# IntelLabs/coach

Measured on AMD Instinct MI355X. Metric: env-steps/sec (+ grad-updates/sec) on Atari-like Clipped-PPO, 64 vectorized envs/GPU, higher is better.
Workload: dtype f32; 1 GPU; C2: Atari-Pong-like Clipped-PPO, 64 vectorized envs/GPU, 84x84x4 uint8 obs, GAE(0.99,0.95), rollout 2048 env-steps (episodes of 32), 10 epochs x 32 minibatches of 64, fp32 conv torso x2 (value/policy), TF1-Adam; parallelism=dp1 (env vectors sharded per GPU, flat fp32 gradient all-reduce), hip_graphs=True

## Files before the change

### coach_amd/_rlx.py

```python
import ctypes
import os
import re
import subprocess
import threading

_HERE = os.path.dirname(os.path.abspath(__file__))
_ROOT = os.path.dirname(_HERE)
HEADER = os.path.join(_ROOT, "include", "rlx.h")
LIB_PATH = os.path.join(_HERE, "librlx.so")
CSRC = os.path.join(_HERE, "csrc")


class RlxUnavailable(RuntimeError):
    """librlx.so is missing or cannot be loaded; the HIP hot path cannot run."""


class RlxError(RuntimeError):
    """A librlx entry point returned a non-zero rlx_status."""


_CTYPE = {
    "int": ctypes.c_int,
    "unsigned": ctypes.c_uint,
    "unsigned int": ctypes.c_uint,
# ... 78 lines not shown
                             {"_fields_": fields, "__doc__": "%s (include/rlx.h)." % name, "__module__": __name__})
    return structs


def parse_constants(text):
    consts = {k: int(v) for k, v in _DEFINE.findall(text)}
    for body in _ENUM.findall(text):
        for item in filter(None, (" ".join(i.split()) for i in body.split(","))):
            m = re.fullmatch(r"(RLX_\w+) ?= ?(-?\d+)", item)
            if not m:
                raise ValueError("rlx.h: enumerator %r needs an explicit integer value" % item)
            consts[m.group(1)] = int(m.group(2))
    return consts


def build_library(verbose=False):
    hipcc = os.environ.get("HIPCC", "/opt/rocm/bin/hipcc")
    if not os.path.exists(hipcc):
        raise RlxUnavailable("hipcc not found at %s; cannot build librlx.so" % hipcc)
    jobs = str(max(1, min(16, os.cpu_count() or 1)))
    res = subprocess.run(["make", "-C", CSRC, "-j", jobs, "HIPCC=" + hipcc],
                         stdout=subprocess.PIPE, stderr=subprocess.STDOUT, text=True)
    if verbose or res.returncode != 0:
        print(res.stdout)
    if res.returncode != 0:
        raise RlxUnavailable("building librlx.so failed (see output above)")
    return LIB_PATH


def _as_arg(a):
    if hasattr(a, "data_ptr"):
        if hasattr(a, "is_contiguous") and not a.is_contiguous():
            raise ValueError("librlx expects contiguous tensors")
        return a.data_ptr()
    return a


class _Lib:
    def __init__(self):
        import torch

        if not os.path.exists(LIB_PATH):
            if os.path.exists("/opt/rocm/bin/hipcc"):
                build_library()
            else:
                raise RlxUnavailable(
                    "%s is missing and hipcc is not available to build it. Run "
                    "`python -c 'import __graft_entry__ as g; g.build()'`." % LIB_PATH)
        try:
            self._dll = ctypes.CDLL(LIB_PATH, mode=ctypes.RTLD_GLOBAL)
        except OSError as e:
            raise RlxUnavailable("cannot load %s: %s" % (LIB_PATH, e))
        self.protos = parse_header()
        self._fns = {}
        missing = []
        for name, (restype, params) in self.protos.items():
            try:
                fn = getattr(self._dll, name)
            except AttributeError:
                missing.append(name)
                continue
            fn.restype = restype
            fn.argtypes = [t for t, _ in params]
            self._fns[name] = fn
        if missing:
            raise RlxUnavailable("librlx.so does not export: " + ", ".join(missing))
        built = self._fns["rlx_abi_version"]()
        if built != ABI_VERSION:
            raise RlxUnavailable("%s is ABI version %d, this package drives version %d: rebuild it "
                                 "(python -c 'import __graft_entry__ as g; g.build()')" % (LIB_PATH, built, ABI_VERSION))

    def raw(self, name):
        return self._fns[name]

    def last_error(self):
        return self._fns["rlx_last_error"]().decode()

    def __getattr__(self, name):
        fns = self.__dict__.get("_fns", {})
        full = name if name.startswith("rlx_") else "rlx_" + name
        if full not in fns:
            raise AttributeError(name)
        fn = fns[full]
        nparams = len(self.protos[full][1])
        if fn.restype is ctypes.c_char_p:
            def call_str(*args):
                return fn(*args).decode()
            return call_str
        if returns_value(full):
            return fn

        def call(*args):
            global CALL_COUNT
            CALL_COUNT += 1
            if len(args) != nparams:
                raise TypeError("%s expects %d arguments, got %d" % (full, nparams, len(args)))
            rc = fn(*[_as_arg(a) for a in args])
            if rc != 0:
                raise RlxError("%s failed (%d): %s" % (full, rc, self.last_error()))
            return rc
        call.__name__ = full
        setattr(self, name, call)
        return call


_lock = threading.Lock()
_lib = None


def lib():
    global _lib
    if _lib is None:
        with _lock:
            if _lib is None:
                _lib = _Lib()
    return _lib


def current_stream():
    import torch
    return torch.cuda.current_stream().cuda_stream


class KernelTimer(object):

    def __init__(self, max_records=4096):
        self.max_records, self.records = int(max_records), []

    def __enter__(self):
        lib().profile_begin(self.max_records)
        return self

    def __exit__(self, *exc):
        n = ctypes.c_int()
        try:
            lib().profile_end(ctypes.byref(n))
        except Exception:
            if exc[0] is None:
                raise
        if exc[0] is None:
            name, ms = ctypes.c_char_p(), ctypes.c_float()
            for i in range(n.value):
                lib().profile_read(i, ctypes.byref(name), ctypes.byref(ms))
                self.records.append((name.value.decode().strip("()"), 1e3 * ms.value))
        return False


STRUCT_NAMES = {
    "rlx_column": "Column", "rlx_gemm_desc": "GemmDesc", "rlx_splitk_job": "SplitkJob", "rlx_noisy_layer": "NoisyLayer",
    "rlx_per_update_desc": "PerUpdateDesc", "rlx_conv_dw_item": "ConvDwItem",
    "rlx_small_dense_problem": "SmallDenseProblem", "rlx_mlp_dqn_desc": "MlpDqnDesc", "rlx_mlp3": "Mlp3",
    "rlx_fused_net": "FusedNet", "rlx_td3_fused_desc": "Td3FusedDesc", "rlx_sac_fused_desc": "SacFusedDesc",
    "rlx_ppo_fc_heads_desc": "PpoFcHeadsDesc", "rlx_ppo_rows_desc": "PpoRowsDesc", "rlx_observe_desc": "ObserveDesc",
    "rlx_signal_source": "SignalSource",
}
_TEXT = header_text()
STRUCTS = parse_structs(_TEXT, STRUCT_NAMES)
CONSTANTS = parse_constants(_TEXT)

Column, GemmDesc, NoisyLayer = STRUCTS["rlx_column"], STRUCTS["rlx_gemm_desc"], STRUCTS["rlx_noisy_layer"]
PerUpdateDesc, ConvDwItem = STRUCTS["rlx_per_update_desc"], STRUCTS["rlx_conv_dw_item"]
SmallDenseProblem, MlpDqnDesc = STRUCTS["rlx_small_dense_problem"], STRUCTS["rlx_mlp_dqn_desc"]
Mlp3, FusedNet = STRUCTS["rlx_mlp3"], STRUCTS["rlx_fused_net"]
Td3FusedDesc, SacFusedDesc = STRUCTS["rlx_td3_fused_desc"], STRUCTS["rlx_sac_fused_desc"]
PpoFcHeadsDesc, PpoRowsDesc = STRUCTS["rlx_ppo_fc_heads_desc"], STRUCTS["rlx_ppo_rows_desc"]
ObserveDesc, SignalSource = STRUCTS["rlx_observe_desc"], STRUCTS["rlx_signal_source"]


class SplitkJob(STRUCTS["rlx_splitk_job"]):
    __doc__ = STRUCTS["rlx_splitk_job"].__doc__

    def workspace_floats(self):
        return (self.M * self.N + self.N) * self.batch * self.splits if self.splits > 1 else 0


ABI_VERSION = CONSTANTS["RLX_ABI_VERSION"]
NOISY_PASSES = CONSTANTS["RLX_NOISY_PASSES"]
NOISY_MAX_LAYERS = CONSTANTS["RLX_NOISY_MAX_LAYERS"]
NOISY_PASS = {"act": 0, "online": 1, "target": 2, "online_next": 3}
assert sorted(NOISY_PASS.values()) == list(range(NOISY_PASSES)), "NOISY_PASS names every pass of RLX_NOISY_PASSES"
ADAM_TICKET_WORDS = CONSTANTS["RLX_ADAM_TICKET_WORDS"]
MAX_SPLITK_JOBS = CONSTANTS["RLX_MAX_SPLITK_JOBS"]
MAX_COLUMNS = CONSTANTS["RLX_MAX_COLUMNS"]
A3C_TARGETS_GIVEN = CONSTANTS["RLX_A3C_TARGETS_GIVEN"]
NSTEPQ_HORIZON = {"N-Step": CONSTANTS["RLX_NSTEPQ_N_STEP"], "1-Step": CONSTANTS["RLX_NSTEPQ_ONE_STEP"]}
NSTEPQ_TARGETS_GIVEN = CONSTANTS["RLX_NSTEPQ_TARGETS_GIVEN"]
ACER_TRUST_REGION, ACER_TARGETS_GIVEN = CONSTANTS["RLX_ACER_TRUST_REGION"], CONSTANTS["RLX_ACER_TARGETS_GIVEN"]
ACT = {None: CONSTANTS["RLX_ACT_NONE"]}
ACT.update((k[len("RLX_ACT_"):].lower(), v) for k, v in CONSTANTS.items() if k.startswith("RLX_ACT_"))


def make_columns(pairs):
    arr = (Column * len(pairs))()
    for i, (s, d) in enumerate(pairs):
        rb = (s[0].numel() if s.dim() > 1 else 1) * s.element_size()
        arr[i] = Column(s.data_ptr(), d.data_ptr(), rb)
    return arr


def splitk_reduce_jobs(jobs, stream=None, ppo_tail=None, per_tail=None):
    live = [j for j in jobs if j.splits > 1]
    s = current_stream() if stream is None else stream
    for i in range(0, len(live), MAX_SPLITK_JOBS):
        chunk = live[i:i + MAX_SPLITK_JOBS]
        arr = (SplitkJob * len(chunk))(*chunk)
        if per_tail is not None and ppo_tail is None and i + MAX_SPLITK_JOBS >= len(live):
            run = lambda a=arr, n=len(chunk), t=per_tail: lib().splitk_reduce_jobs_per_update(ctypes.byref(a), n, *t, s)
            per_tail = None
        elif ppo_tail is not None and i + MAX_SPLITK_JOBS >= len(live):
            run = lambda a=arr, n=len(chunk), t=ppo_tail: lib().splitk_reduce_jobs_ppo_tail(ctypes.byref(a), n, ctypes.byref(t), s)
            ppo_tail = None
        else:
            run = lambda a=arr, n=len(chunk): lib().splitk_reduce_jobs(ctypes.byref(a), n, s)
        _record((), run, flops=0.0)
        run()
    if ppo_tail is not None:
        lib().ppo_heads_tail(ctypes.byref(ppo_tail), s)
    if per_tail is not None:
        lib().per_update(*per_tail, s)


def conv_input_grad(dz, weights, dx, x_out, deriv, tables, B, H, W, C, KH, KW, S, Co, towers, dy_stride, w_stride,
                    dx_stride, stream=None):
    s = current_stream() if stream is None else stream
    OH, OW = (H - KH) // S + 1, (W - KW) // S + 1
    run = lambda: lib().conv_input_grad(dz, weights, dx, x_out, ACT[deriv], tables, B, H, W, C, KH, KW, S, Co, towers,
                                        dy_stride, w_stride, dx_stride, s)
    if GEMM_HOOK is not None:
        d = GemmDesc()
        d.M, d.N, d.K, d.batch = B * OH * OW, KH * KW * C, Co, towers
        _record((d,), run)
    run()


def per_update_desc(args):
    sum_t, min_t, max_t, cap, idx, err, n, alpha, eps, maxp, status = args
    d = PerUpdateDesc()
    d.sum_tree, d.min_tree, d.max_tree, d.capacity = sum_t.data_ptr(), min_t.data_ptr(), max_t.data_ptr(), int(cap)
    d.idx, d.td_errors, d.n, d.alpha, d.epsilon = idx.data_ptr(), err.data_ptr(), int(n), float(alpha), float(eps)
    d.max_priority, d.status = maxp.data_ptr(), status.data_ptr()
    return d


def conv_dw_item(x, x_tower_stride, x_is_u8, a_div, dz, dz_tower_stride, B, H, W, C, KH, KW, S, Co, towers, dw, dw_tower_stride, db,
                 db_tower_stride, workspace):
    it = ConvDwItem()
    it.x, it.x_tower_stride, it.x_is_u8, it.a_div = x.data_ptr(), x_tower_stride, int(bool(x_is_u8)), float(a_div)
    it.dz, it.dz_tower_stride = dz.data_ptr(), dz_tower_stride
    it.B, it.H, it.W, it.C, it.KH, it.KW, it.S, it.filters, it.towers = B, H, W, C, KH, KW, S, Co, towers
    it.dw, it.dw_tower_stride, it.db, it.db_tower_stride = dw.data_ptr(), dw_tower_stride, _ptr(db), db_tower_stride
    it.workspace, it.workspace_floats = workspace.data_ptr(), workspace.numel()
    return it


def conv_dw_multi(items, jobs, stream=None):
    s = current_stream() if stream is None else stream
    n = len(items)
    arr = (ConvDwItem * n)(*items)
    jarr = (SplitkJob * n)()

    def run():
        lib().conv_dw_multi(arr, jarr, n, s)
    if GEMM_HOOK is not None:
        descs = []
        for it in items:
            OH, OW = (it.H - it.KH) // it.S + 1, (it.W - it.KW) // it.S + 1
            d = GemmDesc()
            d.M, d.K = it.KH * it.KW * it.C, it.B * OH * OW
            d.N, d.batch, d.a_is_u8 = (it.towers * it.filters, 1, 1) if it.x_is_u8 else (it.filters, it.towers, 0)
            descs.append(d)
        _record(tuple(descs), run)
    run()
    for j, out in zip(jarr, jobs):
        ctypes.memmove(ctypes.byref(out), ctypes.byref(j), ctypes.sizeof(SplitkJob))


GEMM_HOOK = None
CALL_COUNT = 0


def _ptr(t):
    return None if t is None else (t.data_ptr() if hasattr(t, "data_ptr") else t)


def gemm(M, N, K, A, B, C, *, a_strides=None, a_tabs=None, a_u8=False, a_div=1.0,
         a_vec_along_k=1, a_tab_vec_ok=0, b_strides=None, ldc=None, bias=None, activation=None,
         deriv_aux=None, aux_ld=None, deriv_kind=None, accumulate=False, batch=1,
         a_batch_stride=0, b_batch_stride=0, c_batch_stride=0, bias_batch_stride=0,
         aux_batch_stride=0, workspace=None, colsum_out=None, colsum_batch_stride=0, stream=None,
         batch_inner=0, a_batch_stride2=0, b_batch_stride2=0, bias_batch_stride2=0, n_fold=0, launch=True,
         defer=None, row_heads=None, kw_min_tiles=0):
    d = GemmDesc()
    d.M, d.N, d.K, d.batch = int(M), int(N), int(K), int(batch)
    d.A, d.B, d.C = _ptr(A), _ptr(B), _ptr(C)
    if a_tabs is not None:
        d.a_row_tab, d.a_k_tab = _ptr(a_tabs[0]), _ptr(a_tabs[1])
        d.a_row_stride, d.a_k_stride = 0, 0
    else:
        rs, ks = a_strides if a_strides is not None else (K, 1)
        d.a_row_stride, d.a_k_stride = int(rs), int(ks)
    ks, ns = b_strides if b_strides is not None else (N, 1)
    d.b_k_stride, d.b_n_stride = int(ks), int(ns)
    d.a_batch_stride, d.b_batch_stride = int(a_batch_stride), int(b_batch_stride)
    d.ldc = int(N if ldc is None else ldc)
    d.c_batch_stride, d.bias_batch_stride = int(c_batch_stride), int(bias_batch_stride)
    d.bias, d.deriv_aux = _ptr(bias), _ptr(deriv_aux)
    d.aux_ld = int(N if aux_ld is None else aux_ld)
    d.aux_batch_stride = int(aux_batch_stride)
    d.workspace = _ptr(workspace)
    d.colsum_out, d.colsum_batch_stride = _ptr(colsum_out), int(colsum_batch_stride)
    d.workspace_floats = int(workspace.numel()) if workspace is not None else 0
    d.a_is_u8, d.a_div = int(bool(a_u8)), float(a_div)
    d.a_vec_along_k, d.a_tab_vec_ok = int(a_vec_along_k), int(a_tab_vec_ok)
    d.activation, d.deriv_kind = ACT[activation], ACT[deriv_kind]
    d.accumulate = int(bool(accumulate))
    d.batch_inner = int(batch_inner)
    d.a_batch_stride2, d.b_batch_stride2 = int(a_batch_stride2), int(b_batch_stride2)
    d.bias_batch_stride2 = int(bias_batch_stride2)
    d.n_fold = int(n_fold)
    d.kw_min_tiles = int(kw_min_tiles)
    if row_heads is not None:
        d._row_heads = row_heads
        d.row_heads, d.n_row_heads = ctypes.addressof(row_heads), len(row_heads)
    if not launch:
        return d
    s = current_stream() if stream is None else stream
    if defer is not None:
        run = lambda: lib().gemm_defer(ctypes.byref(d), ctypes.byref(defer), s)
    else:
        run = lambda: lib().gemm(ctypes.byref(d), s)
    _record((d,), run)
    run()


def _record(descs, run, flops=None):
    if GEMM_HOOK is not None:
        GEMM_HOOK({"descs": tuple(GemmDesc.from_buffer_copy(x) for x in descs), "run": run, "flops": flops})


def gemm_pair_or_single(desc, stream=None):
    s = current_stream() if stream is None else stream
    run = lambda: lib().gemm(ctypes.byref(desc), s)
    _record((desc,), run)
    run()


def gemm_multi(descs, jobs, stream=None):
    s = current_stream() if stream is None else stream
    n = len(descs)
    darr = (GemmDesc * n)(*descs)
    jarr = (SplitkJob * n)()

    def run():
        lib().gemm_multi_defer(darr, n, jarr, s)
        for i, j in enumerate(jobs):
            ctypes.memmove(ctypes.addressof(j), ctypes.addressof(jarr[i]), ctypes.sizeof(SplitkJob))
    _record(tuple(descs), run)
    run()


def gemm_pair(weight_grad, input_grad, stream=None, defer=None):
    s = current_stream() if stream is None else stream
    if defer is not None:
        run = lambda: lib().gemm_pair_defer(ctypes.byref(weight_grad), ctypes.byref(input_grad), ctypes.byref(defer), s)
    else:
        run = lambda: lib().gemm_pair(ctypes.byref(weight_grad), ctypes.byref(input_grad), s)
    _record((weight_grad, input_grad), run)
    run()
```

### coach_amd/agents/clipped_ppo_agent.py

```python
import os
import random

import numpy as np
import torch

from .. import _rlx
from ..core_types import EnvironmentSteps, RunPhase
from ..memories.episodic.episodic_rollout_buffer import DeviceEpisodicRolloutBuffer
from ..nn.networks import ClippedPPONet
from ..schedules import ConstantSchedule


from ..architectures.scheme_views import SchemeViews


class ClippedPPONetworkParameters(SchemeViews):
    def __init__(self):
        self.activation_function = 'tanh'
        self.embedder_scheme = 'Medium'
        self.middleware_scheme = 'Medium'
        self.batch_size = 64
        self.optimizer_type = 'Adam'
        self.learning_rate = 0.00025
        self.adam_optimizer_beta1 = 0.9
        self.adam_optimizer_beta2 = 0.99
        self.optimizer_epsilon = 0.0001
        self.clip_gradients = None
        self.use_separate_networks_per_head = True
        self.async_training = False
        self.l2_regularization = 0
        self.create_target_network = True
        self.shared_optimizer = True
        self.scale_down_gradients_by_number_of_workers_for_sync_training = True


class ClippedPPOAlgorithmParameters(object):
    def __init__(self):
        self.discount = 0.99
        self.num_episodes_in_experience_replay = 1000000
        self.gae_lambda = 0.95
        self.use_kl_regularization = False
        self.clip_likelihood_ratio_using_epsilon = 0.2
        self.estimate_state_value_using_gae = True
        self.beta_entropy = 0.01
        self.num_consecutive_playing_steps = EnvironmentSteps(2048)
        self.num_consecutive_training_steps = 1
        self.optimization_epochs = 10
        self.clipping_decay_schedule = ConstantSchedule(1)
        self.act_for_full_episodes = True
        self.reward_clipping = (-1.0, 1.0)
        self.reward_rescale = 1.0
        self.normalize_observations = False


class ClippedPPOAgentParameters(object):
    def __init__(self):
        self.algorithm = ClippedPPOAlgorithmParameters()
        self.network_wrappers = {"main": ClippedPPONetworkParameters()}
        self.seed = 0

    @property
    def path(self):
        return 'coach_amd.agents.clipped_ppo_agent:ClippedPPOAgent'


def _capture(fn):
    from .vector_agent import capture
    return capture(fn)


class ClippedPPOAgent(object):
    epoch_graph = True
    ragged = False
    _device_env = True
    restarts_memory_on_reset = True
    FUSE_ACTING_LAUNCHES = True
    RECORD_WHILE_ACTING = True
    DATASET_CHUNK = 2048

    def __init__(self, agent_parameters, environment, device=None, dist=None, use_graphs=None):
        self.ap = agent_parameters
        self.env = environment
        self.device = device or environment.device
        self.dist = dist if (dist is not None and dist.enabled) else None
        self.lib = _rlx.lib()
        self.use_graphs = True if use_graphs is None else bool(use_graphs)
        self.overlap_allreduce = None if self.dist is not None else False
        self.overlap_decision = None
        alg, net = self.ap.algorithm, self.ap.network_wrappers["main"]
        ep = environment.p
        self.continuous = ep.action_dim is not None
        self.n_env, self.A = ep.num_envs, (ep.action_dim if self.continuous else ep.num_actions)
        self.image = ep.kind == "image"
        self.stack = 4
        self.L = ep.episode_length
        obs_shape = tuple(ep.observation_shape) + (self.stack,) if self.image else tuple(ep.observation_shape)
        if self.ap.seed is not None:
            random.seed(self.ap.seed)
            np.random.seed(self.ap.seed)
        self.networks = {"main": ClippedPPONet(
            self.device, obs_shape, self.A, activation=net.activation_function,
            embedder=net.embedder_scheme, middleware=net.middleware_scheme,
            learning_rate=net.learning_rate, adam_beta1=net.adam_optimizer_beta1,
            adam_beta2=net.adam_optimizer_beta2, optimizer_epsilon=net.optimizer_epsilon,
            clip_likelihood_ratio_using_epsilon=alg.clip_likelihood_ratio_using_epsilon,
            beta_entropy=alg.beta_entropy, seed=self.ap.seed or 0, continuous=self.continuous)}
        if self.dist is not None and self.ap.seed is not None:
            random.seed(self.ap.seed + self.dist.rank)
            np.random.seed(self.ap.seed + self.dist.rank)
        per_env = -(-alg.num_consecutive_playing_steps.num_steps // self.n_env)
        self.steps_per_phase = -(-per_env // self.L) * self.L
        self._device_env = hasattr(environment, "launch_step") and hasattr(environment, "host_tick")
        lens = getattr(environment, "lengths_host", None)
        self.ragged = getattr(environment, "dones_host", None) is not None and \
            (lens is None or getattr(environment, "lengths", None) is not None)
        if self.ragged:
            longest = int(max(lens)) if lens is not None else int(self.L)
            self.steps_per_phase = per_env + longest * (1 if lens is not None else 4)
        self.memory = DeviceEpisodicRolloutBuffer(
            self.device, self.n_env, self.steps_per_phase,
            frame_shape=ep.observation_shape if self.image else None, stack=self.stack,
            obs_dim=None if self.image else int(ep.observation_shape[0]),
            action_dim=self.A if self.continuous else None)
        self._rec_missing = False
        dev, n = self.device, self.n_env
        self.actions = torch.zeros((n, self.A), dtype=torch.float32, device=dev) if self.continuous else \
            torch.zeros(n, dtype=torch.int32, device=dev)
        self.norm = None
        if alg.normalize_observations:
            if self.image:
                raise ValueError("ObservationNormalizationFilter applies to vector observations")
            from ..filters.observation import ObservationNormalizationFilter
            self.norm = ObservationNormalizationFilter(int(ep.observation_shape[0]), dev)
            self.act_obs = torch.empty(n, int(ep.observation_shape[0]), dtype=torch.float32, device=dev)
        self._records_acting()
        if self.continuous:
            lo = np.broadcast_to(np.asarray(ep.action_low, dtype=np.float32), (self.A,)).copy()
            hi = np.broadcast_to(np.asarray(ep.action_high, dtype=np.float32), (self.A,)).copy()
            self.d_low, self.d_high = torch.from_numpy(lo).to(dev), torch.from_numpy(hi).to(dev)
        self.filtered_reward = torch.zeros(n, dtype=torch.float32, device=dev)
        self.ep_return = torch.zeros(n, dtype=torch.float64, device=dev)
        self.ep_len = torch.zeros(n, dtype=torch.int32, device=dev)
        self.ep_acc = torch.zeros(8, dtype=torch.float64, device=dev)
        self.lib.episode_stats_init(self.ep_return, self.ep_len, n, self.ep_acc, _rlx.current_stream())
        self.phase = RunPhase.TRAIN
        self.total_steps_counter = 0
        self.last_training_phase_step = 0
        self.training_iteration = 0
        self.signals = {}
        self._graphs = {}
        self._warm = set()
        self._episode_steps = np.zeros(self.n_env, dtype=np.int64)
        self._episode_just_ended = False
        self._draw_pool, self._draw_pos, self._draw_table_from = None, 0, None
        self._eval_mem = None
        self._alloc_training_buffers()
        self.memory.reset(self.env.reset_internal_state())

    def _alloc_training_buffers(self):
        from ..staging import Stager
        dev, B = self.device, self.ap.network_wrappers["main"].batch_size
        cap = self.memory.cap
        f32, f64 = torch.float32, torch.float64
        self.ds_reward = torch.empty(cap, dtype=f32, device=dev)
        self.ds_done = torch.empty(cap, dtype=torch.uint8, device=dev)
        act_shape = (cap, self.A) if self.continuous else (cap,)
        self.ds_action = torch.empty(act_shape, dtype=self.actions.dtype, device=dev)
        self.ds_value = torch.empty(cap, dtype=f32, device=dev)
        self.ds_adv64 = torch.empty(cap, dtype=f64, device=dev)
        self.ds_adv = torch.empty(cap, dtype=f32, device=dev)
        self.ds_vtarget = torch.empty(cap, dtype=f32, device=dev)
        self.ds_old_probs = torch.empty(cap, self.A, dtype=f32, device=dev)
        self.ds_old_std = torch.empty(cap, self.A, dtype=f32, device=dev) if self.continuous else None
        if self.norm is not None:
            D = self.memory.obs_dim
            self.ds_obs_raw = torch.empty(cap, D, dtype=f32, device=dev)
            self.ds_obs = torch.empty(cap, D, dtype=f32, device=dev)
        self.adv_stats = torch.empty(2, dtype=f64, device=dev)
        obs_tail = tuple(self.memory.cur_state.shape[1:])
        odt = self.memory.cur_state.dtype
        self.chunk = min(int(self.DATASET_CHUNK), cap)
        self.chunk_obs = torch.empty((self.chunk,) + obs_tail, dtype=odt, device=dev)
        self.mb_obs = torch.empty((B,) + obs_tail, dtype=odt, device=dev)
        self.mb_rows = torch.empty(B, dtype=torch.int32, device=dev)
        self._perm = Stager((cap,), torch.int32, dev, depth=4)
        self.perm_dev = self._perm.dst
        self.mb_action = torch.empty((B, self.A) if self.continuous else (B,), dtype=self.actions.dtype, device=dev)
        self.mb_old_std = torch.empty(B, self.A, dtype=f32, device=dev) if self.continuous else None
        self.mb_adv = torch.empty(B, dtype=f32, device=dev)
        self.mb_vtarget = torch.empty(B, dtype=f32, device=dev)
        self.mb_old = torch.empty(B, self.A, dtype=f32, device=dev)
        self.mb_ratio = torch.empty(B, dtype=f32, device=dev)
        self.mb_clipped = torch.empty(B, dtype=f32, device=dev)
        self.scalar_acc = torch.zeros(8, dtype=f32, device=dev)
        shape = (self.steps_per_phase, self.n_env, self.A) if self.continuous else (self.steps_per_phase, self.n_env)
        if self.ragged:
            shape = (1,) + shape[1:]
        self._uniforms = Stager(shape, f64, dev, depth=32 if self.ragged else 4)
        self.uniforms_all = self._uniforms.dst

    def _run(self, key, fn):
        if not self.use_graphs:
            return fn()
        g = self._graphs.get(key)
        if g is not None:
            return g.replay()
        if key not in self._warm:
            self._warm.add(key)
            return fn()
        torch.cuda.synchronize()
        self._graphs[key] = _capture(fn)
        return self._graphs[key].replay()

    def _refill_draws(self, from_step):
        shape = (self.n_env, self.A) if self.continuous else (self.n_env,)
        need = self.steps_per_phase - from_step
        left = self._draw_pool[self._draw_pos:] if self._draw_pool is not None else np.zeros((0,) + shape)
        if left.shape[0] < need:
            m = need - left.shape[0]
            fresh = np.random.standard_normal((m,) + shape) if self.continuous else np.random.random_sample((m,) + shape)
            left = np.concatenate([left, fresh], 0)
        self._draw_pool, self._draw_pos = left, 0
        table = np.zeros((self.steps_per_phase,) + shape, dtype=np.float64)
        table[from_step:] = left[:need]
        self._uniforms.push(table)
        self._draw_table_from = from_step

    def _act_device(self, step):
        s = _rlx.current_stream()
        alg = self.ap.algorithm
# ... 142 lines not shown
        else:
            if getattr(self, "_eval_state", None) is None:
                self._eval_state = torch.empty_like(self.memory.cur_state)
            self._eval_state.copy_(first)
        if getattr(self, "_eval_total", None) is None:
            self._eval_total = torch.zeros(n, dtype=torch.float64, device=dev)
            self._eval_active = torch.ones(n, dtype=torch.float64, device=dev)
        self._eval_total.zero_()
        self._eval_active.fill_(1.0)
        finished = np.zeros(n, dtype=np.int64)
        lockstep_t = 0
        try:
            while (finished < episodes_per_env).any():
                if self._device_env:
                    self._run(("evaluate",), lambda: self._evaluate_device(scratch))
                    self.env.host_tick()
                else:
                    self._evaluate_device(scratch)
                self.env.total_steps += n
                dh = getattr(self.env, "dones_host", None)
                if dh is None:
                    lockstep_t += 1
                    dh = np.full(n, lockstep_t % self.L == 0)
                was_active = finished < episodes_per_env
                finished += dh.astype(np.int64)
                active = finished < episodes_per_env
                if (active != was_active).any():
                    self._eval_active.copy_(torch.from_numpy(active.astype(np.float64)))
        finally:
            self.phase = prev
            self.env.phase = prev_env if prev_env is not None else prev
            self._episode_steps[:] = 0
            self._episode_just_ended = False
            self.lib.episode_stats_init(self.ep_return, self.ep_len, n, None, s)
            self.memory.reset(self.env.reset_internal_state())
        return float(self._eval_total.mean().item()) / episodes_per_env

    def _should_train(self):
        steps = self.ap.algorithm.num_consecutive_playing_steps.num_steps
        if self.ragged:
            done = self.memory.num_transitions_in_complete_episodes()
            if done >= steps or (self.memory.steps >= self.memory.T and done > 0):
                if done < steps and self.dist is not None:
                    raise ValueError("rollout buffer full with %d < %d complete-episode transitions: with data "
                                     "parallelism every rank trains on num_consecutive_playing_steps transitions; "
                                     "declare a longer max episode length" % (done, steps))
                self.last_training_phase_step = self.total_steps_counter
                return True
            if self.memory.steps >= self.memory.T:
                raise ValueError("no episode completed within %d vector steps: an episode is longer than the "
                                 "environment's declared maximum" % self.memory.T)
            return False
        enough = (self.total_steps_counter - self.last_training_phase_step) >= steps
        complete = self.memory.steps > 0 and self.memory.steps % self.L == 0
        if enough and complete and self.memory.num_transitions() > 0:
            self.last_training_phase_step = self.total_steps_counter
            return True
        return False

    def _fill_advantages_device(self, n, rows, n_train=None, recorded=False):
        mem, net, alg = self.memory, self.networks["main"], self.ap.algorithm
        n_train = n if n_train is None else min(n, n_train)
        s = _rlx.current_stream()
        cols = [(mem.reward, self.ds_reward), (mem.game_over, self.ds_done), (mem.action, self.ds_action)]
        if recorded:
            cols += [(mem.act_value, self.ds_value), (mem.act_probs, self.ds_old_probs)]
        mem.gather_columns(rows, n, cols)
        if self.norm is not None:
            mem.gather_states(rows, n, self.ds_obs_raw[:n])
            self.norm.filter(self.ds_obs_raw[:n], update_internal_state=self.dist is None, out=self.ds_obs[:n])
            if self.dist is None:
                mem.gather_next_states(rows, n, self.ds_obs_raw[:n])
                self.norm.push(self.ds_obs_raw[:n])

        def chunk_obs(c0, m):
            if self.norm is not None:
                return self.ds_obs[c0:c0 + m]
            return mem.gather_states(rows[c0:c0 + m], m, self.chunk_obs[:m])
        for c0 in range(0, 0 if recorded else n, self.chunk):
            m = min(self.chunk, n - c0)
            net.values(chunk_obs(c0, m), m, out=self.ds_value[c0:c0 + m])
        n_seq = 1 if self.ragged else mem.n_env
        self.lib.gae(self.ds_reward, self.ds_value, self.ds_done, None, n_seq, n // n_seq,
                     alg.discount, alg.gae_lambda, self.ds_adv64, self.ds_vtarget, s)
        self.lib.standardize(self.ds_adv64, n, self.ds_adv, None, self.adv_stats, s)
        for c0 in range(0, 0 if recorded else n_train, self.chunk):
            m = min(self.chunk, n_train - c0)
            if self.continuous:
                net.policy_mean_std(chunk_obs(c0, m), m, use_target=True, tag="old",
                                    out_mean=self.ds_old_probs[c0:c0 + m], out_std=self.ds_old_std[c0:c0 + m])
            else:
                net.policy_probs(chunk_obs(c0, m), m, use_target=True, tag="old",
                                 out=self.ds_old_probs[c0:c0 + m])

    def fill_advantages(self):
        n = self.memory.num_transitions()
        rows = self.memory.dataset_rows()
        if self.norm is not None and self.dist is not None:
            self.memory.gather_states(rows, n, self.ds_obs_raw[:n])
            self.norm.push_shared(self.ds_obs_raw[:n], self.dist)
        n_train = min(n, self.ap.algorithm.num_consecutive_playing_steps.num_steps)
        recorded = self._records_acting() and not self._rec_missing
        self._run(("fill", n, n_train, recorded), lambda: self._fill_advantages_device(n, rows, n_train, recorded))
        if self.norm is not None and self.dist is not None:
            self.memory.gather_next_states(rows, n, self.ds_obs_raw[:n])
            self.norm.push_shared(self.ds_obs_raw[:n], self.dist)

    def _gather_minibatch(self, m, i=0):
        mem, s = self.memory, _rlx.current_stream()
        rows_all = mem.dataset_rows()
        B = self.ap.network_wrappers["main"].batch_size
        idx, rows = self.perm_dev[i * B:i * B + m], self.mb_rows[:m]
        cols = [(rows_all, rows), (self.ds_action, self.mb_action), (self.ds_adv, self.mb_adv), (self.ds_vtarget, self.mb_vtarget),
                (self.ds_old_probs, self.mb_old)]
        if self.continuous:
            cols.append((self.ds_old_std, self.mb_old_std))
        if self.norm is not None:
            cols.append((self.ds_obs, self.mb_obs))
        self.lib.copy_columns(_rlx.make_columns(cols), len(cols), idx, None, 0, 0, self.ds_adv.numel(), m, m,
                              mem.status, s)
        if self.norm is not None:
            return self.mb_obs[:m]
        return mem.gather_states(rows, m, self.mb_obs[:m])

    def _gather_epoch(self, n):
        mem, s = self.memory, _rlx.current_stream()
        e = self._epoch_buffers()
        cols = [(mem.dataset_rows(), e["rows"]), (self.ds_action, e["action"]), (self.ds_adv, e["adv"]),
                (self.ds_vtarget, e["vtarget"]), (self.ds_old_probs, e["old"])]
        if self.continuous:
            cols.append((self.ds_old_std, e["old_std"]))
        if self.norm is not None:
            cols.append((self.ds_obs, e["obs"]))
        self.lib.copy_columns(_rlx.make_columns(cols), len(cols), self.perm_dev[:n], None, 0, 0, self.ds_adv.numel(), n, n,
                              mem.status, s)
        if self.norm is None:
            mem.gather_states(e["rows"][:n], n, e["obs"][:n])
        return e

    def _epoch_buffers(self):
        e = getattr(self, "_epoch_bufs", None)
        if e is None:
            cap, dev, f32 = self.memory.cap, self.device, torch.float32
            e = self._epoch_bufs = dict(
                rows=torch.empty(cap, dtype=torch.int32, device=dev),
                action=torch.empty((cap, self.A) if self.continuous else (cap,), dtype=self.actions.dtype, device=dev),
                adv=torch.empty(cap, dtype=f32, device=dev), vtarget=torch.empty(cap, dtype=f32, device=dev),
                old=torch.empty(cap, self.A, dtype=f32, device=dev),
                old_std=torch.empty(cap, self.A, dtype=f32, device=dev) if self.continuous else None,
                obs=torch.empty((cap,) + tuple(self.mb_obs.shape[1:]), dtype=self.mb_obs.dtype, device=dev))
        return e

    def _minibatch_fb(self, m, clip_rescaler, stop_after_dense=False, i=0, epoch=None):
        if epoch is not None:
            B = self.ap.network_wrappers["main"].batch_size
            sl = slice(i * B, i * B + m)
            old = (epoch["old"][sl], epoch["old_std"][sl]) if self.continuous else epoch["old"][sl]
            self.networks["main"].forward_backward(epoch["obs"][sl], m, epoch["action"][sl], epoch["adv"][sl],
                                                   epoch["vtarget"][sl], old, clip_rescaler, self.mb_ratio,
                                                   self.mb_clipped, stop_after_dense=stop_after_dense)
            return
        obs = self._gather_minibatch(m, i)
        old = (self.mb_old, self.mb_old_std) if self.continuous else self.mb_old
        self.networks["main"].forward_backward(obs, m, self.mb_action, self.mb_adv, self.mb_vtarget,
                                               old, clip_rescaler, self.mb_ratio, self.mb_clipped,
                                               stop_after_dense=stop_after_dense)

    def _minibatch_finish(self, scale):
        net = self.networks["main"]
        net.finish_update(scale, signal_acc=self.scalar_acc)

    OVERLAP_EDGE_PAIR_US = 50.0

    def _decide_overlap(self, n, clip):
        net, d = self.networks["main"], self.dist
        off = net.late_gradient_offset()
        rec = {"graph_resident": bool(self.use_graphs and d.capturable()), "edge_pair_us": self.OVERLAP_EDGE_PAIR_US,
               "late_bucket_allreduce_us": None, "conv_backward_us": None}
        if not rec["graph_resident"] or off <= 0:
            rec.update(overlap=False, why="collectives are not graph nodes on this backend" if off > 0
                       else "no early-finished bucket (no convolution layers)")
        else:
            B = self.ap.network_wrappers["main"].batch_size
            m = min(B, n)
            e = self._gather_epoch(n)
            ev = [torch.cuda.Event(enable_timing=True) for _ in range(2)]
            us = []
            for _ in range(3):
                self._minibatch_fb(m, clip, True, i=0, epoch=e)
                ev[0].record()
                net.backward_rest()
                ev[1].record()
                ev[1].synchronize()
                us.append(1e3 * ev[0].elapsed_time(ev[1]))
            bw = d.max_over_ranks(min(us))
            ar = d.max_over_ranks(d.all_reduce_us(net.params.grads.numel() - off) or 0.0)
            hidden = min(ar, bw)
            rec.update(late_bucket_allreduce_us=round(ar, 1), conv_backward_us=round(bw, 1), overlap=bool(hidden > self.OVERLAP_EDGE_PAIR_US),
                       why="min(all-reduce, convolution backward) = %.1f us %s the %.0f us edge pair"
                           % (hidden, ">" if hidden > self.OVERLAP_EDGE_PAIR_US else "<=", self.OVERLAP_EDGE_PAIR_US))
        self.overlap_decision = rec
        self.overlap_allreduce = rec["overlap"]

    def train_network(self, order, epochs):
        alg = self.ap.algorithm
        netp = self.ap.network_wrappers["main"]
        B = netp.batch_size
        n = len(order)
        self.networks["main"].set_clip_rescaler(float(alg.clipping_decay_schedule.current_value))
        clip = None
        scale = self.dist.grad_scale(netp.scale_down_gradients_by_number_of_workers_for_sync_training) \
            if self.dist else 1.0
        results = []
        for j in range(epochs):
            batch_order = list(range(n))
            random.shuffle(batch_order)
            order = [order[i] for i in batch_order]
            full = np.zeros(self.perm_dev.numel(), dtype=np.int32)
            full[:n] = order
            self._perm.push(full)
            self.scalar_acc.zero_()
            nmb = -(-n // B)
            if self.overlap_allreduce is None:
                self._decide_overlap(n, clip)
            in_graph = self.dist is not None and self.use_graphs and self.dist.capturable()
            net = self.networks["main"]

            def reduced_fb(m, i, e=None):
                if self.overlap_allreduce and net.late_gradient_offset() > 0:
                    grads, off = net.params.grads, net.late_gradient_offset()
                    self._minibatch_fb(m, clip, True, i=i, epoch=e)
                    w1 = self.dist.all_reduce_sum_async(grads[off:])
                    net.backward_rest()
                    w2 = self.dist.all_reduce_sum_async(grads[:off])
                    w1.wait()
                    w2.wait()
                else:
                    self._minibatch_fb(m, clip, i=i, epoch=e)
                    self.dist.all_reduce_sum(net.params.grads)

            if (self.dist is None or in_graph) and self.epoch_graph and not self.ragged:
                def epoch():
                    e = self._gather_epoch(n)
                    for i in range(nmb):
                        if self.dist is None:
                            self._minibatch_fb(min(B, n - i * B), clip, i=i, epoch=e)
                        else:
                            reduced_fb(min(B, n - i * B), i, e)
                        self._minibatch_finish(scale)
                self._run(("epoch", n, clip, scale, self.dist is not None and self.overlap_allreduce), epoch)
                results.append(self.scalar_acc / nmb)
                continue
            for i in range(nmb):
                m = min(B, n - i * B)
                if self.dist is None:
                    self._run(("mb", m, clip, scale, i), lambda: (self._minibatch_fb(m, clip, i=i),
                                                                  self._minibatch_finish(scale)))
                elif in_graph:
                    self._run(("mb_dp", m, clip, scale, i, self.overlap_allreduce),
                              lambda: (reduced_fb(m, i), self._minibatch_finish(scale)))
                elif not self.overlap_allreduce:
                    if i == 0:
                        self._run(("mb_fb", m, clip, i), lambda: self._minibatch_fb(m, clip, i=i))
                    else:
                        self._run(("mb_fin_fb", m, clip, scale, i),
                                  lambda: (self._minibatch_finish(scale), self._minibatch_fb(m, clip, i=i)))
                    self.dist.all_reduce_sum(self.networks["main"].params.grads)
                    if i == nmb - 1:
                        self._run(("mb_fin", scale), lambda: self._minibatch_finish(scale))
                else:
                    grads, off = net.params.grads, net.late_gradient_offset()
                    self._run(("mb_p1", m, clip, i), lambda: self._minibatch_fb(m, clip, True, i=i))
                    w1 = self.dist.all_reduce_sum_async(grads[off:])
                    self._run(("mb_p2", m), net.backward_rest)
                    w2 = self.dist.all_reduce_sum_async(grads[:off]) if off > 0 else None
                    w1.wait()
                    if w2 is not None:
                        w2.wait()
                    self._run(("mb_fin", scale), lambda: self._minibatch_finish(scale))
            results.append(self.scalar_acc / nmb)
        return results

    def post_training_commands(self):
        self.memory.clean()
        self._rec_missing = False

    def train(self):
        if not self._should_train():
            return None
        alg = self.ap.algorithm
        net = self.networks["main"]
        results = None
        for pass_index in range(alg.num_consecutive_training_steps):
            net.update_target(1.0)
            if pass_index > 0:
                self._rec_missing = True
            self.fill_advantages()
            n = min(self.memory.num_transitions(), alg.num_consecutive_playing_steps.num_steps)
            order = list(range(n))
            random.shuffle(order)
            results = self.train_network(order, alg.optimization_epochs)
        self.post_training_commands()
        self.training_iteration += 1
        last = results[-1]
        self.signals = {"Surrogate loss": last[0], "Entropy": last[1], "KL Divergence": last[2],
                        "Value Loss": last[4], "Grads (unclipped)": last[5]}
        return results

    def check_status(self):
        bits = int(self.memory.status.item())
        if bits:
            self.memory.status.zero_()
            raise ValueError("rollout buffer kernel reported an out-of-range row (status bits %d)" % bits)
        for net in self.networks.values():
            net.check_status()

    def episode_statistics(self):
        a = self.ep_acc.cpu().numpy()
        n = max(a[0], 1.0)
        return {"episodes": int(a[0]), "mean_return": a[1] / n, "max_return": a[3], "min_return": a[4],
                "mean_length": a[5] / n}
```

### coach_amd/csrc/conv_dw_multi.hip

```cpp
#include "conv_dw_body.hpp"

namespace {

using namespace rlx_convdw;

struct MultiArgs {
    DwU8 u8;
    DwF32 f[2];
    int nb_u8, nb_f[2], kind[2];
    int u8_half;
};

template <int PASSES>
__global__ void __launch_bounds__(kThreads) conv_dw_multi_kernel(const MultiArgs m) {
    extern __shared__ __attribute__((aligned(16))) float smem[];
    int bid = blockIdx.x;
    if (bid < m.nb_u8) {
        if (m.u8_half) conv_dw_u8_body_half(m.u8, bid, smem);
        else if constexpr (PASSES > 1) conv_dw_u8_body_passes<PASSES>(m.u8, bid, smem);
        else conv_dw_u8_body<20, 16, 84>(m.u8, bid, smem);
        return;
    }
    bid -= m.nb_u8;
#pragma unroll
    for (int i = 0; i < 2; ++i) {
        if (bid < m.nb_f[i]) {
            if (m.kind[i] == 1) {
                if constexpr (PASSES > 1) conv_dw_f32_body_two_pass<64, 3, 1, 9, 7, 4, 7>(m.f[i], bid, smem);
                else conv_dw_f32_body<64, 3, 1, 9, 7>(m.f[i], bid, smem);
            } else {
                if constexpr (PASSES > 1) conv_dw_f32_body_two_pass<32, 4, 2, 20, 9, 5, 9>(m.f[i], bid, smem);
                else conv_dw_f32_body<32, 4, 2, 20, 9>(m.f[i], bid, smem);
            }
            return;
        }
        bid -= m.nb_f[i];
    }
}

int g_passes = 2;
int g_pairs_per_wg = 0;
inline int pairs_per_wg(int B, int towers) {
    if (g_passes <= 1) return 1;
    if (g_pairs_per_wg > 0) return g_pairs_per_wg;
    return towers * ((B + 1) / 2) >= 64 ? 2 : 1;
}

}

extern "C" {

int rlx_conv_dw_multi(const rlx_conv_dw_item *items, rlx_splitk_job *jobs, int n_items, void *stream) {
    RLX_REQUIRE(items && jobs && n_items >= 1 && n_items <= 3, "rlx_conv_dw_multi: 1 .. 3 items");
    int n_u8 = 0, n_f = 0;
    bool one = n_items >= 2;
    GeometryU8 gu;
    GeometryF32 gf[2];
    const rlx_conv_dw_item *iu = nullptr, *fi[2] = {nullptr, nullptr};
    int ju = -1, jf[2] = {-1, -1};
    for (int i = 0; i < n_items && one; ++i) {
        const rlx_conv_dw_item &it = items[i];
        if (it.x_is_u8) {
            one = n_u8 == 0 && geometry_u8(it.B, it.H, it.W, it.C, it.KH, it.KW, it.S, it.filters, it.towers, &gu) && gu.OW == 20 &&
                  gu.OH == 20 && it.S * it.C == 16 && gu.rowf == 336;
            iu = &it; ju = i; ++n_u8;
        } else {
            one = n_f < 2 && geometry_f32(it.B, it.H, it.W, it.C, it.KH, it.KW, it.S, it.filters, it.towers, &gf[n_f < 2 ? n_f : 1],
                                          pairs_per_wg(it.B, it.towers));
            if (n_f < 2) { fi[n_f] = &it; jf[n_f] = i; }
            ++n_f;
        }
    }
    if (!one) {
        for (int i = 0; i < n_items; ++i) {
            const rlx_conv_dw_item &it = items[i];
            const int rc = it.x_is_u8
                ? rlx_conv_dw_u8(static_cast<const unsigned char *>(it.x), it.a_div, it.dz, it.dz_tower_stride, it.B, it.H, it.W, it.C,
                                 it.KH, it.KW, it.S, it.filters, it.towers, it.dw, it.dw_tower_stride, it.db, it.db_tower_stride,
                                 it.workspace, it.workspace_floats, &jobs[i], stream)
                : rlx_conv_dw_f32(static_cast<const float *>(it.x), it.x_tower_stride, it.dz, it.dz_tower_stride, it.B, it.H, it.W,
                                  it.C, it.KH, it.KW, it.S, it.filters, it.towers, it.dw, it.dw_tower_stride, it.db,
                                  it.db_tower_stride, it.workspace, it.workspace_floats, &jobs[i], stream);
            if (rc != RLX_OK) return rc;
        }
        return RLX_OK;
    }
    MultiArgs m;
    m.nb_u8 = m.nb_f[0] = m.nb_f[1] = 0;
    m.kind[0] = m.kind[1] = 0;
    m.u8_half = 0;
    size_t lds = 0;
    if (iu) {
        const rlx_conv_dw_item &it = *iu;
        RLX_REQUIRE(it.x && it.dz && it.dw && it.workspace && it.a_div != 0.f, "rlx_conv_dw_multi: null pointer (uint8 item)");
        const long long need = (long long)it.B * ((long long)gu.K * kN + kN);
        RLX_REQUIRE(it.workspace_floats >= need, "rlx_conv_dw_multi: workspace of %lld floats, need %lld", it.workspace_floats, need);
        RLX_REQUIRE((((uintptr_t)it.x) & 3) == 0 && ((((uintptr_t)it.dz) | ((uintptr_t)it.workspace)) & 15) == 0 &&
                        (it.dz_tower_stride & 3) == 0, "rlx_conv_dw_multi: misaligned operand (uint8 item)");
        DwU8 &a = m.u8;
        a.x = static_cast<const unsigned char *>(it.x); a.dz = it.dz; a.dz_ts = it.dz_tower_stride;
        a.part = it.workspace; a.cpart = it.workspace + (size_t)it.B * gu.K * kN;
        a.a_div = it.a_div;
        a.B = it.B; a.H = it.H; a.W = it.W; a.C = it.C; a.KH = it.KH; a.S = it.S; a.OH = gu.OH; a.OW = gu.OW; a.Co = it.filters;
        a.K = gu.K; a.P = gu.P; a.rowf = gu.rowf; a.NQ = gu.NQ; a.stamps = nullptr;
        m.nb_u8 = ((it.B + 7) / 8) * 8 * gu.NQ;
        m.u8_half = gu.nch == kNH;
        lds = gu.lds;
        rlx_splitk_job &j = jobs[ju];
        j.partials = a.part; j.colsum_partials = it.db ? a.cpart : nullptr;
        j.C = it.dw; j.colsum_out = it.db;
        j.ldc = it.filters; j.c_batch_stride = it.dw_tower_stride; j.colsum_batch_stride = it.db_tower_stride;
        j.M = gu.K; j.N = gu.nch; j.batch = 1; j.splits = gu.splits; j.n_fold = it.filters;
    }
    for (int k = 0; k < 2; ++k) {
        if (!fi[k]) continue;
        const rlx_conv_dw_item &it = *fi[k];
        const GeometryF32 &g = gf[k];
        RLX_REQUIRE(it.x && it.dz && it.dw && it.workspace, "rlx_conv_dw_multi: null pointer (fp32 item)");
        const long long need = (long long)it.towers * g.splits * ((long long)g.K * kN + kN);
        RLX_REQUIRE(it.workspace_floats >= need, "rlx_conv_dw_multi: workspace of %lld floats, need %lld", it.workspace_floats, need);
        RLX_REQUIRE(((((uintptr_t)it.x) | ((uintptr_t)it.dz) | ((uintptr_t)it.workspace)) & 15) == 0 && (it.x_tower_stride & 3) == 0 &&
                        (it.dz_tower_stride & 3) == 0, "rlx_conv_dw_multi: misaligned operand (fp32 item)");
        DwF32 &a = m.f[k];
        a.x = static_cast<const float *>(it.x); a.x_ts = it.x_tower_stride; a.dz = it.dz; a.dz_ts = it.dz_tower_stride;
        a.part = it.workspace; a.cpart = it.db ? it.workspace + (size_t)it.towers * g.splits * g.K * kN : nullptr;
        a.B = it.B; a.H = it.H; a.OH = g.OH; a.KH = it.KH; a.splits = g.splits; a.units = it.towers * g.splits;
        a.ppw = pairs_per_wg(it.B, it.towers);
        a.stamps = nullptr;
        m.nb_f[k] = ((a.units + 7) / 8) * 8 * it.KH;
        m.kind[k] = g.kind;
        lds = g.lds > lds ? g.lds : lds;
        rlx_splitk_job &j = jobs[jf[k]];
        j.partials = a.part; j.colsum_partials = a.cpart;
        j.C = it.dw; j.colsum_out = it.db;
        j.ldc = it.filters; j.c_batch_stride = it.dw_tower_stride; j.colsum_batch_stride = it.db_tower_stride;
        j.M = g.K; j.N = kN; j.batch = it.towers; j.splits = g.splits; j.n_fold = 0;
    }
    static bool configured = false;
    if (!configured) {
        RLX_HIP(hipFuncSetAttribute(reinterpret_cast<const void *>(conv_dw_multi_kernel<1>),
                                    hipFuncAttributeMaxDynamicSharedMemorySize, 160 * 1024));
        RLX_HIP(hipFuncSetAttribute(reinterpret_cast<const void *>(conv_dw_multi_kernel<2>),
                                    hipFuncAttributeMaxDynamicSharedMemorySize, 160 * 1024));
        RLX_HIP(hipFuncSetAttribute(reinterpret_cast<const void *>(conv_dw_multi_kernel<4>),
                                    hipFuncAttributeMaxDynamicSharedMemorySize, 160 * 1024));
        configured = true;
    }
    const unsigned grid = m.nb_u8 + m.nb_f[0] + m.nb_f[1];
    if (g_passes > 1) {
        size_t lds2 = iu ? (m.u8_half ? lds_u8_half() : (g_passes == 4 ? lds_u8_passes<4>() : lds_u8_passes<2>())) : 0;
        for (int k = 0; k < 2; ++k) {
            if (!fi[k]) continue;
            const size_t l = m.kind[k] == 2 ? lds_f32_two_pass<32, 20, 9, 5>() : lds_f32_two_pass<64, 9, 7, 4>();
            lds2 = l > lds2 ? l : lds2;
        }
        if (g_passes == 4) RLX_LAUNCH((conv_dw_multi_kernel<4>), grid, kThreads, lds2, rlx::as_stream(stream), m);
        else RLX_LAUNCH((conv_dw_multi_kernel<2>), grid, kThreads, lds2, rlx::as_stream(stream), m);
    } else {
        RLX_LAUNCH((conv_dw_multi_kernel<1>), grid, kThreads, lds, rlx::as_stream(stream), m);
    }
    RLX_LAUNCH_CHECK();
    return RLX_OK;
}

int rlx_conv_dw_pairs_per_workgroup(int pairs) {
    RLX_REQUIRE(pairs >= 0 && pairs <= 2, "rlx_conv_dw_pairs_per_workgroup: 0 (by the number of workgroups), 1 or 2");
    g_pairs_per_wg = pairs;
    return RLX_OK;
}

int rlx_conv_dw_passes(int passes) {
    RLX_REQUIRE(passes == 1 || passes == 2 || passes == 4, "rlx_conv_dw_passes: 1, 2 or 4");
    g_passes = passes;
    return RLX_OK;
}

}
```

### coach_amd/csrc/optim.hip

```cpp
#include "rlx_common.hpp"

namespace {

constexpr int kBlock = 256;

#if defined(__HIP_DEVICE_COMPILE__) && !defined(__gfx950__) && !defined(__gfx942__)
#error "optim.hip: the last-arriver ticket protocol is written for gfx950 (gfx942-compatible) only"
#endif

constexpr unsigned kTicketGroups = 32, kTicketStride = 32;
static_assert(kTicketStride * (1 + kTicketGroups) == RLX_ADAM_TICKET_WORDS, "rlx.h: RLX_ADAM_TICKET_WORDS");
__device__ __forceinline__ bool draw_last_ticket(unsigned int *ticket) {
    const unsigned G = gridDim.x < kTicketGroups ? gridDim.x : kTicketGroups;
    const unsigned grp = blockIdx.x % G, gsize = (gridDim.x - grp + G - 1) / G;
    unsigned int *gw = ticket + kTicketStride * (1 + grp);
    if (__hip_atomic_fetch_add(gw, 1u, __ATOMIC_RELAXED, __HIP_MEMORY_SCOPE_AGENT) != gsize - 1) return false;
    __hip_atomic_store(gw, 0u, __ATOMIC_RELAXED, __HIP_MEMORY_SCOPE_AGENT);
    if (__hip_atomic_fetch_add(ticket, 1u, __ATOMIC_RELAXED, __HIP_MEMORY_SCOPE_AGENT) != G - 1) return false;
    __hip_atomic_store(ticket, 0u, __ATOMIC_RELAXED, __HIP_MEMORY_SCOPE_AGENT);
    return true;
}

template <bool NORM>
__global__ void adam_tf1_kernel(float *__restrict__ w, const float *__restrict__ g,
                                float *__restrict__ m, float *__restrict__ v, long long n,
                                float lr, float beta1, float beta2, float eps,
                                const float *__restrict__ state, float grad_scale,
                                float *__restrict__ sumsq_part) {
    __shared__ float red[kBlock];
    float ss = 0.f;
    const float b1p = state[0], b2p = state[1];
    const float alpha = lr * sqrtf(1.f - b2p) / (1.f - b1p);
    const float omb1 = 1.f - beta1, omb2 = 1.f - beta2;
    const long long stride = (long long)gridDim.x * blockDim.x;
    const long long n4 = n >> 2;
    for (long long i = (long long)blockIdx.x * blockDim.x + threadIdx.x; i < n4; i += stride) {
        float4 gw = reinterpret_cast<const float4 *>(g)[i];
        float4 mw = reinterpret_cast<float4 *>(m)[i];
        float4 vw = reinterpret_cast<float4 *>(v)[i];
        float4 ww = reinterpret_cast<float4 *>(w)[i];
        float *gp = &gw.x, *mp = &mw.x, *vp = &vw.x, *wp = &ww.x;
#pragma unroll
        for (int k = 0; k < 4; ++k) {
            if (NORM) ss += gp[k] * gp[k];
            const float gr = gp[k] * grad_scale;
            mp[k] += (gr - mp[k]) * omb1;
            vp[k] += (gr * gr - vp[k]) * omb2;
            wp[k] -= (mp[k] * alpha) / (sqrtf(vp[k]) + eps);
        }
        reinterpret_cast<float4 *>(m)[i] = mw;
        reinterpret_cast<float4 *>(v)[i] = vw;
        reinterpret_cast<float4 *>(w)[i] = ww;
    }
    for (long long i = (n4 << 2) + (long long)blockIdx.x * blockDim.x + threadIdx.x; i < n; i += stride) {
        if (NORM) ss += g[i] * g[i];
        const float gr = g[i] * grad_scale;
        m[i] += (gr - m[i]) * omb1;
        v[i] += (gr * gr - v[i]) * omb2;
        w[i] -= (m[i] * alpha) / (sqrtf(v[i]) + eps);
    }
    if (NORM) {
        red[threadIdx.x] = ss;
        __syncthreads();
        for (int d = kBlock >> 1; d > 0; d >>= 1) {
            if (threadIdx.x < d) red[threadIdx.x] += red[threadIdx.x + d];
            __syncthreads();
        }
        if (threadIdx.x == 0) sumsq_part[blockIdx.x] = red[0];
    }
}


template <bool NORM, bool MIX, bool TICKET>
__global__ void __launch_bounds__(kBlock)
adam_step_kernel(float *__restrict__ w, const float *__restrict__ g, float *__restrict__ m, float *__restrict__ v,
                 long long n, float lr, float beta1, float beta2, float eps, float *state, float grad_scale,
                 float *sumsq_part, float *__restrict__ target, float rate, float one_minus_rate,
                 unsigned int *ticket, float *norm_out, const float *acc_src, float *acc_dst, int n_acc) {
    __shared__ float red[kBlock];
    __shared__ int last_s;
    float ss = 0.f;
    const float b1p = state[0], b2p = state[1];
    const float alpha = lr * sqrtf(1.f - b2p) / (1.f - b1p);
    const float omb1 = 1.f - beta1, omb2 = 1.f - beta2;
    const long long stride = (long long)gridDim.x * blockDim.x;
    const long long n4 = n >> 2;
    for (long long i = (long long)blockIdx.x * blockDim.x + threadIdx.x; i < n4; i += stride) {
        float4 gw = reinterpret_cast<const float4 *>(g)[i];
        float4 mw = reinterpret_cast<float4 *>(m)[i];
        float4 vw = reinterpret_cast<float4 *>(v)[i];
        float4 ww = reinterpret_cast<float4 *>(w)[i];
        float4 tw = MIX ? reinterpret_cast<float4 *>(target)[i] : make_float4(0.f, 0.f, 0.f, 0.f);
        float *gp = &gw.x, *mp = &mw.x, *vp = &vw.x, *wp = &ww.x, *tp = &tw.x;
#pragma unroll
        for (int k = 0; k < 4; ++k) {
            if (NORM) ss += gp[k] * gp[k];
            const float gr = gp[k] * grad_scale;
            mp[k] += (gr - mp[k]) * omb1;
            vp[k] += (gr * gr - vp[k]) * omb2;
            wp[k] -= (mp[k] * alpha) / (sqrtf(vp[k]) + eps);
            if (MIX) tp[k] = rate * wp[k] + one_minus_rate * tp[k];
        }
        reinterpret_cast<float4 *>(m)[i] = mw;
        reinterpret_cast<float4 *>(v)[i] = vw;
        reinterpret_cast<float4 *>(w)[i] = ww;
        if (MIX) reinterpret_cast<float4 *>(target)[i] = tw;
    }
    for (long long i = (n4 << 2) + (long long)blockIdx.x * blockDim.x + threadIdx.x; i < n; i += stride) {
        if (NORM) ss += g[i] * g[i];
        const float gr = g[i] * grad_scale;
        m[i] += (gr - m[i]) * omb1;
        v[i] += (gr * gr - v[i]) * omb2;
        w[i] -= (m[i] * alpha) / (sqrtf(v[i]) + eps);
        if (MIX) target[i] = rate * w[i] + one_minus_rate * target[i];
    }
    if (NORM) {
        red[threadIdx.x] = ss;
        __syncthreads();
        for (int d = kBlock >> 1; d > 0; d >>= 1) {
            if (threadIdx.x < d) red[threadIdx.x] += red[threadIdx.x + d];
            __syncthreads();
        }
        if (threadIdx.x == 0) {
            if (TICKET) __hip_atomic_store(&sumsq_part[blockIdx.x], red[0], __ATOMIC_RELAXED, __HIP_MEMORY_SCOPE_AGENT);
            else sumsq_part[blockIdx.x] = red[0];
        }
    }
    if (!TICKET) return;
    __syncthreads();
    if (threadIdx.x == 0) {
        if (NORM) asm volatile("s_waitcnt vmcnt(0)" ::: "memory");
        const bool last = draw_last_ticket(ticket);
        if (last && !NORM) {
            state[0] = b1p * beta1;
            state[1] = b2p * beta2;
        }
        last_s = last;
    }
    if (!NORM) return;
    __syncthreads();
    if (!last_s) return;
    __builtin_amdgcn_fence(__ATOMIC_ACQUIRE, "agent");
    float s = 0.f;
    for (int i = threadIdx.x; i < (int)gridDim.x; i += kBlock)
        s += __hip_atomic_load(&sumsq_part[i], __ATOMIC_RELAXED, __HIP_MEMORY_SCOPE_AGENT);
    red[threadIdx.x] = s;
    __syncthreads();
    for (int d = kBlock >> 1; d > 0; d >>= 1) {
        if (threadIdx.x < d) red[threadIdx.x] += red[threadIdx.x + d];
        __syncthreads();
    }
    if (threadIdx.x == 0) {
        norm_out[0] = sqrtf(red[0]);
        state[0] = b1p * beta1;
        state[1] = b2p * beta2;
        for (int i = 0; i < n_acc; ++i) acc_dst[i] += acc_src[i];
    }
}

constexpr int kNormIt = 4;
template <bool MIX>
__global__ void __launch_bounds__(kBlock)
adam_step_norm_kernel(float *__restrict__ w, const float *__restrict__ g, float *__restrict__ m, float *__restrict__ v,
                      long long n, float lr, float beta1, float beta2, float eps, float *state, float grad_scale,
                      float *sumsq_part, float *__restrict__ target, float rate, float one_minus_rate,
                      unsigned int *ticket, float *norm_out, const float *acc_src, float *acc_dst, int n_acc) {
    __shared__ float red[kBlock];
    __shared__ int last_s;
    const float b1p = state[0], b2p = state[1];
    const float alpha = lr * sqrtf(1.f - b2p) / (1.f - b1p);
    const float omb1 = 1.f - beta1, omb2 = 1.f - beta2;
    const long long stride = (long long)gridDim.x * blockDim.x;
    const long long n4 = n >> 2;
    const long long i0 = (long long)blockIdx.x * blockDim.x + threadIdx.x;
    float4 gw[kNormIt], mw[kNormIt], vw[kNormIt], ww[kNormIt], tw[kNormIt];
#pragma unroll
    for (int it = 0; it < kNormIt; ++it) {
        const long long i = i0 + it * stride;
        if (i < n4) {
            gw[it] = reinterpret_cast<const float4 *>(g)[i];
            mw[it] = reinterpret_cast<float4 *>(m)[i];
            vw[it] = reinterpret_cast<float4 *>(v)[i];
            ww[it] = reinterpret_cast<float4 *>(w)[i];
            if (MIX) tw[it] = reinterpret_cast<float4 *>(target)[i];
        }
    }
    const long long it0 = (n4 << 2) + i0;
    const bool has_tail = it0 < n;
    const float gt = has_tail ? g[it0] : 0.f;
    float ss = 0.f;
#pragma unroll
    for (int it = 0; it < kNormIt; ++it)
        if (i0 + it * stride < n4) {
            const float *gp = &gw[it].x;
#pragma unroll
            for (int k = 0; k < 4; ++k) ss += gp[k] * gp[k];
        }
    if (has_tail) ss += gt * gt;
    red[threadIdx.x] = ss;
    __syncthreads();
    for (int d = kBlock >> 1; d > 0; d >>= 1) {
        if (threadIdx.x < d) red[threadIdx.x] += red[threadIdx.x + d];
        __syncthreads();
    }
    float old = 0.f;
    if (threadIdx.x == 0)
        old = __hip_atomic_exchange(&sumsq_part[blockIdx.x], red[0], __ATOMIC_RELAXED, __HIP_MEMORY_SCOPE_AGENT);
#pragma unroll
    for (int it = 0; it < kNormIt; ++it) {
        const long long i = i0 + it * stride;
        if (i < n4) {
            float *gp = &gw[it].x, *mp = &mw[it].x, *vp = &vw[it].x, *wp = &ww[it].x, *tp = &tw[it].x;
#pragma unroll
            for (int k = 0; k < 4; ++k) {
                const float gr = gp[k] * grad_scale;
                mp[k] += (gr - mp[k]) * omb1;
                vp[k] += (gr * gr - vp[k]) * omb2;
                wp[k] -= (mp[k] * alpha) / (sqrtf(vp[k]) + eps);
                if (MIX) tp[k] = rate * wp[k] + one_minus_rate * tp[k];
            }
            reinterpret_cast<float4 *>(m)[i] = mw[it];
            reinterpret_cast<float4 *>(v)[i] = vw[it];
            reinterpret_cast<float4 *>(w)[i] = ww[it];
            if (MIX) reinterpret_cast<float4 *>(target)[i] = tw[it];
        }
    }
    if (has_tail) {
        const float gr = gt * grad_scale;
        m[it0] += (gr - m[it0]) * omb1;
        v[it0] += (gr * gr - v[it0]) * omb2;
        w[it0] -= (m[it0] * alpha) / (sqrtf(v[it0]) + eps);
        if (MIX) target[it0] = rate * w[it0] + one_minus_rate * target[it0];
    }
    if (threadIdx.x == 0) {
        asm volatile("" ::"v"(old) : "memory");
        last_s = draw_last_ticket(ticket);
    }
    __syncthreads();
    if (!last_s) return;
    __builtin_amdgcn_fence(__ATOMIC_ACQUIRE, "agent");
    float s = 0.f;
    for (int i = threadIdx.x; i < (int)gridDim.x; i += kBlock)
        s += __hip_atomic_load(&sumsq_part[i], __ATOMIC_RELAXED, __HIP_MEMORY_SCOPE_AGENT);
    red[threadIdx.x] = s;
    __syncthreads();
    for (int d = kBlock >> 1; d > 0; d >>= 1) {
        if (threadIdx.x < d) red[threadIdx.x] += red[threadIdx.x + d];
        __syncthreads();
    }
    if (threadIdx.x == 0) {
        norm_out[0] = sqrtf(red[0]);
        state[0] = b1p * beta1;
        state[1] = b2p * beta2;
        for (int i = 0; i < n_acc; ++i) acc_dst[i] += acc_src[i];
    }
}

__global__ void adam_advance_kernel(float *state, float beta1, float beta2) {
    state[0] *= beta1;
    state[1] *= beta2;
}

__global__ void adam_finish_norm_kernel(float *state, float beta1, float beta2,
                                        const float *__restrict__ part, int nparts,
                                        float *__restrict__ norm_out, const float *acc_src,
                                        float *acc_dst, int n_acc) {
    __shared__ float red[kBlock];
    float s = 0.f;
    for (int i = threadIdx.x; i < nparts; i += kBlock) s += part[i];
    red[threadIdx.x] = s;
    __syncthreads();
    for (int d = kBlock >> 1; d > 0; d >>= 1) {
        if (threadIdx.x < d) red[threadIdx.x] += red[threadIdx.x + d];
        __syncthreads();
    }
    if (threadIdx.x == 0) {
        norm_out[0] = sqrtf(red[0]);
        state[0] *= beta1;
        state[1] *= beta2;
        for (int i = 0; i < n_acc; ++i) acc_dst[i] += acc_src[i];
    }
}

__global__ void mix_kernel(float *__restrict__ target, const float *__restrict__ online, long long n,
                           float rate, float one_minus_rate) {
    const long long stride = (long long)gridDim.x * blockDim.x;
    const long long n4 = n >> 2;
    for (long long i = (long long)blockIdx.x * blockDim.x + threadIdx.x; i < n4; i += stride) {
        const float4 o = reinterpret_cast<const float4 *>(online)[i];
        float4 t = reinterpret_cast<float4 *>(target)[i];
        t.x = rate * o.x + one_minus_rate * t.x;
        t.y = rate * o.y + one_minus_rate * t.y;
        t.z = rate * o.z + one_minus_rate * t.z;
        t.w = rate * o.w + one_minus_rate * t.w;
        reinterpret_cast<float4 *>(target)[i] = t;
    }
    for (long long i = (n4 << 2) + (long long)blockIdx.x * blockDim.x + threadIdx.x; i < n; i += stride)
        target[i] = rate * online[i] + one_minus_rate * target[i];
}

__global__ void sumsq_partial_kernel(const float *__restrict__ x, long long n, float *__restrict__ part) {
    __shared__ float red[kBlock];
    float s = 0.f;
    for (long long i = (long long)blockIdx.x * blockDim.x + threadIdx.x; i < n;
         i += (long long)gridDim.x * blockDim.x)
        s += x[i] * x[i];
    red[threadIdx.x] = s;
    __syncthreads();
    for (int d = kBlock >> 1; d > 0; d >>= 1) {
        if (threadIdx.x < d) red[threadIdx.x] += red[threadIdx.x + d];
        __syncthreads();
    }
    if (threadIdx.x == 0) part[blockIdx.x] = red[0];
}
__global__ void sumsq_final_kernel(const float *__restrict__ part, int nparts, float *__restrict__ out) {
    __shared__ float red[kBlock];
    float s = 0.f;
    for (int i = threadIdx.x; i < nparts; i += kBlock) s += part[i];
    red[threadIdx.x] = s;
    __syncthreads();
    for (int d = kBlock >> 1; d > 0; d >>= 1) {
        if (threadIdx.x < d) red[threadIdx.x] += red[threadIdx.x + d];
        __syncthreads();
    }
    if (threadIdx.x == 0) out[0] = sqrtf(red[0]);
}

__global__ void clip_by_global_norm_kernel(float *__restrict__ g, long long n, const float *__restrict__ norm,
                                           float clip) {
    const float inv_norm = 1.0f / *norm, inv_clip = 1.0f / clip;
    const float scale = clip * (inv_clip < inv_norm ? inv_clip : inv_norm);
    const long long stride = (long long)gridDim.x * blockDim.x;
    for (long long i = (long long)blockIdx.x * blockDim.x + threadIdx.x; i < n; i += stride) g[i] *= scale;
}

__global__ void clip_by_value_kernel(float *__restrict__ g, long long n, float clip) {
    const long long stride = (long long)gridDim.x * blockDim.x;
    for (long long i = (long long)blockIdx.x * blockDim.x + threadIdx.x; i < n; i += stride) {
        float x = g[i];
        x = x < -clip ? -clip : x;
        g[i] = x > clip ? clip : x;
    }
}

int g_norm_in_kernel = 2;
}

extern "C" {

int rlx_adam_init(float *m, float *v, long long n, float *state, float beta1, float beta2,
                  void *stream) {
    RLX_REQUIRE(m && v && state && n > 0, "rlx_adam_init: bad arguments");
    hipStream_t s = rlx::as_stream(stream);
    RLX_HIP(hipMemsetAsync(m, 0, sizeof(float) * n, s));
    RLX_HIP(hipMemsetAsync(v, 0, sizeof(float) * n, s));
    const float init[2] = {beta1, beta2};
    RLX_HIP(hipMemcpyAsync(state, init, sizeof(init), hipMemcpyHostToDevice, s));
    return RLX_OK;
}

int rlx_adam_tf1(float *weights, const float *grads, float *m, float *v, long long n,
                 float learning_rate, float beta1, float beta2, float epsilon, float *state,
                 float grad_scale, void *stream) {
    RLX_REQUIRE(weights && grads && m && v && state, "rlx_adam_tf1: null pointer");
    RLX_REQUIRE(n > 0, "rlx_adam_tf1: empty parameter buffer");
    RLX_REQUIRE((((uintptr_t)weights | (uintptr_t)grads | (uintptr_t)m | (uintptr_t)v) & 15) == 0,
                "rlx_adam_tf1: buffers must be 16-byte aligned");
    hipStream_t s = rlx::as_stream(stream);
    RLX_LAUNCH((adam_tf1_kernel<false>), rlx::grid_for(n / 4 + 1, kBlock), kBlock, 0, s, weights, grads, m, v, n, learning_rate, beta1, beta2, epsilon, state, grad_scale, nullptr);
    RLX_LAUNCH_CHECK();
    RLX_LAUNCH((adam_advance_kernel), 1, 1, 0, s, state, beta1, beta2);
    RLX_LAUNCH_CHECK();
    return RLX_OK;
}

int rlx_adam_tf1_norm(float *weights, const float *grads, float *m, float *v, long long n,
                      float learning_rate, float beta1, float beta2, float epsilon, float *state,
                      float grad_scale, float *norm_out, float *workspace, long long workspace_floats,
                      const float *acc_src, float *acc_dst, int n_acc, void *stream) {
    RLX_REQUIRE(weights && grads && m && v && state && norm_out && workspace,
                "rlx_adam_tf1_norm: null pointer");
    RLX_REQUIRE(n > 0, "rlx_adam_tf1_norm: empty parameter buffer");
    RLX_REQUIRE(n_acc == 0 || (acc_src && acc_dst && n_acc > 0 && n_acc <= 64),
                "rlx_adam_tf1_norm: bad signal accumulation arguments");
    RLX_REQUIRE((((uintptr_t)weights | (uintptr_t)grads | (uintptr_t)m | (uintptr_t)v) & 15) == 0,
                "rlx_adam_tf1_norm: buffers must be 16-byte aligned");
    int blocks = rlx::grid_for(n / 4 + 1, kBlock, 1024);
    if (blocks > workspace_floats) blocks = (int)workspace_floats;
    RLX_REQUIRE(blocks >= 1, "rlx_adam_tf1_norm: workspace too small");
    hipStream_t s = rlx::as_stream(stream);
    RLX_LAUNCH((adam_tf1_kernel<true>), blocks, kBlock, 0, s, weights, grads, m, v, n, learning_rate, beta1, beta2,
                                                    epsilon, state, grad_scale, workspace);
    RLX_LAUNCH_CHECK();
    RLX_LAUNCH((adam_finish_norm_kernel), 1, kBlock, 0, s, state, beta1, beta2, workspace, blocks, norm_out, acc_src,
                                                 acc_dst, n_acc);
    RLX_LAUNCH_CHECK();
    return RLX_OK;
}

int rlx_adam_norm_in_kernel(int on) {
    g_norm_in_kernel = on;
    return RLX_OK;
}

int rlx_adam_tf1_step(float *weights, const float *grads, float *m, float *v, long long n, float learning_rate,
                      float beta1, float beta2, float epsilon, float *state, float grad_scale, float *norm_out,
                      float *workspace, long long workspace_floats, const float *acc_src, float *acc_dst, int n_acc,
                      float *target, double mix_rate, unsigned int *ticket, void *stream) {
    RLX_REQUIRE(weights && grads && m && v && state && ticket, "rlx_adam_tf1_step: null pointer");
    RLX_REQUIRE(n > 0, "rlx_adam_tf1_step: empty parameter buffer");
    RLX_REQUIRE(!norm_out || workspace, "rlx_adam_tf1_step: the gradient norm needs a workspace");
    RLX_REQUIRE(n_acc == 0 || (acc_src && acc_dst && n_acc > 0 && n_acc <= 64),
                "rlx_adam_tf1_step: bad signal accumulation arguments");
    RLX_REQUIRE((((uintptr_t)weights | (uintptr_t)grads | (uintptr_t)m | (uintptr_t)v | (uintptr_t)target) & 15) == 0,
                "rlx_adam_tf1_step: buffers must be 16-byte aligned");
    int blocks = rlx::grid_for(n / 4 + 1, kBlock, 1024);
    if (norm_out && blocks > workspace_floats) blocks = (int)workspace_floats;
    RLX_REQUIRE(blocks >= 1, "rlx_adam_tf1_step: workspace too small");
    hipStream_t s = rlx::as_stream(stream);
    const float rate = (float)mix_rate, omr = (float)(1.0 - mix_rate);
#define RLX_ADAM_STEP(NORM, MIX, TICKET)                                                                      \
    RLX_LAUNCH((adam_step_kernel<NORM, MIX, TICKET>), blocks, kBlock, 0, s, weights, grads, m, v, n, learning_rate, beta1,  \
                                                                  beta2, epsilon, state, grad_scale, workspace, \
                                                                  target, rate, omr, ticket, nullptr, nullptr, nullptr, 0)
    if (norm_out && g_norm_in_kernel == 2 && (n >> 2) <= (long long)blocks * kBlock * kNormIt) {
        if (target)
            RLX_LAUNCH((adam_step_norm_kernel<true>), blocks, kBlock, 0, s, weights, grads, m, v, n, learning_rate, beta1, beta2,
                       epsilon, state, grad_scale, workspace, target, rate, omr, ticket, norm_out, acc_src, acc_dst, n_acc);
        else
            RLX_LAUNCH((adam_step_norm_kernel<false>), blocks, kBlock, 0, s, weights, grads, m, v, n, learning_rate, beta1, beta2,
                       epsilon, state, grad_scale, workspace, target, rate, omr, ticket, norm_out, acc_src, acc_dst, n_acc);
        RLX_LAUNCH_CHECK();
        return RLX_OK;
    }
    if (norm_out && g_norm_in_kernel == 1) {
        if (target)
            RLX_LAUNCH((adam_step_kernel<true, true, true>), blocks, kBlock, 0, s, weights, grads, m, v, n, learning_rate, beta1,
                       beta2, epsilon, state, grad_scale, workspace, target, rate, omr, ticket, norm_out, acc_src, acc_dst, n_acc);
        else
            RLX_LAUNCH((adam_step_kernel<true, false, true>), blocks, kBlock, 0, s, weights, grads, m, v, n, learning_rate, beta1,
                       beta2, epsilon, state, grad_scale, workspace, target, rate, omr, ticket, norm_out, acc_src, acc_dst, n_acc);
        RLX_LAUNCH_CHECK();
        return RLX_OK;
    }
    if (norm_out && target) RLX_ADAM_STEP(true, true, false);
    else if (norm_out) RLX_ADAM_STEP(true, false, false);
    else if (target) RLX_ADAM_STEP(false, true, true);
    else RLX_ADAM_STEP(false, false, true);
#undef RLX_ADAM_STEP
    RLX_LAUNCH_CHECK();
    if (norm_out) {
        RLX_LAUNCH((adam_finish_norm_kernel), 1, kBlock, 0, s, state, beta1, beta2, workspace, blocks, norm_out, acc_src,
                                                     acc_dst, n_acc);
        RLX_LAUNCH_CHECK();
    } else if (n_acc > 0) {
        RLX_REQUIRE(false, "rlx_adam_tf1_step: signal sums ride with the norm finish (give norm_out)");
    }
    return RLX_OK;
}

int rlx_mix_weights(float *target, const float *online, long long n, double rate, void *stream) {
    RLX_REQUIRE(target && online && n > 0, "rlx_mix_weights: bad arguments");
    RLX_REQUIRE((((uintptr_t)target | (uintptr_t)online) & 15) == 0,
                "rlx_mix_weights: buffers must be 16-byte aligned");
    RLX_LAUNCH((mix_kernel), rlx::grid_for(n / 4 + 1, kBlock), kBlock, 0, rlx::as_stream(stream), target, online, n, (float)rate, (float)(1.0 - rate));
    RLX_LAUNCH_CHECK();
    return RLX_OK;
}

int rlx_global_norm(const float *x, long long n, float *norm_out, float *workspace,
                    long long workspace_floats, void *stream) {
    RLX_REQUIRE(x && norm_out && workspace && n > 0, "rlx_global_norm: bad arguments");
    int parts = rlx::grid_for(n, kBlock, 1024);
    if (parts > workspace_floats) parts = (int)workspace_floats;
    RLX_REQUIRE(parts >= 1, "rlx_global_norm: workspace too small");
    hipStream_t s = rlx::as_stream(stream);
    RLX_LAUNCH((sumsq_partial_kernel), parts, kBlock, 0, s, x, n, workspace);
    RLX_LAUNCH_CHECK();
    RLX_LAUNCH((sumsq_final_kernel), 1, kBlock, 0, s, workspace, parts, norm_out);
    RLX_LAUNCH_CHECK();
    return RLX_OK;
}

int rlx_clip_by_global_norm(float *grads, long long n, const float *global_norm, float clip_norm,
                            void *stream) {
    RLX_REQUIRE(grads && global_norm && n > 0, "rlx_clip_by_global_norm: bad arguments");
    RLX_REQUIRE(clip_norm > 0.f, "rlx_clip_by_global_norm: clip_norm must be positive (got %g)", (double)clip_norm);
    RLX_LAUNCH((clip_by_global_norm_kernel), rlx::grid_for(n, kBlock, 1024), kBlock, 0, rlx::as_stream(stream), grads, n, global_norm, clip_norm);
    RLX_LAUNCH_CHECK();
    return RLX_OK;
}

int rlx_clip_by_value(float *grads, long long n, float clip_value, void *stream) {
    RLX_REQUIRE(grads && n > 0, "rlx_clip_by_value: bad arguments");
    RLX_REQUIRE(clip_value > 0.f, "rlx_clip_by_value: clip_value must be positive (got %g)", (double)clip_value);
    RLX_LAUNCH((clip_by_value_kernel), rlx::grid_for(n, kBlock, 1024), kBlock, 0, rlx::as_stream(stream), grads, n, clip_value);
    RLX_LAUNCH_CHECK();
    return RLX_OK;
}

}
```

### coach_amd/nn/graph.py

```python
import ctypes
import math
import os

import numpy as np
import torch

from .. import _rlx

ALIGN = 4
SMALL_N = 16
FOLD_SHARED_INPUT = True


def _thin_takes(M, N, K, batch):
    return K <= 1024 and N * K <= (1 << 18) and -(-M // 64) * -(-N // 64) * batch <= 96


def _fold(M, N, K, T):
    return FOLD_SHARED_INPUT and not (_thin_takes(M, N, K, T) and K >= 64)


def _align(n):
    return (n + ALIGN - 1) // ALIGN * ALIGN


class FlatParams:

    def __init__(self):
        self.entries = {}
        self.size = 0
        self.weights = self.grads = None

    def add_group(self, specs, towers=1):
        per_tower = sum(_align(int(np.prod(s))) for _, s in specs)
        base, off = self.size, 0
        for name, shape in specs:
            if name in self.entries:
                raise ValueError("duplicate parameter name %s" % name)
            self.entries[name] = (base + off, tuple(shape), towers, per_tower)
            off += _align(int(np.prod(shape)))
        self.size += per_tower * towers
        return per_tower

    def finalize(self, device):
        self.both = torch.zeros(2, self.size, dtype=torch.float32, device=device)
        self.weights = self.both[0]
        self.target_weights = self.both[1]
        self.grads = torch.zeros(self.size, dtype=torch.float32, device=device)
        return self

    def view(self, buf, name, tower=0):
        off, shape, towers, stride = self.entries[name]
        n = int(np.prod(shape))
        return buf[off + tower * stride: off + tower * stride + n].view(*shape)

    def w(self, name, tower=0, buf=None):
        return self.view(self.weights if buf is None else buf, name, tower)

    def g(self, name, tower=0):
        return self.view(self.grads, name, tower)

    def stride(self, name):
        return self.entries[name][3]

    def named_arrays(self, buf=None):
        out = {}
        for name, (off, shape, towers, stride) in self.entries.items():
            out[name] = [self.view(self.weights if buf is None else buf, name, t).cpu().numpy().copy()
                         for t in range(towers)]
        return out


def xavier_uniform(rng, fan_in, fan_out, shape):
    limit = math.sqrt(6.0 / (fan_in + fan_out))
    return rng.uniform(-limit, limit, size=shape).astype(np.float32)


def normalized_columns(std):
    def init(shape):
        out = np.random.randn(*shape).astype(np.float32)
        out *= std / np.sqrt(np.square(out).sum(axis=0, keepdims=True))
        return out
    return init


PAIR_GRADIENT_GEMMS = True
DIRECT_CONV_INPUT_GRAD = False
FUSE_CONV_PAIR = True
FUSE_CONV_FIRST = True
FUSE_CONV_INPUT_GRADS = True
FUSE_CONV_INPUT_GRADS_MIN_WORKGROUPS = 64
PER_RIDER_MAX_WORKGROUPS = 256
DENSE_DX_KW_MIN_TILES = 96
CONV1_CHUNKS = None
CONV_FORWARD_WAVE_GROUPS = 4


def _fused_operands_aligned(args):
    prev_tensor = False
    for a in args:
        if hasattr(a, "data_ptr"):
            if a.data_ptr() % 16:
                return False
            prev_tensor = True
        else:
            if prev_tensor and isinstance(a, int) and a % 4:
                return False
            prev_tensor = False
    return True


def _tiled_wave_groups(M, N, batch):
    if N <= 32:
        return 1
    below, least = ctypes.c_int(), ctypes.c_int()
    _rlx.lib().gemm_tuning_get(ctypes.byref(below), ctypes.byref(least), None)
    t64 = -(-M // 64) * -(-N // 64) * batch
    if t64 >= below.value:
        return 1
    if -(-M // 32) * -(-N // 64) * batch >= least.value:
        return 2
    if -(-M // 32) * -(-N // 32) * batch >= least.value:
        return 4
    return 1


def _kw2_tiling(M, N, batch):
    return _tiled_wave_groups(M, N, batch) == 2


MULTI_DW = False
SPLIT_CAP_BOUND = 128
CONV_DW_U8 = True
CONV_DW_F32 = True
CONV_DW_ONE_LAUNCH = True


class Workspace:
    def __init__(self, device, floats=1 << 24):
        self.splitk = torch.empty(floats, dtype=torch.float32, device=device)
        self.splitk_side = torch.empty(floats, dtype=torch.float32, device=device)
        self.small = torch.empty(1 << 18, dtype=torch.float32, device=device)


class Context:

    def __init__(self, device, ws=None):
        self.device = device
        self.lib = _rlx.lib()
        self.ws = ws or Workspace(device)
        self.cache = {}
        self.buffers = {}
        self.overlap = False
        self.deferred, self.arena, self._arena_off = None, None, 0

    @property
    def stream(self):
        return torch.cuda.current_stream().cuda_stream

    def join(self):
        pass

    ARENA_FLOATS = 1 << 25
    _arenas = {}
    private_arena = False

    def begin_deferring(self):
        if self.deferred is not None:
            return False
        if self.arena is None or (self.private_arena and self.arena is Context._arenas.get(str(self.device))):
            if self.private_arena:
                self.arena = torch.empty(self.ARENA_FLOATS, dtype=torch.float32, device=self.device)
            else:
                key = str(self.device)
                if key not in Context._arenas:
                    Context._arenas[key] = torch.empty(self.ARENA_FLOATS, dtype=torch.float32, device=self.device)
                self.arena = Context._arenas[key]
        self.deferred, self._arena_off = [], 0
        return True

    def deferred_workspace(self, M, N, batch):
        bound = (M * N + N) * batch * SPLIT_CAP_BOUND
        room = self.ARENA_FLOATS - self._arena_off
        if self.deferred is None or len(self.deferred) >= _rlx.MAX_SPLITK_JOBS or room < (M * N + N) * batch * 2:
            return None, self.ws.splitk
        return _rlx.SplitkJob(), self.arena[self._arena_off:self._arena_off + min(bound, room)]

    def commit_deferred(self, job, reserved=False):
        if job is not None and job.splits > 1:
            self.deferred.append(job)
            if not reserved:
                self._arena_off += (job.workspace_floats() + 3) // 4 * 4

    def reserve_deferred_workspace(self, M, N, batch):
        job, ws = self.deferred_workspace(M, N, batch)
        if job is not None:
            self._arena_off += (ws.numel() + 3) // 4 * 4
        return job, ws

    def flush_deferred(self):
        jobs, self.deferred = self.deferred, None
        tail, self.ppo_tail = self.ppo_tail, None
        per, self.per_tail = self.per_tail, None
        if jobs or tail is not None or per is not None:
            _rlx.splitk_reduce_jobs(jobs or [], self.stream, ppo_tail=tail, per_tail=per)

    ppo_tail = None
    per_tail = None

    def flush_ppo_tail(self):
        tail, self.ppo_tail = self.ppo_tail, None
        if tail is not None:
            self.lib.ppo_heads_tail(ctypes.byref(tail), self.stream)

    def buffer(self, name, shape, dtype=torch.float32, tag=""):
        key = (name, tuple(shape), dtype, tag)
        buf = self.buffers.get(key)
        if buf is None:
            buf = torch.empty(shape, dtype=dtype, device=self.device)
            self.buffers[key] = buf
        return buf


class Tensor:

    def __init__(self, data, rows, cols, towers, u8=False, div=1.0, grad_key=None, act=None):
        self.data, self.rows, self.cols, self.towers = data, rows, cols, towers
        self.u8, self.div = u8, div
        self.act = act
        self.grad_is_dz = False
        self.grad = None
        self.grad_key = grad_key
        self.bn_saved = None

    def tower_stride(self):
        return 0 if self.towers == 0 else self.rows * self.cols

    def ensure_grad(self):
        if self.grad is None:
            if self.grad_key is not None:
                ctx, name, tag = self.grad_key
                self.grad = ctx.buffer(name + ":grad", tuple(self.data.shape), tag=tag)
            else:
                self.grad = torch.empty(self.data.shape, dtype=torch.float32, device=self.data.device)
        return self.grad

    def tower(self, t):
        g = self.ensure_grad()
        v = Tensor(self.data[t:t + 1], self.rows, self.cols, 1, u8=self.u8, div=self.div, act=self.act)
        v.grad = g[t:t + 1]
        v.bn_saved = self.bn_saved
        return v

    def slice_towers(self, t0, n, with_grad=True):
        v = Tensor(self.data[t0:t0 + n], self.rows, self.cols, n, u8=self.u8, div=self.div, act=self.act)
        if with_grad:
            v.grad = self.ensure_grad()[t0:t0 + n]
        v.bn_saved = self.bn_saved
        return v

    def tower_view(self, t):
        return Tensor(self.data[t:t + 1], self.rows, self.cols, 1, u8=self.u8, div=self.div, act=self.act)


def input_tensor(data, rows, cols, u8=False, div=1.0):
    return Tensor(data, rows, cols, 0, u8=u8, div=div)


class Layer:
    def _range(self, t0, nt):
        nt = self.T - t0 if nt is None else nt
        assert 0 <= t0 and t0 + nt <= self.T
        return t0, nt


class Dense(Layer):

    def __init__(self, params, name, in_features, units, activation=None, towers=1, init=None):
        self.name, self.K, self.N, self.act, self.T = name, in_features, units, activation, towers
        self.init, self.params = init, params
        self.kname, self.bname = name + "/kernel", name + "/bias"
        params.add_group([(self.kname, (in_features, units)), (self.bname, (units,))], towers)

    def initialize(self, rng):
        for t in range(self.T):
            w = self.init((self.K, self.N)) if self.init is not None else \
                xavier_uniform(rng, self.K, self.N, (self.K, self.N))
            self.params.w(self.kname, t).copy_(torch.from_numpy(np.ascontiguousarray(w)))

    def forward(self, ctx, x, tag="", weights=None, t0=0, nt=None, pair=False, launch=True, row_heads=None):
        t0, T = self._range(t0, nt)
        p = self.params
        M = x.rows
        assert x.cols == self.K, (self.name, x.cols, self.K)
        wstride, bstride = p.stride(self.kname), p.stride(self.bname)
        kw = {}
        if pair:
            assert weights is None and t0 == 0 and T == self.T
            if x.towers == 2 * T:
                a_stride, a_stride2 = M * self.K, T * M * self.K
            else:
                assert x.towers == 2, (self.name, x.towers)
                a_stride, a_stride2 = 0, M * self.K
            kw = dict(batch_inner=T, a_batch_stride2=a_stride2, b_batch_stride2=p.size, bias_batch_stride2=p.size)
            TT = 2 * T
        else:
            assert x.towers in (0, T), (self.name, x.towers, T)
            a_stride, TT = x.tower_stride(), T
        y = ctx.buffer(self.name, (TT, M, self.N), tag=tag)
        desc, head_outs = None, None
        if self.N <= SMALL_N and not x.u8:
            if not pair:
                ctx.lib.dense_small_forward(x.data, a_stride, p.w(self.kname, t0, weights), wstride,
                                            p.w(self.bname, t0, weights), bstride, y, M * self.N, T, M,
                                            self.K, self.N, _rlx.ACT[self.act], ctx.stream)
            else:
                import ctypes
                arr = (_rlx.SmallDenseProblem * 2)()
                for c in range(2):
                    q = arr[c]
                    q.x, q.x_tower_stride = x.data.data_ptr() + c * a_stride2 * 4, a_stride
                    q.w, q.w_tower_stride = p.w(self.kname).data_ptr() + c * p.size * 4, wstride
                    q.bias, q.bias_tower_stride = p.w(self.bname).data_ptr() + c * p.size * 4, bstride
                    q.y, q.y_tower_stride = y.data_ptr() + c * T * M * self.N * 4, M * self.N
                    q.towers, q.M, q.K, q.N, q.activation = T, M, self.K, self.N, _rlx.ACT[self.act]
                ctx.lib.dense_small_forward_multi(ctypes.byref(arr), 2, ctx.stream)
        elif launch and not pair and x.towers == 0 and T > 1 and self.N % 4 == 0 and _fold(M, self.N, self.K, T):
            _rlx.gemm(M, T * self.N, self.K, x.data, p.w(self.kname, t0, weights), y,
                      b_strides=(self.N, 1), ldc=self.N, bias=p.w(self.bname, t0, weights),
                      activation=self.act, batch=1, b_batch_stride=wstride, c_batch_stride=M * self.N,
                      bias_batch_stride=bstride, workspace=ctx.ws.splitk, n_fold=self.N)
        else:
            if row_heads:
                heads_arr, head_outs = row_head_problems(ctx, row_heads, y, M, self.N, tag, weights)
                kw = dict(kw, row_heads=heads_arr)
            desc = _rlx.gemm(M, self.N, self.K, x.data, p.w(self.kname, t0, weights), y,
                             bias=p.w(self.bname, t0, weights), activation=self.act, batch=TT,
                             a_batch_stride=a_stride, b_batch_stride=wstride,
                             c_batch_stride=M * self.N, bias_batch_stride=bstride,
                             workspace=ctx.ws.splitk, launch=launch, **kw)
        T = TT
        out = Tensor(y, M, self.N, T, grad_key=(ctx, self.name, tag), act=self.act)
        if row_heads:
            assert head_outs is not None and launch, "row_heads: only on the tiled-GEMM path of a wide layer"
            return out, head_outs
        return out if launch else (out, desc)

    def backward(self, ctx, x, y, need_dx=True, weights=None, t0=0, nt=None, need_dw=True, overlap=False):
        t0, T = self._range(t0, nt)
        M, p = x.rows, self.params
        overlap = overlap and ctx.overlap
        dz = y.grad
        own_act = self.act if (self.act is not None and not y.grad_is_dz) else None
        lower = x.act if need_dx else None
        shared_dx = need_dx and x.towers == 0 and T > 1
        if need_dx and not shared_dx:
            assert x.towers == T, "input gradients need a per-tower input"
        if self.N <= SMALL_N and not x.u8 and M * self.N <= 1024 and not shared_dx:
            dx = x.ensure_grad() if need_dx else None
            ctx.lib.dense_small_backward(
                x.data, x.tower_stride(), p.w(self.kname, t0, weights), p.stride(self.kname),
                dz, M * self.N, y.data if own_act else None, M * self.N,
                p.g(self.kname, t0) if need_dw else None, p.stride(self.kname),
                p.g(self.bname, t0) if need_dw else None, p.stride(self.bname),
                dx, M * self.K, T, M, self.K, self.N, _rlx.ACT[own_act], _rlx.ACT[lower], ctx.stream)
            if need_dx:
                x.grad_is_dz = lower is not None
            return
        if own_act is not None:
            ctx.lib.act_backward(dz, y.data, T * M * self.N, _rlx.ACT[own_act], ctx.stream)
        if need_dw:
            fold = x.towers == 0 and T > 1 and self.N % 4 == 0 and _fold(self.K, self.N, M, T)
            job, dws = ctx.deferred_workspace(self.K, T * self.N if fold else self.N, 1 if fold else T) \
                if not overlap else (None, None)

            def dw(ws, launch=True):
                ws = dws if job is not None else ws
                dj = job if launch else None
                if fold:
                    return _rlx.gemm(self.K, T * self.N, M, x.data, dz, p.g(self.kname, t0), a_strides=(1, self.K),
                                     b_strides=(self.N, 1), ldc=self.N, batch=1, b_batch_stride=M * self.N,
                                     c_batch_stride=p.stride(self.kname), workspace=ws,
                                     colsum_out=p.g(self.bname, t0), colsum_batch_stride=p.stride(self.bname),
                                     n_fold=self.N, launch=launch, defer=dj)
                return _rlx.gemm(self.K, self.N, M, x.data, dz, p.g(self.kname, t0), a_strides=(1, self.K), batch=T,
                                 a_batch_stride=x.tower_stride(), b_batch_stride=M * self.N,
                                 c_batch_stride=p.stride(self.kname), workspace=ws,
                                 colsum_out=p.g(self.bname, t0), colsum_batch_stride=p.stride(self.bname),
                                 launch=launch, defer=dj)
            pair_dw = need_dx and not shared_dx and not overlap and PAIR_GRADIENT_GEMMS
            if not pair_dw:
                dw(ctx.ws.splitk)
        if shared_dx:
            dx = x.ensure_grad()
            for t in range(T):
                _rlx.gemm(M, self.K, self.N, dz[t], p.w(self.kname, t0 + t, weights), dx, b_strides=(1, self.N),
                          workspace=ctx.ws.splitk, deriv_aux=x.data if lower else None, aux_ld=self.K,
                          deriv_kind=lower, accumulate=t > 0)
            x.grad_is_dz = lower is not None
        elif need_dx:
            dx = x.ensure_grad()
            dxd = _rlx.gemm(M, self.K, self.N, dz, p.w(self.kname, t0, weights), dx, b_strides=(1, self.N),
                            batch=T, a_batch_stride=M * self.N, b_batch_stride=p.stride(self.kname),
                            c_batch_stride=M * self.K, workspace=ctx.ws.splitk,
                            deriv_aux=x.data if lower else None, aux_ld=self.K, deriv_kind=lower,
                            aux_batch_stride=M * self.K, launch=False, kw_min_tiles=DENSE_DX_KW_MIN_TILES)
            if need_dw and not overlap and PAIR_GRADIENT_GEMMS:
                _rlx.gemm_pair(dw(ctx.ws.splitk_side, launch=False), dxd, defer=job)
            else:
                _rlx.gemm_pair_or_single(dxd)
            x.grad_is_dz = lower is not None
        if need_dw:
            ctx.commit_deferred(job)


class NoisyDense(Layer):
    SIGMA0 = 0.5

    def __init__(self, params, name, in_features, units, activation=None, towers=1, init=None):
        if towers != 1 or init is not None:
            raise NotImplementedError("NoisyDense: one tower, the layer's own initialiser")
        self.name, self.K, self.N, self.act, self.T, self.params = name, in_features, units, activation, 1, params
        self.wmname, self.bmname = name + "/weight_mean", name + "/bias_mean"
        self.wsname, self.bsname = name + "/weight_stddev", name + "/bias_stddev"
        self.kname, self.bname = self.wmname, self.bmname
        self.index = None
        params.add_group([(self.wmname, (in_features, units)), (self.bmname, (units,)),
                          (self.wsname, (in_features, units)), (self.bsname, (units,))], 1)

    def initialize(self, rng):
        lim = 1.0 / math.sqrt(self.K)
        put = lambda name, a: self.params.w(name).copy_(torch.from_numpy(np.ascontiguousarray(a.astype(np.float32))))
        put(self.wmname, rng.uniform(-lim, lim, size=(self.K, self.N)))
        put(self.wsname, rng.uniform(-self.SIGMA0 * lim, self.SIGMA0 * lim, size=(self.K, self.N)))
        put(self.bsname, rng.uniform(-self.SIGMA0 * lim, self.SIGMA0 * lim, size=(self.N,)))

    def noise(self, ctx, tag):
        return ctx.buffer(self.name + "/noise", (self.K + 2 * self.N,), tag=tag)

    def forward(self, ctx, x, tag="", weights=None, t0=0, nt=None, pair=False, launch=True, row_heads=None):
        if pair or row_heads or not launch:
            raise NotImplementedError("NoisyDense runs as a launch of its own (no paired / row-head / deferred form)")
        self._range(t0, nt)
        assert x.towers in (0, 1) and x.cols == self.K and not x.u8, (self.name, x.towers, x.cols, self.K)
        p, M = self.params, x.rows
        y = ctx.buffer(self.name, (1, M, self.N), tag=tag)
        ctx.lib.noisy_dense_forward(x.data, self.K, p.w(self.wmname, 0, weights), p.w(self.wsname, 0, weights),
                                    p.w(self.bmname, 0, weights), p.w(self.bsname, 0, weights), self.noise(ctx, tag),
                                    y, self.N, M, self.K, self.N, _rlx.ACT[self.act], ctx.ws.splitk,
                                    ctx.ws.splitk.numel(), ctx.stream)
        return Tensor(y, M, self.N, 1, grad_key=(ctx, self.name, tag), act=self.act)

    def backward(self, ctx, x, y, need_dx=True, weights=None, t0=0, nt=None, need_dw=True, overlap=False):
        p, M = self.params, x.rows
        dz = y.grad
        if self.act is not None and not y.grad_is_dz:
            ctx.lib.act_backward(dz, y.data, M * self.N, _rlx.ACT[self.act], ctx.stream)
        lower = x.act if need_dx else None
        g = (lambda n: p.g(n)) if need_dw else (lambda n: None)
        ctx.lib.noisy_dense_backward(x.data, self.K, p.w(self.wmname, 0, weights), p.w(self.wsname, 0, weights), dz,
                                     self.N, self.noise(ctx, y.grad_key[2]), g(self.wmname), g(self.wsname),
                                     g(self.bmname), g(self.bsname), x.ensure_grad() if need_dx else None, self.K, M,
                                     self.K, self.N, _rlx.ACT[lower], ctx.ws.splitk, ctx.ws.splitk.numel(),
                                     ctx.stream)
        if need_dx:
            x.grad_is_dz = lower is not None


class BatchNorm(Layer):
    MOMENTUM, EPSILON = 0.99, 1e-3
    TRACKED_TAG = "train"

    def __init__(self, params, name, channels, activation=None):
        self.name, self.C, self.act, self.T, self.params = name, channels, activation, 1, params
        self.gname, self.bname = name + "/gamma", name + "/beta"
        self.mname, self.vname = name + "/moving_mean", name + "/moving_variance"
        params.add_group([(self.gname, (channels,)), (self.bname, (channels,)), (self.mname, (channels,)),
                          (self.vname, (channels,))], 1)

    def initialize(self, rng):
        self.params.w(self.gname).fill_(1.0)
        self.params.w(self.vname).fill_(1.0)

    def _saved(self, ctx, tag):
        return (ctx.buffer(self.name + "/batch_mean", (self.C,), tag=tag),
                ctx.buffer(self.name + "/batch_variance", (self.C,), tag=tag))

    def forward(self, ctx, x, tag="", weights=None, t0=0, nt=None, pair=False):
        assert not pair and x.towers == 1 and x.cols == self.C and x.act is None, (self.name, x.towers, x.cols, x.act)
        p, M = self.params, x.rows
        training = bool(getattr(ctx, "bn_training", False))
        y = ctx.buffer(self.name, (1, M, self.C), tag=tag)
        mean, var = self._saved(ctx, tag) if training else (None, None)
        ctx.lib.bn_forward(x.data, p.w(self.gname, 0, weights), p.w(self.bname, 0, weights),
                           p.w(self.mname, 0, weights), p.w(self.vname, 0, weights), M, self.C, self.EPSILON,
                           int(training), _rlx.ACT[self.act], y, mean, var, ctx.stream)
        out = Tensor(y, M, self.C, 1, grad_key=(ctx, self.name, tag), act=self.act)
        out.bn_saved = (mean, var)
        return out

    def backward(self, ctx, x, y, need_dx=True, weights=None, t0=0, nt=None, need_dw=True, overlap=False):
        mean, var = y.bn_saved
        if mean is None:
            raise ValueError("%s: backward through a batch-norm pass that ran on the moving statistics" % self.name)
        p, M = self.params, x.rows
        own = self.act if (self.act is not None and not y.grad_is_dz) else None
        ctx.lib.bn_backward(y.grad, y.data if own else None, x.data, p.w(self.gname, 0, weights), mean, var, M, self.C,
                            self.EPSILON, _rlx.ACT[own], x.ensure_grad(), p.g(self.gname) if need_dw else None,
                            p.g(self.bname) if need_dw else None, ctx.stream)
        x.grad_is_dz = False

    def commit(self, ctx):
        p = self.params
        mean, var = self._saved(ctx, self.TRACKED_TAG)
        ctx.lib.bn_update_moving(p.w(self.mname), p.w(self.vname), mean, var, self.C, self.MOMENTUM, ctx.stream)


class Conv2d(Layer):

    def __init__(self, params, name, in_hwc, filters, kernel, stride, activation=None, towers=1):
        self.name, self.T, self.act, self.params = name, towers, activation, params
        self.H, self.W, self.C = in_hwc
        self.KH = self.KW = kernel
        self.S, self.Co = stride, filters
        self.OH = (self.H - kernel) // stride + 1
        self.OW = (self.W - kernel) // stride + 1
        self.K = kernel * kernel * self.C
        self.kname, self.bname = name + "/kernel", name + "/bias"
        params.add_group([(self.kname, (self.K, filters)), (self.bname, (filters,))], towers)

    @property
    def out_hwc(self):
        return (self.OH, self.OW, self.Co)

    def initialize(self, rng):
        fan_in, fan_out = self.K, self.KH * self.KW * self.Co
        for t in range(self.T):
            w = xavier_uniform(rng, fan_in, fan_out, (self.K, self.Co))
            self.params.w(self.kname, t).copy_(torch.from_numpy(w))

    def _tables(self, ctx, B):
        key = ("convtab", self.name, B)
        if key not in ctx.cache:
            rb = torch.empty(B * self.OH * self.OW, dtype=torch.int32, device=ctx.device)
            ko = torch.empty(self.K, dtype=torch.int32, device=ctx.device)
            ctx.lib.conv_tables(rb, ko, B, self.H, self.W, self.C, self.KH, self.KW, self.S, ctx.stream)
            ctx.cache[key] = (rb, ko)
        return ctx.cache[key]

    def forward(self, ctx, x, tag="", weights=None, t0=0, nt=None, pair=False):
        y, T, args, kw = self.forward_product(ctx, x, tag, weights, t0, nt, pair)
        _rlx.gemm(*args, **kw)
        return Tensor(y, x.rows, self.OH * self.OW * self.Co, T, grad_key=(ctx, self.name, tag), act=self.act)

    def forward_product(self, ctx, x, tag="", weights=None, t0=0, nt=None, pair=False):
        t0, T = self._range(t0, nt)
        B, p = x.rows, self.params
        wstride, bstride = p.stride(self.kname), p.stride(self.bname)
        if pair:
            assert self.T == 1 and weights is None
            T, wstride, bstride = 2, p.size, p.size
        assert x.cols == self.H * self.W * self.C, (self.name, x.cols)
        assert x.towers in (0, T)
        M = B * self.OH * self.OW
        rb, ko = self._tables(ctx, B)
        y = ctx.buffer(self.name, (T, M, self.Co), tag=tag)
# ... 363 lines not shown
        y3 = ctx.buffer(b.name, (T, M3, b.Co), tag=tag)
        stream = ctx.stream
        args = (x.data, x.tower_stride(), p.w(a.kname, t0_, weights), ws2, p.w(a.bname, t0_, weights), bs2,
                p.w(b.kname, t0_, weights), ws3, p.w(b.bname, t0_, weights), bs3, y2, M2 * a.Co, y3, M3 * b.Co, B, T,
                _rlx.ACT[a.act], groups, stream)
        if not _fused_operands_aligned(args):
            return None
        run = lambda: ctx.lib.conv23_forward(*args)
        if _rlx.GEMM_HOOK is not None:
            d2, d3 = _rlx.GemmDesc(), _rlx.GemmDesc()
            d2.M, d2.N, d2.K, d2.batch = M2, a.Co, a.K, T
            d3.M, d3.N, d3.K, d3.batch = M3, b.Co, b.K, T
            _rlx._record((d2, d3), run)
        run()
        return [Tensor(y2, B, a.OH * a.OW * a.Co, T, grad_key=(ctx, a.name, tag), act=a.act),
                Tensor(y3, B, b.OH * b.OW * b.Co, T, grad_key=(ctx, b.name, tag), act=b.act)]

    def _fused_conv_triple(self, ctx, i, x, tag, weights, t0, nt, pair):
        if not (FUSE_CONV_PAIR and FUSE_CONV_FIRST) or i + 2 >= len(self.layers):
            return None
        f, a, b = self.layers[i], self.layers[i + 1], self.layers[i + 2]
        if not all(isinstance(l, Conv2d) for l in (f, a, b)) or not x.u8 or not (f.act == a.act == b.act) or \
                not (f.T == a.T == b.T):
            return None
        t0_, T = f._range(t0, nt)
        p = f.params
        if pair:
            if f.T != 1 or weights is not None:
                return None
            T = 2
        stride = (lambda name: p.size) if pair else p.stride
        lib = ctx.lib
        if x.towers not in (0, T) or f.out_hwc != (a.H, a.W, a.C) or a.out_hwc != (b.H, b.W, b.C) or \
                x.data.data_ptr() % 16 or x.tower_stride() % 16 or \
                not lib.conv123_forward_supported(f.H, f.W, f.C, f.KH, f.S, f.Co) or \
                not lib.conv23_forward_supported(a.H, a.W, a.C, a.KH, a.S, a.Co, b.KH, b.S, b.Co):
            return None
        B = x.rows
        M1, M2, M3 = B * f.OH * f.OW, B * a.OH * a.OW, B * b.OH * b.OW
        groups = _tiled_wave_groups(M2, a.Co, T)
        if groups not in (2, 4) or _tiled_wave_groups(M3, b.Co, T) != groups:
            return None
        groups = CONV_FORWARD_WAVE_GROUPS or groups
        y1, T1, gargs, gkw = f.forward_product(ctx, x, tag, weights, t0, nt, pair)
        assert T1 == T
        d1 = _rlx.gemm(*gargs, launch=False, **gkw)
        q = (ctypes.c_int * 8)()
        lib.gemm_describe(ctypes.byref(d1), q)
        fast, bm, bn, kw, splits, kchunk, ring, thin = list(q)
        if not fast or ring or thin or kw != 1:
            return None
        if (bm, bn) not in ((64, 64), (128, 32)):
            return None
        if splits == 1:
            chunks = 1
        elif splits == 3 and kchunk == 96:
            chunks = 3
        else:
            return None
        chunks = CONV1_CHUNKS or chunks
        y2 = ctx.buffer(a.name, (T, M2, a.Co), tag=tag)
        y3 = ctx.buffer(b.name, (T, M3, b.Co), tag=tag)
        w = lambda l: p.w(l.kname, t0_, weights)
        bi = lambda l: p.w(l.bname, t0_, weights)
        args = (x.data, x.tower_stride(), float(x.div), w(f), stride(f.kname), bi(f), stride(f.bname), y1, M1 * f.Co,
                w(a), stride(a.kname), bi(a), stride(a.bname), w(b), stride(b.kname), bi(b), stride(b.bname),
                y2, M2 * a.Co, y3, M3 * b.Co, B, T, _rlx.ACT[f.act], groups, chunks, ctx.stream)
        if not _fused_operands_aligned(args[3:]):
            return None
        run = lambda: lib.conv123_forward(*args)
        if _rlx.GEMM_HOOK is not None:
            d2, d3 = _rlx.GemmDesc(), _rlx.GemmDesc()
            d2.M, d2.N, d2.K, d2.batch = M2, a.Co, a.K, T
            d3.M, d3.N, d3.K, d3.batch = M3, b.Co, b.K, T
            _rlx._record((d1, d2, d3), run)
        run()
        return [Tensor(y, B, l.OH * l.OW * l.Co, T, grad_key=(ctx, l.name, tag), act=l.act)
                for y, l in ((y1, f), (y2, a), (y3, b))]

    def _fused_conv_input_grads(self, ctx, acts, i, weights, t0, nt, kw, need_dx_below):
        b, a = self.layers[i], self.layers[i - 1]
        if not FUSE_CONV_INPUT_GRADS or not (isinstance(a, Conv2d) and isinstance(b, Conv2d)) or ctx.overlap or \
                not need_dx_below or a.T != b.T or a.direct_input_grad() or b.direct_input_grad():
            return False
        y3, x2, x1 = acts[i + 1], acts[i], acts[i - 1]
        t0_, T = b._range(t0, nt)
        B, p, lib = x2.rows, b.params, ctx.lib
        if x2.towers != T or x1.towers != T or x1.u8 or x2.act != x1.act or a.out_hwc != (b.H, b.W, b.C) or \
                2 * B * T < FUSE_CONV_INPUT_GRADS_MIN_WORKGROUPS or \
                not lib.conv32_input_grad_supported(a.H, a.W, a.C, a.KH, a.S, a.Co, b.KH, b.S, b.Co):
            return False
        M3, M2, M1 = B * b.OH * b.OW, B * a.OH * a.OW, B * a.H * a.W
        dz3 = y3.grad
        dz2, dz1 = x2.ensure_grad(), x1.ensure_grad()
        descs = []
        for l, M, dz in ((b, M3, dz3), (a, M2, dz2)):
            dcol = ctx.buffer(l.name + "/dcol", (T, M, l.K))
            d = _rlx.gemm(M, l.K, l.Co, dz, p.w(l.kname, t0_, weights), dcol, b_strides=(1, l.Co), batch=T,
                          a_batch_stride=M * l.Co, b_batch_stride=p.stride(l.kname), c_batch_stride=M * l.K,
                          workspace=ctx.ws.splitk, launch=False)
            q = (ctypes.c_int * 8)()
            lib.gemm_describe(ctypes.byref(d), q)
            fast, bm, bn, kwg, splits, kchunk, ring, thin = list(q)
            if not (fast and ring and not thin and kwg == 1 and splits == 1):
                return False
            descs.append(d)
        if b.act is not None and not y3.grad_is_dz:
            lib.act_backward(dz3, y3.data, dz3.numel(), _rlx.ACT[b.act], ctx.stream)
            y3.grad_is_dz = True
        args = (dz3, M3 * b.Co, p.w(b.kname, t0_, weights), p.stride(b.kname), x2.data, M2 * a.Co, dz2, M2 * a.Co,
                p.w(a.kname, t0_, weights), p.stride(a.kname), x1.data, M1 * a.C, dz1, M1 * a.C, B, T,
                _rlx.ACT[x2.act], ctx.stream)
        per, ctx.per_tail = ctx.per_tail, None
        if per is not None and 2 * B * T + 1 <= PER_RIDER_MAX_WORKGROUPS:
            pd = _rlx.per_update_desc(per)
            run = lambda: lib.conv32_input_grad_per_update(*args[:-1], ctypes.byref(pd), args[-1])
        else:
            ctx.per_tail = per
            run = lambda: lib.conv32_input_grad(*args)
        _rlx._record(tuple(descs), run)
        run()
        x2.grad_is_dz, x1.grad_is_dz = x2.act is not None, x1.act is not None
        if kw.get("need_dw", True):
            for l, x, y in ((b, x2, y3), (a, x1, x2)):
                l.backward(ctx, x, y, need_dx=False, weights=weights, t0=t0, nt=nt, **kw)
        return True

    def backward(self, ctx, acts, need_input_grad=False, weights=None, t0=0, nt=None, need_dw=True,
                 layers=None):
        lo, hi = layers if layers is not None else (0, len(self.layers))
        mine = need_dw and ctx.begin_deferring()
        try:
            later = [] if (MULTI_DW and need_dw and ctx.deferred is not None and not ctx.overlap and
                           sum(isinstance(self.layers[i], Conv2d) for i in range(lo, hi)) >= 2) else None
            collect = [] if (CONV_DW_ONE_LAUNCH and need_dw and later is None and ctx.deferred is not None and
                             not ctx.overlap) else None
            i = hi
            while i > lo:
                i -= 1
                kw = {"overlap": True} if need_dw else {"need_dw": False}
                if collect is not None and isinstance(self.layers[i], Conv2d):
                    kw["dw_collect"] = collect
                if i - 1 >= lo and later is None and \
                        self._fused_conv_input_grads(ctx, acts, i, weights, t0, nt, kw, i - 1 > 0 or need_input_grad):
                    i -= 1
                    continue
                if later is not None and isinstance(self.layers[i], Conv2d):
                    kw["dw_later"] = later
                self.layers[i].backward(ctx, acts[i], acts[i + 1], need_dx=(i > 0 or need_input_grad),
                                        weights=weights, t0=t0, nt=nt, **kw)
            while collect:
                group = sorted(collect[:3], key=lambda e: (not e[0].x_is_u8, -e[0].H))
                collect = collect[3:]
                _rlx.conv_dw_multi([it for it, _ in group], [j for _, j in group], ctx.stream)
                for _, j in group:
                    ctx.commit_deferred(j, reserved=True)
            while later:
                group, later = later[:3], later[3:]
                _rlx.gemm_multi([d for d, _ in group], [j for _, j in group])
                for _, j in group:
                    ctx.commit_deferred(j, reserved=True)
            ctx.join()
        finally:
            if mine:
                ctx.flush_deferred()


class AdamState:

    def __init__(self, params, lr, beta1=0.9, beta2=0.99, epsilon=1e-4):
        dev = params.weights.device
        self.params, self.lr, self.beta1, self.beta2, self.eps = params, lr, beta1, beta2, epsilon
        self.m = torch.empty_like(params.weights)
        self.v = torch.empty_like(params.weights)
        self.state = torch.empty(2, dtype=torch.float32, device=dev)
        self.ticket = torch.zeros(_rlx.ADAM_TICKET_WORDS, dtype=torch.int32, device=dev)
        self.one_launch = True
        _rlx.lib().adam_init(self.m, self.v, params.size, self.state, beta1, beta2, _rlx.current_stream())

    def step(self, grad_scale=1.0, lr=None, norm_out=None, workspace=None, acc=None, grads=None, mix_target=None,
             mix_rate=0.0):
        p = self.params
        lr = self.lr if lr is None else lr
        g = p.grads if grads is None else grads
        if self.one_launch:
            _rlx.lib().adam_tf1_step(p.weights, g, self.m, self.v, p.size, lr, self.beta1, self.beta2, self.eps,
                                     self.state, grad_scale, norm_out, workspace if norm_out is not None else None,
                                     workspace.numel() if norm_out is not None else 0,
                                     acc[0] if acc else None, acc[1] if acc else None, int(acc[2]) if acc else 0,
                                     mix_target, float(mix_rate), self.ticket, _rlx.current_stream())
            return
        if mix_target is not None:
            raise ValueError("the two-launch Adam path does not fuse the target update")
        if norm_out is not None:
            _rlx.lib().adam_tf1_norm(p.weights, g, self.m, self.v, p.size, lr, self.beta1,
                                     self.beta2, self.eps, self.state, grad_scale, norm_out, workspace,
                                     workspace.numel(), acc[0] if acc else None, acc[1] if acc else None,
                                     int(acc[2]) if acc else 0, _rlx.current_stream())
        else:
            _rlx.lib().adam_tf1(p.weights, g, self.m, self.v, p.size, lr, self.beta1, self.beta2,
                                self.eps, self.state, grad_scale, _rlx.current_stream())
```

### coach_amd/nn/networks.py

```python
import numpy as np
import torch

from .. import _rlx
from ..architectures.head_parameters import DuelingQHeadParameters
from . import graph as G

IMAGE_EMBEDDER = {"Medium": [(32, 8, 4), (64, 4, 2), (64, 3, 1)], "Shallow": [(32, 3, 1)]}
VECTOR_EMBEDDER = {"Medium": [256], "Shallow": [128], "Empty": []}
FC_MIDDLEWARE = {"Medium": [512], "Shallow": [64], "Empty": []}


def build_torso(params, prefix, obs_shape, activation, towers, embedder="Medium", middleware="Medium", noisy=False):
    layers = []
    Dense = G.NoisyDense if noisy else G.Dense
    if len(obs_shape) == 3:
        hwc = tuple(obs_shape)
        convs = IMAGE_EMBEDDER[embedder] if isinstance(embedder, str) else embedder
        for i, (f, k, s) in enumerate(convs):
            c = G.Conv2d(params, "%s/embedder/conv%d" % (prefix, i), hwc, f, k, s, activation, towers)
            layers.append(c)
            hwc = c.out_hwc
        feat = hwc[0] * hwc[1] * hwc[2]
    else:
        feat = int(obs_shape[0])
# ... 124 lines not shown
        fused_heads = self.pi_head.N <= G.SMALL_N and B * self.pi_head.N <= 1024
        if fused_heads and self.HEADS_FORWARD_WITH_TORSO and self.torso.layers[-1].N > G.SMALL_N:
            acts, (v, logits) = self.torso.forward(ctx, self.obs_tensor(obs, B), tag=tag,
                                                   row_heads=[(self.v_head, 0, value_out), (self.pi_head, 1)])
        else:
            acts = self.torso.forward(ctx, self.obs_tensor(obs, B), tag=tag)
            mid = acts[-1]
            if fused_heads:
                v, logits = G.small_dense_forward_multi(ctx, [(self.v_head, mid.tower_view(0)), (self.pi_head, mid.tower_view(1))], tag=tag)
            else:
                v = self.v_head.forward(ctx, mid.tower_view(0), tag=tag)
                logits = self.pi_head.forward(ctx, mid.tower_view(1), tag=tag)
            value_out.copy_(v.data.view(-1))
        self.lib.softmax_categorical_sample(logits.data, self.A, uniforms, B, self.A, probs_out, self.A, actions, ctx.stream)

    def policy_mean_std(self, obs, B, use_target=False, tag="act", out_mean=None, out_std=None):
        w = self.target if use_target else None
        acts = self.torso.forward(self.ctx, self.obs_tensor(obs, B), tag=tag, weights=w, t0=1, nt=1)
        mean = self.pi_head.forward(self.ctx, acts[-1], tag=tag, weights=w).data.view(B, self.A)
        std = out_std if out_std is not None else self.ctx.buffer("policy_std", (B, self.A), tag=tag)
        ls = self.params.w("main/ppo_head/policy_log_std", 0, w)
        self.lib.exp_rows(ls, std, B, self.A, self.ctx.stream)
        if out_mean is not None:
            out_mean.copy_(mean)
            mean = out_mean
        return mean, std

    def values(self, obs, B, tag="val", out=None):
        if self.HEADS_FORWARD_WITH_TORSO and self.torso.layers[-1].N > G.SMALL_N:
            acts, (v,) = self.torso.forward(self.ctx, self.obs_tensor(obs, B), tag=tag, t0=0, nt=1,
                                            row_heads=[(self.v_head, 0)])
        else:
            acts = self.torso.forward(self.ctx, self.obs_tensor(obs, B), tag=tag, t0=0, nt=1)
            v = self.v_head.forward(self.ctx, acts[-1], tag=tag)
        if out is not None:
            out.copy_(v.data.view(-1))
            return out
        return v.data.view(-1)

    def late_gradient_offset(self):
        return self.params.entries[self.torso.layers[self._split_layer()].kname][0]

    def _split_layer(self):
        from .graph import Conv2d
        for i, l in enumerate(self.torso.layers):
            if not isinstance(l, Conv2d):
                return i
        return 0

    def set_clip_rescaler(self, value):
        if self._clip_scale_dev is None:
            self._clip_scale_dev = torch.ones(1, dtype=torch.float32, device=self.device)
        if self._clip_scale_value != float(value):
            self._clip_scale_dev.fill_(float(value))
            self._clip_scale_value = float(value)

    def forward_backward(self, obs, B, actions, advantages, value_targets, old_probs,
                         clip_rescaler=1.0, ratio_out=None, clipped_out=None, stop_after_dense=False):
        ctx = self.ctx
        clip_dev = self._clip_scale_dev if clip_rescaler is None else None
        if clip_rescaler is None:
            assert clip_dev is not None, "set_clip_rescaler first"
            clip_rescaler = 1.0
        fused_heads = self.pi_head.N <= G.SMALL_N and B * self.pi_head.N <= 1024
        heads_with_torso = fused_heads and self.HEADS_FORWARD_WITH_TORSO and self.torso.layers[-1].N > G.SMALL_N
        discrete_fused = heads_with_torso and not self.continuous and self.HEADS_LOSS_BACKWARD_ONE_LAUNCH
        if (self.FC_HEADS_ONE_LAUNCH or (self.HEADS_ROW_LOCAL and B <= 256)) and discrete_fused:
            acts = self.torso.forward(ctx, self.obs_tensor(obs, B), tag="train", skip_last=True)
            if self.HEADS_ROW_LOCAL and B <= 256 and not self.FC_HEADS_ONE_LAUNCH and len(acts) == len(self.torso.layers):
                res = G.ppo_fc_rows(ctx, self.torso.layers[-1], acts[-1], self.v_head, self.pi_head, value_targets, actions,
                                    advantages, old_probs, self.A, self.clip_eps * clip_rescaler, clip_dev, self.beta,
                                    self.scalars, ratio_out, clipped_out, self.status, tag="train",
                                    tail_now=stop_after_dense)
                if res is not None:
                    acts.append(res[0])
                    return self._backward_torso(acts, stop_after_dense)
            if self.FC_HEADS_ONE_LAUNCH and len(acts) == len(self.torso.layers) and \
                    G.ppo_fc_heads_supported(ctx, self.torso.layers[-1], acts[-1], self.v_head, self.pi_head):
                mid, v, logits = G.ppo_fc_heads(ctx, self.torso.layers[-1], acts[-1], self.v_head, self.pi_head, value_targets,
                                                actions, advantages, old_probs, self.A, self.clip_eps * clip_rescaler, clip_dev,
                                                self.beta, self.scalars, ratio_out, clipped_out, self.status, tag="train")
                acts.append(mid)
                return self._backward_torso(acts, stop_after_dense)
            last = self.torso.layers[-1]
            if heads_with_torso:
                y, (v, logits) = last.forward(ctx, acts[-1], tag="train", row_heads=[(self.v_head, 0), (self.pi_head, 1)])
            else:
                y = last.forward(ctx, acts[-1], tag="train")
            acts.append(y)
        elif heads_with_torso:
            acts, (v, logits) = self.torso.forward(ctx, self.obs_tensor(obs, B), tag="train",
                                                   row_heads=[(self.v_head, 0), (self.pi_head, 1)])
        else:
            acts = self.torso.forward(ctx, self.obs_tensor(obs, B), tag="train")
        mid = acts[-1]
        mid.ensure_grad()
        xv, xp = mid.tower(0), mid.tower(1)
        if heads_with_torso:
            pass
        elif fused_heads:
            v, logits = G.small_dense_forward_multi(ctx, [(self.v_head, xv), (self.pi_head, xp)], tag="train")
        else:
            v = self.v_head.forward(ctx, xv, tag="train")
            logits = self.pi_head.forward(ctx, xp, tag="train")
        one_launch = fused_heads and not self.continuous and B <= 256 and self.HEADS_LOSS_BACKWARD_ONE_LAUNCH
        if one_launch:
            G.ppo_heads_loss_backward(ctx, (self.v_head, xv, v), (self.pi_head, xp, logits), value_targets, actions,
                                      advantages, old_probs, self.A, self.clip_eps * clip_rescaler, clip_dev, self.beta,
                                      self.scalars, ratio_out, clipped_out, self.status)
        dv, dlogits = v.ensure_grad(), logits.ensure_grad()
        if one_launch:
            pass
        elif not self.continuous:
            self.lib.ppo_discrete_value_losses(logits.data, self.A, actions, advantages, old_probs, self.A, B,
                                               self.A, self.clip_eps * clip_rescaler, self.beta, 1.0, dlogits,
                                               self.A, self.scalars[0:4], ratio_out, clipped_out, self.status,
                                               v.data, value_targets, dv, self.scalars[4:5], clip_dev, ctx.stream)
        else:
            self.lib.regression_loss(v.data, 1, value_targets, 1, None, B, 1, 0, 1.0, 1.0, dv, 1,
                                     self.scalars[4:5], ctx.stream)
        if self.continuous:
            old_mean, old_std = old_probs
            self.lib.ppo_continuous_loss(logits.data, self.A, self.params.w("main/ppo_head/policy_log_std"),
                                         actions, advantages, old_mean, old_std, self.A, B, self.A,
                                         self.clip_eps * clip_rescaler, self.beta, 1.0, dlogits, self.A,
                                         self.params.g("main/ppo_head/policy_log_std"), self.scalars[0:4],
                                         ratio_out, clipped_out, clip_dev, ctx.stream)

        if one_launch:
            pass
        elif fused_heads:
            G.small_dense_backward_multi(ctx, [(self.v_head, xv, v), (self.pi_head, xp, logits)])
        else:
            self.v_head.backward(ctx, xv, v)
            self.pi_head.backward(ctx, xp, logits)
        mid.grad_is_dz = xv.grad_is_dz and xp.grad_is_dz
        self._backward_torso(acts, stop_after_dense)

    def _backward_torso(self, acts, stop_after_dense):
        ctx = self.ctx
        if stop_after_dense:
            k = self._split_layer()
            self.torso.backward(ctx, acts, layers=(k, len(self.torso.layers)))
            self._resume = (acts, k)
        else:
            self.torso.backward(ctx, acts)
        ctx.flush_ppo_tail()

    def backward_rest(self):
        acts, k = self._resume
        if k > 0:
            self.torso.backward(self.ctx, acts, layers=(0, k))

    def finish_update(self, grad_scale=1.0, signal_acc=None):
        self.apply_gradients(grad_scale, with_norm=True,
                             acc=(self.scalars, signal_acc, 6) if signal_acc is not None else None)

    def train_minibatch(self, obs, B, actions, advantages, value_targets, old_probs,
                        clip_rescaler=1.0, grad_scale=1.0, ratio_out=None, clipped_out=None):
        self.forward_backward(obs, B, actions, advantages, value_targets, old_probs, clip_rescaler,
                              ratio_out, clipped_out)
        self.finish_update(grad_scale)
        return self.scalars


def dqn_net_kwargs(np_, seed):
    head = np_.heads_parameters[0]
    return dict(activation=np_.activation_function, embedder=np_.embedder_scheme, middleware=np_.middleware_scheme,
                learning_rate=np_.learning_rate, adam_beta1=np_.adam_optimizer_beta1,
                adam_beta2=np_.adam_optimizer_beta2, optimizer_epsilon=np_.optimizer_epsilon,
                replace_mse_with_huber_loss=np_.replace_mse_with_huber_loss, seed=seed,
                dueling=isinstance(head, DuelingQHeadParameters), head_activation=head.activation_function,
                head_gradient_rescale=head.rescale_gradient_from_head_by_factor,
                clip_gradients=getattr(np_, "clip_gradients", None))


class DQNNet(_NetBase):
    HEAD_FORWARD_WITH_TORSO = True
    HEAD_LOSS_BACKWARD_ONE_LAUNCH = True
    FUSED_MLP = True
    FUSED_ACT = True

    def __init__(self, device, obs_shape, n_actions, activation="relu", embedder="Medium",
                 middleware="Medium", learning_rate=2.5e-4, adam_beta1=0.9, adam_beta2=0.99,
                 optimizer_epsilon=1e-4, replace_mse_with_huber_loss=True, seed=0, dueling=False,
                 head_activation="relu", head_gradient_rescale=1.0, clip_gradients=None, noisy=False):
        self.obs_shape, self.image, self.A = tuple(obs_shape), len(obs_shape) == 3, n_actions
        self.huber = replace_mse_with_huber_loss
        self.dueling = dueling
        self.noisy = bool(noisy)
        self.head_gradient_rescale = float(head_gradient_rescale)
        self.clip_gradients = clip_gradients
        self.params = G.FlatParams()
        self.torso, feat = build_torso(self.params, "main", obs_shape, activation, 1, embedder, middleware,
                                       noisy=self.noisy)
        if dueling and self.noisy:
            hn = "main/dueling_q_values_head"
            self.v_fc = G.NoisyDense(self.params, hn + "/state_value/fc1", feat, 512, head_activation)
            self.a_fc = G.NoisyDense(self.params, hn + "/action_advantage/fc1", feat, 512, head_activation)
            self.v_out = G.NoisyDense(self.params, hn + "/state_value/fc2", 512, 1, None)
            self.a_out = G.NoisyDense(self.params, hn + "/action_advantage/fc2", 512, n_actions, None)
            self.modules = [self.torso, self.v_fc, self.a_fc, self.v_out, self.a_out]
        elif dueling:
            hn = "main/dueling_q_values_head"
            self.stream_fc = G.Dense(self.params, hn + "/fc1", feat, 512, head_activation, 2)
            self.v_out = G.Dense(self.params, hn + "/state_value/fc2", 512, 1, None, 1)
            self.a_out = G.Dense(self.params, hn + "/action_advantage/fc2", 512, n_actions, None, 1)
            self.modules = [self.torso, self.stream_fc, self.v_out, self.a_out]
        else:
            self.q_head = self._q_head_layer(feat, n_actions)
            self.modules = [self.torso, self.q_head]
        self._finish(device, seed, learning_rate, adam_beta1, adam_beta2, optimizer_epsilon)
        self.loss = torch.zeros(1, dtype=torch.float32, device=device)
        self._noisy_setup()
        self._fused = self._fused_mlp_setup()
        self._act = self._act_setup()

    def _q_head_layer(self, feat, units):
        return (G.NoisyDense if self.noisy else G.Dense)(self.params, "main/q_head/dense", feat, units, None, 1)

    def _noisy_setup(self):
        self.noisy_layers = [l for m in self.modules for l in (m.layers if isinstance(m, G.Sequential) else [m])
                             if isinstance(l, G.NoisyDense)]
        for i, l in enumerate(self.noisy_layers):
            l.index = i
        if len(self.noisy_layers) > _rlx.NOISY_MAX_LAYERS:
            raise ValueError("a noisy network may have at most %d dense layers (this one has %d)"
                             % (_rlx.NOISY_MAX_LAYERS, len(self.noisy_layers)))
        self.noise_seed, self.noise_rank = 0, 0
        self.noise_counters = torch.zeros(max(1, len(self.noisy_layers)) * _rlx.NOISY_PASSES, dtype=torch.int64,
                                          device=self.device) if self.noisy else None

    def sample_noise(self, tag, noise_pass):
        if not self.noisy:
            return
        key = ("noisy_layers", tag)
        arr = self.ctx.cache.get(key)
        if arr is None:
            arr = (_rlx.NoisyLayer * len(self.noisy_layers))()
            for q, l in zip(arr, self.noisy_layers):
                q.f, q.f64, q.K, q.N, q.layer = l.noise(self.ctx, tag).data_ptr(), None, l.K, l.N, l.index
            self.ctx.cache[key] = arr
        import ctypes
        self.lib.noisy_sample(ctypes.byref(arr), len(arr), self.noise_counters, _rlx.NOISY_PASS[noise_pass],
                              self.noise_seed, self.noise_rank, self.ctx.stream)

    def _small_mlp(self):
        ls = self.torso.layers
        if self.image or self.dueling or len(ls) != 2 or \
                any(not isinstance(l, G.Dense) or l.act != "relu" or l.T != 1 for l in ls):
            return None
        offs = tuple(self.params.entries[n][0] for l in (ls[0], ls[1], self.q_head) for n in (l.kname, l.bname))
        return (ls[0].K, ls[0].N, ls[1].N), offs

    def _fused_mlp_setup(self):
        mlp = self._small_mlp() if self.FUSED_MLP else None
        if mlp is None or self.head_gradient_rescale != 1.0 or self.clip_gradients:
            return None
        dims, offs = mlp
        if not self.lib.rlx_mlp_dqn_supported(1, *dims, self.A):
            return None
        import ctypes
        n = ctypes.c_longlong()
        self.lib.mlp_dqn_workspace_floats(dims[1], dims[2], self.A, ctypes.byref(n))
        return dict(dims=dims, ws=torch.zeros(n.value, dtype=torch.float32, device=self.device),
                    sync=torch.zeros(4, dtype=torch.int32, device=self.device), offs=offs)

    def _act_setup(self):
        mlp = self._small_mlp() if self.FUSED_ACT else None
        if mlp is None or getattr(self.q_head, "act", None) is not None:
            return None
        return dict(dims=mlp[0], offs=mlp[1])

    def can_act_fused(self, n_env):
        a = self._act
        return a is not None and bool(self.lib.rlx_mlp_q_act_supported(int(n_env), *a["dims"], self.A))

    def q_act(self, states, n_env, explore_u, random_act, tie_rand, epsilon, q_out, actions, use_target=False):
        a = self._act
        w = self.target if use_target else self.params.weights
        self.lib.mlp_q_act(w, *a["offs"], states, int(n_env), *a["dims"], self.A, explore_u, random_act, tie_rand,
                           float(epsilon), q_out, actions, self.ctx.stream)

    def _fused_learn(self, obs, next_obs, B, actions, rewards, game_overs, discount, w, td_errors, double_dqn,
                     grad_scale):
        f = self._fused
        d = _rlx.MlpDqnDesc()
        d.weights, d.target_weights = self.params.weights.data_ptr(), self.target.data_ptr()
        d.adam_m, d.adam_v, d.adam_state = self.adam.m.data_ptr(), self.adam.v.data_ptr(), self.adam.state.data_ptr()
        d.states, d.next_states = obs.data_ptr(), next_obs.data_ptr()
        d.actions, d.rewards, d.game_overs = actions.data_ptr(), rewards.data_ptr(), game_overs.data_ptr()
        d.importance_weights = None if w is None else w.data_ptr()
        d.workspace, d.workspace_floats, d.sync_words = f["ws"].data_ptr(), f["ws"].numel(), f["sync"].data_ptr()
        d.loss_out, d.norm_out = self.loss.data_ptr(), self.norm.data_ptr()
        d.td_errors = None if td_errors is None else td_errors.data_ptr()
        d.status = self.status.data_ptr()
        d.off_w1, d.off_b1, d.off_w2, d.off_b2, d.off_w3, d.off_b3 = f["offs"]
        d.discount = float(discount)
        d.batch, (d.obs_dim, d.h1, d.h2), d.n_actions = int(B), f["dims"], self.A
        d.huber, d.double_dqn = int(self.huber), int(bool(double_dqn))
        a = self.adam
        d.learning_rate, d.beta1, d.beta2, d.epsilon, d.grad_scale = a.lr, a.beta1, a.beta2, a.eps, float(grad_scale)
        import ctypes
        self.lib.mlp_dqn_update(ctypes.byref(d), self.ctx.stream)
        return self.loss

    def _dueling_forward(self, feat, B, tag, weights=None, train=False):
        ctx = self.ctx
        if self.noisy:
# ... 706 lines not shown
```

### include/rlx.h

```cpp
#ifndef RLX_H
#define RLX_H

#include <stddef.h>
#include <stdint.h>

#ifdef __cplusplus
extern "C" {
#endif

typedef enum rlx_status {
    RLX_OK = 0,
    RLX_ERR_INVALID_ARG = -1,
    RLX_ERR_HIP = -2,
    RLX_ERR_UNSUPPORTED = -3
} rlx_status;

#define RLX_ABI_VERSION 11
int rlx_abi_version(void);
const char *rlx_last_error(void);
const char *rlx_build_arch(void);
int rlx_device_count(int *count_host);
int rlx_stream_sync(void *stream);
int rlx_event_create(void **event_host);
int rlx_event_destroy(void *event);
// ... 272 lines not shown
    const float *colsum_partials;
    float *C;
    float *colsum_out;
    long long ldc, c_batch_stride, colsum_batch_stride;
    int M, N, batch, splits;
    int n_fold;
} rlx_splitk_job;
int rlx_gemm_defer(const rlx_gemm_desc *desc_host, rlx_splitk_job *job_host, void *stream);
int rlx_gemm_pair_defer(const rlx_gemm_desc *weight_grad, const rlx_gemm_desc *input_grad,
                        rlx_splitk_job *weight_grad_job_host, void *stream);
int rlx_splitk_reduce_jobs(const rlx_splitk_job *jobs_host, int n_jobs, void *stream);
int rlx_gemm_multi_defer(const rlx_gemm_desc *descs, int n, rlx_splitk_job *jobs, void *stream);
int rlx_gemm_debug_stamps(void *buffer, long long capacity_u64);
int rlx_gemm_debug_calls(long long *out_host, int max_calls, int *n_calls_host);
int rlx_colsum(const float *x, int M, int N, long long ld, float *out, int accumulate,
               float *workspace, long long workspace_floats, void *stream);
int rlx_act_backward(float *dy, const float *y, long long n, int kind, void *stream);
int rlx_conv_tables(int *rowbase, int *koff, int batch, int H, int W, int C, int KH, int KW,
                    int stride, void *stream);
int rlx_col2im(const float *dcol, float *dx, const float *x_out, int deriv_kind, int batch, int H,
               int W, int C, int KH, int KW, int stride, void *stream);

int rlx_bn_forward(const float *x, const float *gamma, const float *beta, const float *moving_mean,
                   const float *moving_var, int batch, int channels, double epsilon, int training, int activation,
                   float *y, float *save_mean, float *save_var, void *stream);
int rlx_bn_backward(const float *dy, const float *y, const float *x, const float *gamma, const float *save_mean,
                    const float *save_var, int batch, int channels, double epsilon, int activation, float *dx,
                    float *dgamma, float *dbeta, void *stream);
int rlx_bn_update_moving(float *moving_mean, float *moving_var, const float *batch_mean, const float *batch_var,
                         int channels, double momentum, void *stream);

typedef struct rlx_mlp_dqn_desc {
    float *weights; const float *target_weights; float *adam_m; float *adam_v; float *adam_state;
    const float *states; const float *next_states; const int *actions; const float *rewards;
    const unsigned char *game_overs; const double *importance_weights;
    float *workspace; unsigned int *sync_words;
    float *loss_out; float *norm_out; double *td_errors; int *status;
    long long workspace_floats;
    long long off_w1, off_b1, off_w2, off_b2, off_w3, off_b3;
    double discount;
    int batch, obs_dim, h1, h2, n_actions;
    int huber, double_dqn;
    float learning_rate, beta1, beta2, epsilon, grad_scale;
} rlx_mlp_dqn_desc;
int rlx_mlp_dqn_supported(int batch, int obs_dim, int h1, int h2, int n_actions);
int rlx_mlp_dqn_workspace_floats(int h1, int h2, int n_actions, long long *floats_host);
int rlx_mlp_dqn_update(const rlx_mlp_dqn_desc *desc_host, void *stream);
int rlx_mlp_q_act_supported(int n_env, int obs_dim, int h1, int h2, int n_actions);
int rlx_mlp_q_act(const float *weights, long long off_w1, long long off_b1, long long off_w2, long long off_b2,
                  long long off_w3, long long off_b3, const float *states, int n_env, int obs_dim, int h1, int h2,
                  int n_actions, const double *explore_uniforms, const int *random_actions,
                  const double *tie_break_uniforms, double epsilon, float *q_out, int *actions, void *stream);

int rlx_dense_small_forward(const float *x, long long x_tower_stride, const float *w,
                            long long w_tower_stride, const float *bias, long long bias_tower_stride,
                            float *y, long long y_tower_stride, int towers, int M, int K, int N,
                            int activation, void *stream);
int rlx_dense_small_backward(const float *x, long long x_tower_stride, const float *w,
                             long long w_tower_stride, const float *dy, long long dy_tower_stride,
                             const float *y, long long y_tower_stride, float *dw,
                             long long dw_tower_stride, float *db, long long db_tower_stride, float *dx,
                             long long dx_tower_stride, int towers, int M, int K, int N, int activation,
                             int lower_activation, void *stream);

typedef struct rlx_small_dense_problem {
    const float *x; long long x_tower_stride;
    const float *w; long long w_tower_stride;
    const float *bias; long long bias_tower_stride;
    float *y; long long y_tower_stride;
    const float *dy; long long dy_tower_stride;
    float *dw; long long dw_tower_stride;
    float *db; long long db_tower_stride;
    float *dx; long long dx_tower_stride;
    int towers, M, K, N, activation, lower_activation;
} rlx_small_dense_problem;
int rlx_dqn_head_loss_backward(const rlx_small_dense_problem *q_head, const float *q_online, long long ld_q,
                               const float *q_next_target, const float *q_next_selector, long long ld_next,
                               const int *actions, const float *rewards, const unsigned char *game_overs,
                               const double *importance_weights, double discount, int batch, int n_actions, int huber,
                               float grad_scale, double *td_errors, float *loss_scalar, int *status, void *stream);
int rlx_dense_small_forward_multi(const rlx_small_dense_problem *problems_host, int n_problems, void *stream);
int rlx_dense_small_backward_multi(const rlx_small_dense_problem *problems_host, int n_problems, void *stream);
int rlx_ppo_heads_loss_backward(const rlx_small_dense_problem *value_head, const rlx_small_dense_problem *policy_head,
                                const float *values, const float *value_targets, const float *logits,
                                const int *actions, const float *advantages, const float *old_probs, long long ld_old,
                                int batch, float clip_epsilon, const float *clip_scale, float beta_entropy,
                                float grad_scale, float *scalars, float *likelihood_ratio,
                                float *clipped_likelihood_ratio, int *status, void *stream);
typedef struct rlx_ppo_rows_desc {
    rlx_small_dense_problem value_head, policy_head;
    const float *value_targets;
    const int *actions;
    const float *advantages;
    const float *old_probs; long long ld_old;
    const float *clip_scale;
    float clip_epsilon, beta_entropy, grad_scale;
    int batch;
    float *row_terms;
    float *scalars;
    float *likelihood_ratio, *clipped_likelihood_ratio;
    int *status;
} rlx_ppo_rows_desc;
int rlx_ppo_fc_rows_supported(const rlx_gemm_desc *fc, int n_actions);
int rlx_ppo_fc_rows(const rlx_gemm_desc *fc, const rlx_ppo_rows_desc *rows, void *stream);
int rlx_ppo_heads_tail(const rlx_ppo_rows_desc *rows, void *stream);
int rlx_splitk_reduce_jobs_ppo_tail(const rlx_splitk_job *jobs_host, int n_jobs, const rlx_ppo_rows_desc *rows, void *stream);
int rlx_splitk_reduce_jobs_per_update(const rlx_splitk_job *jobs_host, int n_jobs, double *sum_tree, double *min_tree,
                                      double *max_tree, int capacity, const int *idx, const double *td_errors, int n,
                                      double alpha, double epsilon, double *max_priority, int *status, void *stream);

int rlx_regression_loss(const float *out, long long ld_out, const float *target,
                        long long ld_target, const float *importance_weights, int batch, int dim,
                        int kind, float loss_weight, float grad_scale, float *grad,
                        long long ld_grad, float *loss_scalar, void *stream);
int rlx_softmax(const float *logits, long long ld, int batch, int n, float *probs,
                long long ld_out, void *stream);
int rlx_ppo_discrete_loss(const float *logits, long long ld, const int *actions,
                          const float *advantages, const float *old_probs, long long ld_old,
                          int batch, int n_actions, float clip_epsilon, float beta_entropy,
                          float grad_scale, float *dlogits, long long ld_grad, float *scalars,
                          float *likelihood_ratio, float *clipped_likelihood_ratio, int *status,
                          const float *clip_scale, void *stream);

int rlx_ppo_discrete_value_losses(const float *logits, long long ld, const int *actions,
                                  const float *advantages, const float *old_probs, long long ld_old,
                                  int batch, int n_actions, float clip_epsilon, float beta_entropy,
                                  float grad_scale, float *dlogits, long long ld_grad, float *scalars,
                                  float *likelihood_ratio, float *clipped_likelihood_ratio, int *status,
                                  const float *values, const float *value_targets, float *dvalues,
                                  float *value_loss_scalar, const float *clip_scale, void *stream);

int rlx_ppo_continuous_loss(const float *mean, long long ld, const float *log_std, const float *actions,
                            const float *advantages, const float *old_mean, const float *old_std,
                            long long ld_old, int batch, int action_dim, float clip_epsilon,
                            float beta_entropy, float grad_scale, float *dmean, long long ld_grad,
                            float *dlog_std, float *scalars, float *likelihood_ratio,
                            float *clipped_likelihood_ratio, const float *clip_scale, void *stream);

int rlx_adam_init(float *m, float *v, long long n, float *state, float beta1, float beta2,
                  void *stream);
int rlx_adam_tf1(float *weights, const float *grads, float *m, float *v, long long n,
                 float learning_rate, float beta1, float beta2, float epsilon, float *state,
                 float grad_scale, void *stream);
int rlx_adam_tf1_norm(float *weights, const float *grads, float *m, float *v, long long n,
                      float learning_rate, float beta1, float beta2, float epsilon, float *state,
                      float grad_scale, float *norm_out, float *workspace, long long workspace_floats,
                      const float *acc_src, float *acc_dst, int n_acc, void *stream);
#define RLX_ADAM_TICKET_WORDS 1056
int rlx_adam_tf1_step(float *weights, const float *grads, float *m, float *v, long long n, float learning_rate,
                      float beta1, float beta2, float epsilon, float *state, float grad_scale, float *norm_out,
                      float *workspace, long long workspace_floats, const float *acc_src, float *acc_dst, int n_acc,
                      float *target, double mix_rate, unsigned int *ticket, void *stream);
int rlx_adam_norm_in_kernel(int on);
int rlx_mix_weights(float *target, const float *online, long long n, double rate,
                    void *stream);
int rlx_global_norm(const float *x, long long n, float *norm_out, float *workspace,
                    long long workspace_floats, void *stream);

int rlx_clip_by_global_norm(float *grads, long long n, const float *global_norm, float clip_norm,
                            void *stream);
int rlx_clip_by_value(float *grads, long long n, float clip_value, void *stream);

int rlx_copy_2d(const float *src, long long src_ld, float *dst, long long dst_ld, int rows, int cols,
                float scale, void *stream);
int rlx_exp_rows(const float *log_std, float *out, int batch, int action_dim,
                 void *stream);
int rlx_axpby(float *out, float a, const float *x, float b, const float *y, long long n,
              void *stream);
int rlx_min_pair(const float *q1, const float *q2, float *out_min, float *grad1, float *grad2,
                 float grad_scale, int n, void *stream);
int rlx_sac_min_targets(const float *q1, const float *q2, const float *sampled_logprob, float grad_scale, int n,
                        float *out_min, float *value_targets, float *grad1, float *grad2, void *stream);
int rlx_select_rows(const unsigned char *mask, const void *if_set, const void *if_clear, void *out,
                    int n, long long row_bytes, void *stream);
int rlx_sac_policy_head(const float *mu_logsig, long long ld, const double *standard_normals, int batch,
                        int action_dim, float *out_mean, float *out_log_std, float *out_raw_actions,
                        float *out_actions, float *out_logprob, void *stream);
int rlx_sac_policy_head_backward(const float *mu_logsig, long long ld, const double *standard_normals,
                                 int batch, int action_dim, float logprob_mean_weight,
                                 const float *action_weights, float action_weight_scale,
                                 float *d_mu_logsig, long long ld_grad, int accumulate, void *stream);

int rlx_categorical_sample(const float *probs, long long ld, const double *uniforms, int n_env,
                           int n_actions, int *actions, void *stream);
int rlx_softmax_categorical_sample(const float *logits, long long ld, const double *uniforms, int n_env,
                                   int n_actions, float *probs_out, long long ld_out, int *actions, void *stream);
int rlx_argmax_rows(const float *values, long long ld, int n_rows, int n_cols, int *out,
                    void *stream);
int rlx_egreedy(const float *q_values, long long ld, const double *explore_uniforms,
                const int *random_actions, const double *tie_break_uniforms, double epsilon,
                int n_env, int n_actions, int *actions, void *stream);
int rlx_gaussian_action(const float *mean, const float *std_per_dim, const float *std_per_sample,
                        const double *standard_normals, const float *action_low,
                        const float *action_high, int n_env, int action_dim, float *actions,
                        void *stream);

int rlx_qr_dqn_head_loss(const float *theta, long long ld_theta, const float *theta_next_target, long long ld_next,
                         const int *actions, const float *rewards, const unsigned char *game_overs, double discount,
                         float kappa, int n_atoms, int n_actions, int batch, float grad_scale, float *dtheta,
                         long long ld_dtheta, float *row_partials, unsigned int *ticket, float *loss_scalar,
                         int *status, float *targets_out, float *tau_out, int *target_actions_out, void *stream);
int rlx_quantile_egreedy(const float *quantiles, long long ld, int n_atoms, const double *explore_uniforms,
                         const int *random_actions, const double *tie_break_uniforms, double epsilon, int n_env,
                         int n_actions, double *q_out, int *actions, void *stream);

int rlx_c51_head_loss(const float *logits, long long ld_logits, const float *logits_next_target, long long ld_next,
                      const double *z, const int *actions, const float *rewards, const unsigned char *game_overs,
                      double discount, int n_atoms, int n_actions, int batch, float grad_scale, float *dlogits,
                      long long ld_dlogits, double *per_errors, float *row_partials, unsigned int *ticket,
                      float *loss_scalar, int *status, float *m_out, int *target_actions_out, float *action_losses_out,
                      void *stream);
int rlx_categorical_egreedy(const float *logits, long long ld, const double *z, int n_atoms,
                            const double *explore_uniforms, const int *random_actions,
                            const double *tie_break_uniforms, double epsilon, int n_env, int n_actions, double *q_out,
                            int *actions, void *stream);

int rlx_synth_env_reset(int kind, void *obs, int *episode, int *step, int n_env, int obs_elems,
                        unsigned int seed, unsigned int env_id0, void *stream);
int rlx_synth_env_step(int kind, void *next_obs, void *reset_obs, float *reward,
                       unsigned char *game_over, int *episode, int *step, int n_env, int obs_elems,
                       int episode_len, unsigned int seed, unsigned int env_id0, void *stream);

int rlx_synth_env_step_lengths(int kind, void *next_obs, void *reset_obs, float *reward,
                               unsigned char *game_over, int *episode, int *step, int n_env, int obs_elems,
                               const int *episode_len_per_env, unsigned int seed, unsigned int env_id0,
                               void *stream);

int rlx_normal_fill(double *out, const long long *events, int n_events, int stream0, int n_streams, int n,
                    unsigned int seed, unsigned int rank, double scale, void *stream);

#define RLX_NOISY_PASSES 4
#define RLX_NOISY_MAX_LAYERS 8
typedef struct rlx_noisy_layer {
    float *f;
    double *f64;
    int K, N;
    int layer;
} rlx_noisy_layer;
int rlx_noisy_sample(const rlx_noisy_layer *layers_host, int n_layers, long long *counters, int pass,
                     unsigned int seed, unsigned int rank, void *stream);
int rlx_noisy_dense_workspace_floats(int M, int K, int N, long long *floats_host);
int rlx_noisy_dense_forward(const float *x, long long ldx, const float *weight_mean, const float *weight_stddev,
                            const float *bias_mean, const float *bias_stddev, const float *noise, float *y,
                            long long ldy, int M, int K, int N, int activation, float *workspace,
                            long long workspace_floats, void *stream);
int rlx_noisy_dense_backward(const float *x, long long ldx, const float *weight_mean, const float *weight_stddev,
                             const float *dz, long long lddz, const float *noise, float *d_weight_mean,
                             float *d_weight_stddev, float *d_bias_mean, float *d_bias_stddev, float *dx,
                             long long lddx, int M, int K, int N, int lower_activation, float *workspace,
                             long long workspace_floats, void *stream);
int rlx_quantile_argmax(const float *quantiles, long long ld, int n_atoms, int n_env, int n_actions, double *q_out,
                        int *actions, void *stream);
int rlx_categorical_argmax(const float *logits, long long ld, const double *z, int n_atoms, int n_env, int n_actions,
                           double *q_out, int *actions, void *stream);

int rlx_bootstrapped_dqn_head_loss(const float *q_online, long long ld_q, const float *q_next_target,
                                   const float *q_next_online, long long ld_next, const int *actions,
                                   const float *rewards, const unsigned char *game_overs, const uint32_t *masks,
                                   double discount, int batch, int n_heads, int n_actions, int huber, float grad_scale,
                                   float *dq, long long ld_dq, float *partials, unsigned int *ticket, float *loss_scalar,
                                   int *status, float *head_losses, float *td_targets, int *target_actions,
                                   void *stream);
int rlx_bootstrapped_egreedy(const float *q_values, long long ld, int n_heads, const int *selected_head, int vote,
                             const double *explore_uniforms, const int *random_actions,
                             const double *tie_break_uniforms, double epsilon, int n_env, int n_actions,
                             float *values_out, int *actions, void *stream);
int rlx_ucb_egreedy(const float *q_values, long long ld, int n_heads, float lamb, int use_std,
                    const double *explore_uniforms, const int *random_actions, const double *tie_break_uniforms,
                    double epsilon, int n_env, int n_actions, float *values_out, float *std_out, int *actions,
                    void *stream);

int rlx_naf_head_loss(const float *v, long long ld_v, const float *mu_unscaled, long long ld_mu, const float *l_vector,
                      long long ld_l, const float *output_scale, const float *actions, long long ld_act,
                      const float *v_next, long long ld_vnext, const float *rewards, const unsigned char *game_overs,
                      double discount, int batch, int action_dim, int huber, float grad_scale, float *dv,
                      long long ld_dv, float *dmu_unscaled, long long ld_dmu, float *dl_vector, long long ld_dl,
                      float *partials, unsigned int *ticket, float *loss_scalar, float *td_targets_out, float *q_out,
                      float *adv_out, void *stream);
int rlx_naf_head_forward(const float *v, long long ld_v, const float *mu_unscaled, long long ld_mu,
                         const float *l_vector, long long ld_l, const float *output_scale, const float *actions,
                         long long ld_act, int batch, int action_dim, float *mu_out, float *q_out, float *adv_out,
                         float *l_out, void *stream);

int rlx_mixed_target_head_loss(const float *q_online, long long ld_q, const float *q_target_cur,
                               const float *q_next_target, const float *q_next_selector, long long ld_next,
                               const int *actions, const float *rewards, const unsigned char *game_overs,
                               const double *total_returns, double discount, double pal_alpha, int persistent,
                               double mixing_rate, int batch, int n_actions, int huber, float grad_scale, float *dq,
                               long long ld_dq, float *td_targets, long long ld_targets, float *loss_scalar, int *status,
                               void *stream);

int rlx_cartpole_reset(double *state, float *obs, int *episode, int *steps, int n_env, unsigned int seed,
                       unsigned int env_id0, int next_episode, void *stream);
int rlx_cartpole_step(const int *action, double *state, int *episode, int *steps, float *next_obs, float *reset_obs,
                      double *next_state64, float *reward, unsigned char *game_over, int n_env,
                      int max_episode_steps, unsigned int seed, unsigned int env_id0, int *status, void *stream);
int rlx_libm_sincos(const double *x, double *sin_out, double *cos_out, int n, int *status, void *stream);


typedef struct rlx_mlp3 {
    long long off_w1, off_b1, off_w2, off_b2, off_w3, off_b3;
    long long tower_stride1, tower_stride2, tower_stride3;
    int d_in, h1, h2, d_out;
} rlx_mlp3;
typedef struct rlx_fused_net {
    float *weights, *target_weights, *adam_m, *adam_v, *adam_state, *grads, *norm_out;
    unsigned int *ticket;
    float learning_rate, beta1, beta2, epsilon, grad_scale, mix_rate;
} rlx_fused_net;
typedef struct rlx_td3_fused_desc {
    rlx_fused_net actor, critic;
    rlx_mlp3 actor_mlp, critic_mlp;
    const float *obs, *next_obs, *actions, *rewards;
    const unsigned char *game_overs;
    const double *noise;
    const float *action_low, *action_high;
    double noise_clip, discount, clip_low, clip_high;
    int use_non_zero_discount_for_terminal_states, has_clip;
    float actor_scale;
    int batch, obs_dim, act_dim;
    float *workspace; long long workspace_floats;
    float *td_targets, *q_min, *loss, *neg_action_grad;
} rlx_td3_fused_desc;
int rlx_td3_fused_supported(const rlx_td3_fused_desc *desc_host);
int rlx_fused_phase_stamps(int enable);
int rlx_td3_fused_workspace_floats(const rlx_td3_fused_desc *desc_host, long long *floats_host);
int rlx_td3_fused_critic_update(const rlx_td3_fused_desc *desc_host, int write_grads, void *stream);
int rlx_td3_fused_actor_update(const rlx_td3_fused_desc *desc_host, int write_grads, void *stream);


typedef struct rlx_sac_fused_desc {
    rlx_fused_net policy, q, v;
    rlx_mlp3 policy_mlp, v_mlp;
    long long q_off_obs_w, q_off_obs_b, q_off_act_w, q_off_act_b, q_off_fc_w, q_off_fc_b, q_off_out_w, q_off_out_b;
    long long q_stride_obs, q_stride_act, q_stride_fc, q_stride_out;
    const float *obs, *next_obs, *actions, *rewards;
    const unsigned char *game_overs;
    const double *normals;
    double discount;
    int resample_noise_per_pass, batch, obs_dim, act_dim, q_hidden, reserved;
    float *workspace; long long workspace_floats;
    float *value_targets, *log_target, *td_targets, *dq_da, *q_loss, *v_loss;
} rlx_sac_fused_desc;
int rlx_sac_fused_supported(const rlx_sac_fused_desc *desc_host);
int rlx_sac_fused_workspace_floats(const rlx_sac_fused_desc *desc_host, long long *floats_host);
int rlx_sac_fused_update(const rlx_sac_fused_desc *desc_host, int write_grads, void *stream);

int rlx_conv_dw_u8_supported(int B, int H, int W, int C, int KH, int KW, int S, int filters, int towers);
int rlx_conv_dw_u8_workspace_floats(int B, int H, int W, int C, int KH, int KW, int S, int filters, int towers,
                                    long long *floats_host);
int rlx_conv_dw_u8(const unsigned char *frames, float a_div, const float *dz, long long dz_tower_stride, int B, int H, int W,
                   int C, int KH, int KW, int S, int filters, int towers, float *dw, long long dw_tower_stride, float *db,
                   long long db_tower_stride, float *workspace, long long workspace_floats, rlx_splitk_job *job_host,
                   void *stream);
int rlx_conv_dw_u8_stamps(long long *device_words5);

int rlx_conv_dw_f32_supported(int B, int H, int W, int C, int KH, int KW, int S, int filters, int towers);
int rlx_conv_dw_f32_workspace_floats(int B, int H, int W, int C, int KH, int KW, int S, int filters, int towers,
                                     long long *floats_host);
int rlx_conv_dw_f32(const float *x, long long x_tower_stride, const float *dz, long long dz_tower_stride, int B, int H, int W,
                    int C, int KH, int KW, int S, int filters, int towers, float *dw, long long dw_tower_stride, float *db,
                    long long db_tower_stride, float *workspace, long long workspace_floats, rlx_splitk_job *job_host,
                    void *stream);
int rlx_conv_dw_f32_stamps(long long *device_words4);

typedef struct rlx_conv_dw_item {
    const void *x; long long x_tower_stride;
    int x_is_u8; float a_div;
    const float *dz; long long dz_tower_stride;
    int B, H, W, C, KH, KW, S, filters, towers;
    float *dw; long long dw_tower_stride;
    float *db; long long db_tower_stride;
    float *workspace; long long workspace_floats;
} rlx_conv_dw_item;
int rlx_conv_dw_multi(const rlx_conv_dw_item *items_host, rlx_splitk_job *jobs_host, int n_items, void *stream);
int rlx_conv_dw_passes(int passes);
int rlx_conv_dw_pairs_per_workgroup(int pairs);

typedef struct rlx_ppo_fc_heads_desc {
    const float *x; long long x_tower_stride;
    const float *weights; long long weight_tower_stride;
    const float *bias; long long bias_tower_stride;
    const float *value_w, *value_b, *policy_w, *policy_b;
    const float *value_targets, *advantages, *old_probs; long long ld_old;
    const int *actions;
    const float *clip_scale;
    float clip_epsilon, beta_entropy, grad_scale;
    int batch, in_features, units, n_actions, activation;
    float *h, *dz, *values, *logits, *dvalues, *dlogits;
    float *d_value_w, *d_value_b, *d_policy_w, *d_policy_b;
    float *scalars, *likelihood_ratio, *clipped_likelihood_ratio;
    int *status;
    float *workspace; long long workspace_floats;
    unsigned int *tickets;
} rlx_ppo_fc_heads_desc;
int rlx_ppo_fc_heads_supported(int batch, int in_features, int units, int n_actions);
int rlx_ppo_fc_heads_workspace(int units, long long *floats_host, long long *ticket_words_host);
int rlx_ppo_fc_heads(const rlx_ppo_fc_heads_desc *desc_host, void *stream);
int rlx_ppo_fc_heads_stamps(int enable);

int rlx_bitflip_reset(unsigned char *bits, float *obs, int *episode, int *steps, int n_env, int bit_length,
                      int mean_zero, unsigned int seed, unsigned int env_id0, int next_episode, void *stream);
int rlx_bitflip_step(const int *action, unsigned char *bits, int *episode, int *steps, float *next_obs,
                     float *reset_obs, float *reward, unsigned char *game_over, int n_env, int bit_length,
                     int max_steps, int mean_zero, unsigned int seed, unsigned int env_id0, int *status,
                     void *stream);
#define RLX_HER_EUCLIDEAN 0
#define RLX_HER_MANHATTAN 2
int rlx_her_relabel_episode(float *obs, float *next_obs, void *action, float *reward, unsigned char *game_over,
                            const int *selected_steps, long long first_step, int length, int n_base, int k, int env,
                            int n_env, long long ring_steps, int obs_dim, int goal_at, int achieved_at, int goal_dim,
                            int action_row_bytes, int metric, double threshold, float goal_reaching_reward,
                            float default_reward, int *status, void *stream);

int rlx_chain_reset(int *state, int *steps, float *obs, int n_env, int chain_length, int start_state, int therm,
                    void *stream);
int rlx_chain_step(const int *action, int *state, int *steps, float *next_obs, float *reset_obs, float *reward,
                   unsigned char *game_over, int n_env, int chain_length, int start_state, int max_steps, int therm,
                   float left_state_reward, float right_state_reward, int *status, void *stream);

#define RLX_PG_TOTAL_RETURN 0
#define RLX_PG_FUTURE_RETURN 1
#define RLX_PG_FUTURE_RETURN_NORMALIZED_BY_EPISODE 2
#define RLX_PG_FUTURE_RETURN_NORMALIZED_BY_TIMESTEP 3
#define RLX_PG_STATUS_EPISODE_TOO_LONG 2
int rlx_pg_episode_window(const float *rewards, int length, int start, double discount, int rescaler,
                          double *mean_over_episodes, double *episodes_seen, int max_length, double *returns_out,
                          double *rescaled_out, float *advantages_out, double *stats_out, int *status, void *stream);
int rlx_pg_head_loss(const float *logits, long long ld, const int *actions, const float *advantages, float beta_entropy,
                     int rows, int true_rows, int n_actions, float *dlogits, long long ld_dlogits, float *scalars,
                     int *status, void *stream);
int rlx_action_entropy(const float *probs, long long ld, int n_env, int n_actions, float *entropy_out, void *stream);

#define RLX_A3C_A_VALUE 5
#define RLX_A3C_GAE 8
#define RLX_A3C_TARGETS_GIVEN -1
#define RLX_A3C_STATUS_NO_BOOTSTRAP_ROW 2
int rlx_a3c_window_loss(const float *V, long long ld_v, const float *logits, long long ld, const int *actions,
                        const float *rewards, const unsigned char *game_over, int T, int rows, int n_actions,
                        double discount, double gae_lambda, int rescaler, int estimate_state_value_using_gae,
                        float beta_entropy, float v_loss_weight, double *targets_out, double *advantages_out, float *dV,
                        long long ld_dv, float *dlogits, long long ld_dlogits, float *scalars, int *status,
                        void *stream);

#define RLX_NSTEPQ_N_STEP 0
#define RLX_NSTEPQ_ONE_STEP 1
#define RLX_NSTEPQ_TARGETS_GIVEN -1
#define RLX_NSTEPQ_STATUS_BAD_ACTION 1
#define RLX_NSTEPQ_STATUS_NO_TARGET_ROWS 2
int rlx_nstep_q_window_loss(const float *q_online, long long ld_q, const float *q_target, long long ld_t, int rows_t,
                            const int *actions, const float *rewards, const unsigned char *game_over, int T,
                            int n_actions, double discount, int horizon, int huber, float *targets, float *td_targets,
                            long long ld_tt, float *dq, long long ld_dq, float *scalars, int *status, void *stream);

#define RLX_ACER_TRUST_REGION 1
#define RLX_ACER_TARGETS_GIVEN 2
#define RLX_ACER_STATUS_BAD_ACTION 1
#define RLX_ACER_STATUS_NO_BOOTSTRAP_ROW 2
int rlx_acer_window_loss(const float *q, long long ld_q, const float *logits, long long ld_logits, int rows,
                         const float *avg_logits, long long ld_avg_logits, const float *mu, long long ld_mu,
                         const int *actions, const float *rewards, const unsigned char *game_over, int T, int n_actions,
                         double discount, float truncation, float max_kl, float beta_entropy, float q_loss_weight,
                         int mode, float *V, float *rho, long long ld_rho, float *rho_i, float *avg_policy,
                         long long ld_avg_policy, float *q_retrace, float *bootstrap_value, float *td_targets,
                         long long ld_tt, float *dq, long long ld_dq, float *dlogits, long long ld_dlogits,
                         float *scalars, int *status, void *stream);

#ifdef __cplusplus
}
#endif
#endif
```

Baseline: 38760 env-steps/s.

## Overlap early Adam blocks for dense parameters with the conv weight-gradient kernel

Splits the Adam step into early blocks, which cover the dense torso parameters whose gradients are already final, and late blocks. The early blocks ride as extra workgroups inside the conv dW multi-kernel launch, so part of the optimizer update runs alongside the conv backward instead of after it. A late launch then finishes the remaining blocks and the global norm from per-block partials. The cost is added complexity, a forced four-pass conv dW configuration when Adam rides along, and register-held block limits on parameter count.

```diff
diff --git a/coach_amd/_rlx.py b/coach_amd/_rlx.py
--- a/coach_amd/_rlx.py
+++ b/coach_amd/_rlx.py
@@ -254,7 +254,7 @@
     "rlx_small_dense_problem": "SmallDenseProblem", "rlx_mlp_dqn_desc": "MlpDqnDesc", "rlx_mlp3": "Mlp3",
     "rlx_fused_net": "FusedNet", "rlx_td3_fused_desc": "Td3FusedDesc", "rlx_sac_fused_desc": "SacFusedDesc",
     "rlx_ppo_fc_heads_desc": "PpoFcHeadsDesc", "rlx_ppo_rows_desc": "PpoRowsDesc", "rlx_observe_desc": "ObserveDesc",
-    "rlx_signal_source": "SignalSource",
+    "rlx_signal_source": "SignalSource", "rlx_adam_split_desc": "AdamSplitDesc",
 }
 _TEXT = header_text()
 STRUCTS = parse_structs(_TEXT, STRUCT_NAMES)
@@ -267,6 +267,7 @@
 Td3FusedDesc, SacFusedDesc = STRUCTS["rlx_td3_fused_desc"], STRUCTS["rlx_sac_fused_desc"]
 PpoFcHeadsDesc, PpoRowsDesc = STRUCTS["rlx_ppo_fc_heads_desc"], STRUCTS["rlx_ppo_rows_desc"]
 ObserveDesc, SignalSource = STRUCTS["rlx_observe_desc"], STRUCTS["rlx_signal_source"]
+AdamSplitDesc = STRUCTS["rlx_adam_split_desc"]
 
 
 class SplitkJob(STRUCTS["rlx_splitk_job"]):
@@ -355,7 +356,7 @@
     return it
 
 
-def conv_dw_multi(items, jobs, stream=None):
+def conv_dw_multi(items, jobs, stream=None, adam=None):
     s = current_stream() if stream is None else stream
     n = len(items)
     arr = (ConvDwItem * n)(*items)
@@ -363,6 +364,12 @@
 
     def run():
         lib().conv_dw_multi(arr, jarr, n, s)
+    if adam is not None:
+        if GEMM_HOOK is not None:
+            raise RuntimeError("rlx_conv_dw_multi_adam applies an Adam step: it cannot be recorded for replay")
+        desc, riders, first = adam
+        lib().conv_dw_multi_adam(arr, jarr, n, ctypes.byref(desc), int(riders), int(bool(first)), s)
+        run = lambda: None
     if GEMM_HOOK is not None:
         descs = []
         for it in items:
diff --git a/coach_amd/agents/clipped_ppo_agent.py b/coach_amd/agents/clipped_ppo_agent.py
--- a/coach_amd/agents/clipped_ppo_agent.py
+++ b/coach_amd/agents/clipped_ppo_agent.py
@@ -76,6 +76,7 @@
     restarts_memory_on_reset = True
     FUSE_ACTING_LAUNCHES = True
     RECORD_WHILE_ACTING = True
+    ADAM_UNDER_CONV_DW = True
     DATASET_CHUNK = 2048
 
     def __init__(self, agent_parameters, environment, device=None, dist=None, use_graphs=None):
@@ -524,6 +525,7 @@
         return e
 
     def _minibatch_fb(self, m, clip_rescaler, stop_after_dense=False, i=0, epoch=None):
+        self._arm_early_adam(stop_after_dense)
         if epoch is not None:
             B = self.ap.network_wrappers["main"].batch_size
             sl = slice(i * B, i * B + m)
@@ -537,6 +539,14 @@
         self.networks["main"].forward_backward(obs, m, self.mb_action, self.mb_adv, self.mb_vtarget,
                                                old, clip_rescaler, self.mb_ratio, self.mb_clipped,
                                                stop_after_dense=stop_after_dense)
+
+    EARLY_ADAM_SCALE = 1.0
+
+    def _arm_early_adam(self, stop_after_dense=False):
+        net = self.networks["main"]
+        net.disarm_early_adam()
+        if self.ADAM_UNDER_CONV_DW and self.dist is None and not stop_after_dense and _rlx.GEMM_HOOK is None:
+            net.arm_early_adam(self.EARLY_ADAM_SCALE, prepare=not torch.cuda.is_current_stream_capturing())
 
     def _minibatch_finish(self, scale):
         net = self.networks["main"]
@@ -581,6 +591,9 @@
         n = len(order)
         self.networks["main"].set_clip_rescaler(float(alg.clipping_decay_schedule.current_value))
         clip = None
+        early = bool(self.ADAM_UNDER_CONV_DW and self.dist is None)
+        if early:
+            self.networks["main"].prepare_early_adam()
         scale = self.dist.grad_scale(netp.scale_down_gradients_by_number_of_workers_for_sync_training) \
             if self.dist else 1.0
         results = []
@@ -620,13 +633,13 @@
                         else:
                             reduced_fb(min(B, n - i * B), i, e)
                         self._minibatch_finish(scale)
-                self._run(("epoch", n, clip, scale, self.dist is not None and self.overlap_allreduce), epoch)
+                self._run(("epoch", n, clip, scale, self.dist is not None and self.overlap_allreduce, early), epoch)
                 results.append(self.scalar_acc / nmb)
                 continue
             for i in range(nmb):
                 m = min(B, n - i * B)
                 if self.dist is None:
-                    self._run(("mb", m, clip, scale, i), lambda: (self._minibatch_fb(m, clip, i=i),
+                    self._run(("mb", m, clip, scale, i, early), lambda: (self._minibatch_fb(m, clip, i=i),
                                                                   self._minibatch_finish(scale)))
                 elif in_graph:
                     self._run(("mb_dp", m, clip, scale, i, self.overlap_allreduce),
diff --git a/coach_amd/csrc/adam_block_body.hpp b/coach_amd/csrc/adam_block_body.hpp
--- /dev/null
+++ b/coach_amd/csrc/adam_block_body.hpp
@@ -0,0 +1,130 @@
+#pragma once
+#include "rlx_common.hpp"
+
+namespace rlx_adam {
+
+constexpr int kBlock = 256;
+constexpr int kNormIt = 4;
+
+struct Coef {
+    float alpha, omb1, omb2, eps, grad_scale, rate, one_minus_rate;
+};
+
+__device__ __forceinline__ Coef coef(const float b1p, const float b2p, float lr, float beta1, float beta2, float eps,
+                                     float grad_scale, float rate, float one_minus_rate) {
+    Coef c;
+    c.alpha = lr * sqrtf(1.f - b2p) / (1.f - b1p);
+    c.omb1 = 1.f - beta1;
+    c.omb2 = 1.f - beta2;
+    c.eps = eps;
+    c.grad_scale = grad_scale;
+    c.rate = rate;
+    c.one_minus_rate = one_minus_rate;
+    return c;
+}
+
+template <bool MIX, bool EXCHANGE>
+__device__ __forceinline__ float block_step(float *__restrict__ w, const float *__restrict__ g, float *__restrict__ m,
+                                            float *__restrict__ v, const long long n, const Coef c, float *sumsq_part,
+                                            float *__restrict__ target, const int vb, const int blocks, float *red) {
+    const long long stride = (long long)blocks * kBlock;
+    const long long n4 = n >> 2;
+    const long long i0 = (long long)vb * kBlock + threadIdx.x;
+    float4 gw[kNormIt], mw[kNormIt], vw[kNormIt], ww[kNormIt], tw[kNormIt];
+#pragma unroll
+    for (int it = 0; it < kNormIt; ++it) {
+        const long long i = i0 + it * stride;
+        if (i < n4) {
+            gw[it] = reinterpret_cast<const float4 *>(g)[i];
+            mw[it] = reinterpret_cast<float4 *>(m)[i];
+            vw[it] = reinterpret_cast<float4 *>(v)[i];
+            ww[it] = reinterpret_cast<float4 *>(w)[i];
+            if (MIX) tw[it] = reinterpret_cast<float4 *>(target)[i];
+        }
+    }
+    const long long it0 = (n4 << 2) + i0;
+    const bool has_tail = it0 < n;
+    const float gt = has_tail ? g[it0] : 0.f;
+    float ss = 0.f;
+#pragma unroll
+    for (int it = 0; it < kNormIt; ++it)
+        if (i0 + it * stride < n4) {
+            const float *gp = &gw[it].x;
+#pragma unroll
+            for (int k = 0; k < 4; ++k) ss += gp[k] * gp[k];
+        }
+    if (has_tail) ss += gt * gt;
+    red[threadIdx.x] = ss;
+    __syncthreads();
+    for (int d = kBlock >> 1; d > 0; d >>= 1) {
+        if (threadIdx.x < d) red[threadIdx.x] += red[threadIdx.x + d];
+        __syncthreads();
+    }
+    float old = 0.f;
+    if (threadIdx.x == 0) {
+        if (EXCHANGE) old = __hip_atomic_exchange(&sumsq_part[vb], red[0], __ATOMIC_RELAXED, __HIP_MEMORY_SCOPE_AGENT);
+        else __hip_atomic_store(&sumsq_part[vb], red[0], __ATOMIC_RELAXED, __HIP_MEMORY_SCOPE_AGENT);
+    }
+#pragma unroll
+    for (int it = 0; it < kNormIt; ++it) {
+        const long long i = i0 + it * stride;
+        if (i < n4) {
+            float *gp = &gw[it].x, *mp = &mw[it].x, *vp = &vw[it].x, *wp = &ww[it].x, *tp = &tw[it].x;
+#pragma unroll
+            for (int k = 0; k < 4; ++k) {
+                const float gr = gp[k] * c.grad_scale;
+                mp[k] += (gr - mp[k]) * c.omb1;
+                vp[k] += (gr * gr - vp[k]) * c.omb2;
+                wp[k] -= (mp[k] * c.alpha) / (sqrtf(vp[k]) + c.eps);
+                if (MIX) tp[k] = c.rate * wp[k] + c.one_minus_rate * tp[k];
+            }
+            reinterpret_cast<float4 *>(m)[i] = mw[it];
+            reinterpret_cast<float4 *>(v)[i] = vw[it];
+            reinterpret_cast<float4 *>(w)[i] = ww[it];
+            if (MIX) reinterpret_cast<float4 *>(target)[i] = tw[it];
+        }
+    }
+    if (has_tail) {
+        const float gr = gt * c.grad_scale;
+        m[it0] += (gr - m[it0]) * c.omb1;
+        v[it0] += (gr * gr - v[it0]) * c.omb2;
+        w[it0] -= (m[it0] * c.alpha) / (sqrtf(v[it0]) + c.eps);
+        if (MIX) target[it0] = c.rate * w[it0] + c.one_minus_rate * target[it0];
+    }
+    return old;
+}
+
+struct EarlyDev {
+    float *w;
+    const float *g;
+    float *m, *v;
+    long long n;
+    float lr, beta1, beta2, eps, grad_scale;
+    const float *state;
+    float *sumsq_part;
+    const int *early;
+    int n_early, blocks;
+};
+
+__device__ __forceinline__ void early_blocks(const EarlyDev &e, const int r, const int R, float *red) {
+    const Coef c = coef(e.state[0], e.state[1], e.lr, e.beta1, e.beta2, e.eps, e.grad_scale, 0.f, 0.f);
+    for (int k = r; k < e.n_early; k += R)
+        block_step<false, false>(e.w, e.g, e.m, e.v, e.n, c, e.sumsq_part, nullptr, e.early[k], e.blocks, red);
+}
+
+inline int early_dev(const rlx_adam_split_desc *d, EarlyDev *e, const char *who) {
+    RLX_REQUIRE(d && d->weights && d->grads && d->m && d->v && d->state && d->partials, "%s: null pointer", who);
+    RLX_REQUIRE(d->n > 0 && d->blocks >= 1 && (d->n >> 2) <= (long long)d->blocks * kBlock * kNormIt,
+                "%s: %lld parameters do not fit %d register-held blocks", who, d->n, d->blocks);
+    RLX_REQUIRE(d->n_early >= 0 && d->n_late >= 1 && d->n_early + d->n_late == d->blocks && d->late && (d->early || !d->n_early),
+                "%s: the early and late lists must name every one of the %d blocks once (%d + %d), late not empty", who,
+                d->blocks, d->n_early, d->n_late);
+    RLX_REQUIRE((((uintptr_t)d->weights | (uintptr_t)d->grads | (uintptr_t)d->m | (uintptr_t)d->v) & 15) == 0,
+                "%s: buffers must be 16-byte aligned", who);
+    e->w = d->weights; e->g = d->grads; e->m = d->m; e->v = d->v; e->n = d->n;
+    e->lr = d->learning_rate; e->beta1 = d->beta1; e->beta2 = d->beta2; e->eps = d->epsilon; e->grad_scale = d->grad_scale;
+    e->state = d->state; e->sumsq_part = d->partials; e->early = d->early; e->n_early = d->n_early; e->blocks = d->blocks;
+    return RLX_OK;
+}
+
+}
diff --git a/coach_amd/csrc/conv_dw_multi.hip b/coach_amd/csrc/conv_dw_multi.hip
--- a/coach_amd/csrc/conv_dw_multi.hip
+++ b/coach_amd/csrc/conv_dw_multi.hip
@@ -1,4 +1,7 @@
 #include "conv_dw_body.hpp"
+#pragma clang fp contract(off)
+#include "adam_block_body.hpp"
+#pragma clang fp contract(fast)
 
 namespace {
 
@@ -38,20 +41,48 @@
     }
 }
 
+__global__ void __launch_bounds__(kThreads)
+conv_dw_multi_adam_kernel(const MultiArgs m, const rlx_adam::EarlyDev e, const int riders, const int first) {
+    extern __shared__ __attribute__((aligned(16))) float smem[];
+    static_assert(kThreads == rlx_adam::kBlock, "a rider is one Adam block");
+    int bid = blockIdx.x;
+    if (first) {
+        if (bid < riders) {
+            rlx_adam::early_blocks(e, bid, riders, smem);
+            return;
+        }
+        bid -= riders;
+    }
+    if (bid < m.nb_u8) {
+        if (m.u8_half) conv_dw_u8_body_half(m.u8, bid, smem);
+        else conv_dw_u8_body_passes<4>(m.u8, bid, smem);
+        return;
+    }
+    bid -= m.nb_u8;
+#pragma unroll
+    for (int i = 0; i < 2; ++i) {
+        if (bid < m.nb_f[i]) {
+            if (m.kind[i] == 1) conv_dw_f32_body_two_pass<64, 3, 1, 9, 7, 4, 7>(m.f[i], bid, smem);
+            else conv_dw_f32_body_two_pass<32, 4, 2, 20, 9, 5, 9>(m.f[i], bid, smem);
+            return;
+        }
+        bid -= m.nb_f[i];
+    }
+    if (!first && bid < riders) rlx_adam::early_blocks(e, bid, riders, smem);
+}
+
 int g_passes = 2;
 int g_pairs_per_wg = 0;
-inline int pairs_per_wg(int B, int towers) {
-    if (g_passes <= 1) return 1;
+inline int pairs_per_wg(int B, int towers, int passes) {
+    if (passes <= 1) return 1;
     if (g_pairs_per_wg > 0) return g_pairs_per_wg;
     return towers * ((B + 1) / 2) >= 64 ? 2 : 1;
 }
 
-}
-
-extern "C" {
-
-int rlx_conv_dw_multi(const rlx_conv_dw_item *items, rlx_splitk_job *jobs, int n_items, void *stream) {
+int conv_dw_multi_impl(const rlx_conv_dw_item *items, rlx_splitk_job *jobs, int n_items, void *stream,
+                       const rlx_adam_split_desc *adam, int riders, int riders_first) {
     RLX_REQUIRE(items && jobs && n_items >= 1 && n_items <= 3, "rlx_conv_dw_multi: 1 .. 3 items");
+    const int passes = adam ? 4 : g_passes;
     int n_u8 = 0, n_f = 0;
     bool one = n_items >= 2;
     GeometryU8 gu;
@@ -66,7 +97,7 @@
             iu = &it; ju = i; ++n_u8;
         } else {
             one = n_f < 2 && geometry_f32(it.B, it.H, it.W, it.C, it.KH, it.KW, it.S, it.filters, it.towers, &gf[n_f < 2 ? n_f : 1],
-                                          pairs_per_wg(it.B, it.towers));
+                                          pairs_per_wg(it.B, it.towers, passes));
             if (n_f < 2) { fi[n_f] = &it; jf[n_f] = i; }
             ++n_f;
         }
@@ -83,7 +114,7 @@
                                   it.db_tower_stride, it.workspace, it.workspace_floats, &jobs[i], stream);
             if (rc != RLX_OK) return rc;
         }
-        return RLX_OK;
+        return adam ? rlx_adam_tf1_step_early(adam, riders, stream) : RLX_OK;
     }
     MultiArgs m;
     m.nb_u8 = m.nb_f[0] = m.nb_f[1] = 0;
@@ -125,7 +156,7 @@
         a.x = static_cast<const float *>(it.x); a.x_ts = it.x_tower_stride; a.dz = it.dz; a.dz_ts = it.dz_tower_stride;
         a.part = it.workspace; a.cpart = it.db ? it.workspace + (size_t)it.towers * g.splits * g.K * kN : nullptr;
         a.B = it.B; a.H = it.H; a.OH = g.OH; a.KH = it.KH; a.splits = g.splits; a.units = it.towers * g.splits;
-        a.ppw = pairs_per_wg(it.B, it.towers);
+        a.ppw = pairs_per_wg(it.B, it.towers, passes);
         a.stamps = nullptr;
         m.nb_f[k] = ((a.units + 7) / 8) * 8 * it.KH;
         m.kind[k] = g.kind;
@@ -144,23 +175,49 @@
                                     hipFuncAttributeMaxDynamicSharedMemorySize, 160 * 1024));
         RLX_HIP(hipFuncSetAttribute(reinterpret_cast<const void *>(conv_dw_multi_kernel<4>),
                                     hipFuncAttributeMaxDynamicSharedMemorySize, 160 * 1024));
+        RLX_HIP(hipFuncSetAttribute(reinterpret_cast<const void *>(conv_dw_multi_adam_kernel),
+                                    hipFuncAttributeMaxDynamicSharedMemorySize, 160 * 1024));
         configured = true;
     }
     const unsigned grid = m.nb_u8 + m.nb_f[0] + m.nb_f[1];
-    if (g_passes > 1) {
-        size_t lds2 = iu ? (m.u8_half ? lds_u8_half() : (g_passes == 4 ? lds_u8_passes<4>() : lds_u8_passes<2>())) : 0;
+    if (passes > 1) {
+        size_t lds2 = iu ? (m.u8_half ? lds_u8_half() : (passes == 4 ? lds_u8_passes<4>() : lds_u8_passes<2>())) : 0;
         for (int k = 0; k < 2; ++k) {
             if (!fi[k]) continue;
             const size_t l = m.kind[k] == 2 ? lds_f32_two_pass<32, 20, 9, 5>() : lds_f32_two_pass<64, 9, 7, 4>();
             lds2 = l > lds2 ? l : lds2;
         }
-        if (g_passes == 4) RLX_LAUNCH((conv_dw_multi_kernel<4>), grid, kThreads, lds2, rlx::as_stream(stream), m);
+        if (adam) {
+            rlx_adam::EarlyDev e;
+            const int rc = rlx_adam::early_dev(adam, &e, "rlx_conv_dw_multi_adam");
+            if (rc != RLX_OK) return rc;
+            if (riders > e.n_early) riders = riders_first ? (e.n_early + 7) / 8 * 8 : e.n_early;
+            const size_t red = sizeof(float) * rlx_adam::kBlock;
+            RLX_LAUNCH((conv_dw_multi_adam_kernel), grid + riders, kThreads, lds2 > red ? lds2 : red, rlx::as_stream(stream), m, e,
+                       riders, riders_first);
+        } else if (passes == 4) RLX_LAUNCH((conv_dw_multi_kernel<4>), grid, kThreads, lds2, rlx::as_stream(stream), m);
         else RLX_LAUNCH((conv_dw_multi_kernel<2>), grid, kThreads, lds2, rlx::as_stream(stream), m);
     } else {
         RLX_LAUNCH((conv_dw_multi_kernel<1>), grid, kThreads, lds, rlx::as_stream(stream), m);
     }
     RLX_LAUNCH_CHECK();
     return RLX_OK;
+}
+
+}
+
+extern "C" {
+
+int rlx_conv_dw_multi(const rlx_conv_dw_item *items, rlx_splitk_job *jobs, int n_items, void *stream) {
+    return conv_dw_multi_impl(items, jobs, n_items, stream, nullptr, 0, 0);
+}
+
+int rlx_conv_dw_multi_adam(const rlx_conv_dw_item *items, rlx_splitk_job *jobs, int n_items, const rlx_adam_split_desc *adam,
+                           int riders, int riders_first, void *stream) {
+    RLX_REQUIRE(adam, "rlx_conv_dw_multi_adam: null Adam descriptor");
+    RLX_REQUIRE(riders >= 1 && riders <= 1024 && (!riders_first || riders % 8 == 0),
+                "rlx_conv_dw_multi_adam: 1 .. 1024 riders, a multiple of 8 when they are dispatched first");
+    return conv_dw_multi_impl(items, jobs, n_items, stream, adam, riders, riders_first ? 1 : 0);
 }
 
 int rlx_conv_dw_pairs_per_workgroup(int pairs) {
diff --git a/coach_amd/csrc/optim.hip b/coach_amd/csrc/optim.hip
--- a/coach_amd/csrc/optim.hip
+++ b/coach_amd/csrc/optim.hip
@@ -1,8 +1,9 @@
 #include "rlx_common.hpp"
+#include "adam_block_body.hpp"
 
 namespace {
 
-constexpr int kBlock = 256;
+using rlx_adam::kBlock;
 
 #if defined(__HIP_DEVICE_COMPILE__) && !defined(__gfx950__) && !defined(__gfx942__)
 #error "optim.hip: the last-arriver ticket protocol is written for gfx950 (gfx942-compatible) only"
@@ -158,7 +159,44 @@
     }
 }
 
-constexpr int kNormIt = 4;
+using rlx_adam::kNormIt;
+
+__device__ __forceinline__ void adam_norm_finish(const float old, unsigned int *ticket, float *sumsq_part, const int nparts,
+                                                 float *state, const float b1p, const float b2p, const float beta1,
+                                                 const float beta2, float *norm_out, const float *acc_src, float *acc_dst,
+                                                 const int n_acc, float *red, int *last_s) {
+    if (threadIdx.x == 0) {
+        asm volatile("" ::"v"(old) : "memory");
+        *last_s = draw_last_ticket(ticket);
+    }
+    __syncthreads();
+    if (!*last_s) return;
+    __builtin_amdgcn_fence(__ATOMIC_ACQUIRE, "agent");
+    float s = 0.f, part[4];
+#pragma unroll
+    for (int k = 0; k < 4; ++k) {
+        const int i = threadIdx.x + k * kBlock;
+        part[k] = i < nparts ? __hip_atomic_load(&sumsq_part[i], __ATOMIC_RELAXED, __HIP_MEMORY_SCOPE_AGENT) : 0.f;
+    }
+#pragma unroll
+    for (int k = 0; k < 4; ++k)
+        if ((int)threadIdx.x + k * kBlock < nparts) s += part[k];
+    for (int i = threadIdx.x + 4 * kBlock; i < nparts; i += kBlock)
+        s += __hip_atomic_load(&sumsq_part[i], __ATOMIC_RELAXED, __HIP_MEMORY_SCOPE_AGENT);
+    red[threadIdx.x] = s;
+    __syncthreads();
+    for (int d = kBlock >> 1; d > 0; d >>= 1) {
+        if (threadIdx.x < d) red[threadIdx.x] += red[threadIdx.x + d];
+        __syncthreads();
+    }
+    if (threadIdx.x == 0) {
+        norm_out[0] = sqrtf(red[0]);
+        state[0] = b1p * beta1;
+        state[1] = b2p * beta2;
+        for (int i = 0; i < n_acc; ++i) acc_dst[i] += acc_src[i];
+    }
+}
+
 template <bool MIX>
 __global__ void __launch_bounds__(kBlock)
 adam_step_norm_kernel(float *__restrict__ w, const float *__restrict__ g, float *__restrict__ m, float *__restrict__ v,
@@ -168,92 +206,29 @@
     __shared__ float red[kBlock];
     __shared__ int last_s;
     const float b1p = state[0], b2p = state[1];
-    const float alpha = lr * sqrtf(1.f - b2p) / (1.f - b1p);
-    const float omb1 = 1.f - beta1, omb2 = 1.f - beta2;
-    const long long stride = (long long)gridDim.x * blockDim.x;
-    const long long n4 = n >> 2;
-    const long long i0 = (long long)blockIdx.x * blockDim.x + threadIdx.x;
-    float4 gw[kNormIt], mw[kNormIt], vw[kNormIt], ww[kNormIt], tw[kNormIt];
-#pragma unroll
-    for (int it = 0; it < kNormIt; ++it) {
-        const long long i = i0 + it * stride;
-        if (i < n4) {
-            gw[it] = reinterpret_cast<const float4 *>(g)[i];
-            mw[it] = reinterpret_cast<float4 *>(m)[i];
-            vw[it] = reinterpret_cast<float4 *>(v)[i];
-            ww[it] = reinterpret_cast<float4 *>(w)[i];
-            if (MIX) tw[it] = reinterpret_cast<float4 *>(target)[i];
-        }
-    }
-    const long long it0 = (n4 << 2) + i0;
-    const bool has_tail = it0 < n;
-    const float gt = has_tail ? g[it0] : 0.f;
-    float ss = 0.f;
-#pragma unroll
-    for (int it = 0; it < kNormIt; ++it)
-        if (i0 + it * stride < n4) {
-            const float *gp = &gw[it].x;
-#pragma unroll
-            for (int k = 0; k < 4; ++k) ss += gp[k] * gp[k];
-        }
-    if (has_tail) ss += gt * gt;
-    red[threadIdx.x] = ss;
-    __syncthreads();
-    for (int d = kBlock >> 1; d > 0; d >>= 1) {
-        if (threadIdx.x < d) red[threadIdx.x] += red[threadIdx.x + d];
-        __syncthreads();
-    }
-    float old = 0.f;
-    if (threadIdx.x == 0)
-        old = __hip_atomic_exchange(&sumsq_part[blockIdx.x], red[0], __ATOMIC_RELAXED, __HIP_MEMORY_SCOPE_AGENT);
-#pragma unroll
-    for (int it = 0; it < kNormIt; ++it) {
-        const long long i = i0 + it * stride;
-        if (i < n4) {
-            float *gp = &gw[it].x, *mp = &mw[it].x, *vp = &vw[it].x, *wp = &ww[it].x, *tp = &tw[it].x;
-#pragma unroll
-            for (int k = 0; k < 4; ++k) {
-                const float gr = gp[k] * grad_scale;
-                mp[k] += (gr - mp[k]) * omb1;
-                vp[k] += (gr * gr - vp[k]) * omb2;
-                wp[k] -= (mp[k] * alpha) / (sqrtf(vp[k]) + eps);
-                if (MIX) tp[k] = rate * wp[k] + one_minus_rate * tp[k];
-            }
-            reinterpret_cast<float4 *>(m)[i] = mw[it];
-            reinterpret_cast<float4 *>(v)[i] = vw[it];
-            reinterpret_cast<float4 *>(w)[i] = ww[it];
-            if (MIX) reinterpret_cast<float4 *>(target)[i] = tw[it];
-        }
-    }
-    if (has_tail) {
-        const float gr = gt * grad_scale;
-        m[it0] += (gr - m[it0]) * omb1;
-        v[it0] += (gr * gr - v[it0]) * omb2;
-        w[it0] -= (m[it0] * alpha) / (sqrtf(v[it0]) + eps);
-        if (MIX) target[it0] = rate * w[it0] + one_minus_rate * target[it0];
-    }
-    if (threadIdx.x == 0) {
-        asm volatile("" ::"v"(old) : "memory");
-        last_s = draw_last_ticket(ticket);
-    }
-    __syncthreads();
-    if (!last_s) return;
-    __builtin_amdgcn_fence(__ATOMIC_ACQUIRE, "agent");
-    float s = 0.f;
-    for (int i = threadIdx.x; i < (int)gridDim.x; i += kBlock)
-        s += __hip_atomic_load(&sumsq_part[i], __ATOMIC_RELAXED, __HIP_MEMORY_SCOPE_AGENT);
-    red[threadIdx.x] = s;
-    __syncthreads();
-    for (int d = kBlock >> 1; d > 0; d >>= 1) {
-        if (threadIdx.x < d) red[threadIdx.x] += red[threadIdx.x + d];
-        __syncthreads();
-    }
-    if (threadIdx.x == 0) {
-        norm_out[0] = sqrtf(red[0]);
-        state[0] = b1p * beta1;
-        state[1] = b2p * beta2;
-        for (int i = 0; i < n_acc; ++i) acc_dst[i] += acc_src[i];
-    }
+    const rlx_adam::Coef c = rlx_adam::coef(b1p, b2p, lr, beta1, beta2, eps, grad_scale, rate, one_minus_rate);
+    const float old = rlx_adam::block_step<MIX, true>(w, g, m, v, n, c, sumsq_part, target, (int)blockIdx.x, (int)gridDim.x, red);
+    adam_norm_finish(old, ticket, sumsq_part, (int)gridDim.x, state, b1p, b2p, beta1, beta2, norm_out, acc_src, acc_dst, n_acc,
+                     red, &last_s);
+}
+
+__global__ void __launch_bounds__(kBlock) adam_early_kernel(const rlx_adam::EarlyDev e) {
+    __shared__ float red[kBlock];
+    rlx_adam::early_blocks(e, (int)blockIdx.x, (int)gridDim.x, red);
+}
+
+__global__ void __launch_bounds__(kBlock)
+adam_late_kernel(float *__restrict__ w, const float *__restrict__ g, float *__restrict__ m, float *__restrict__ v,
+                 long long n, float lr, float beta1, float beta2, float eps, float *state, float grad_scale,
+                 float *sumsq_part, const int *__restrict__ late, int blocks, unsigned int *ticket, float *norm_out,
+                 const float *acc_src, float *acc_dst, int n_acc) {
+    __shared__ float red[kBlock];
+    __shared__ int last_s;
+    const float b1p = state[0], b2p = state[1];
+    const rlx_adam::Coef c = rlx_adam::coef(b1p, b2p, lr, beta1, beta2, eps, grad_scale, 0.f, 0.f);
+    const float old = rlx_adam::block_step<false, true>(w, g, m, v, n, c, sumsq_part, nullptr, late[blockIdx.x], blocks, red);
+    adam_norm_finish(old, ticket, sumsq_part, blocks, state, b1p, b2p, beta1, beta2, norm_out, acc_src, acc_dst, n_acc, red,
+                     &last_s);
 }
 
 __global__ void adam_advance_kernel(float *state, float beta1, float beta2) {
@@ -459,6 +434,69 @@
     return RLX_OK;
 }
 
+int rlx_adam_step_blocks(long long n, long long workspace_floats, int *blocks_host) {
+    RLX_REQUIRE(n > 0 && blocks_host, "rlx_adam_step_blocks: bad arguments");
+    int blocks = rlx::grid_for(n / 4 + 1, kBlock, 1024);
+    if (blocks > workspace_floats) blocks = (int)workspace_floats;
+    *blocks_host = (blocks >= 1 && g_norm_in_kernel == 2 && (n >> 2) <= (long long)blocks * kBlock * kNormIt) ? blocks : 0;
+    return RLX_OK;
+}
+
+int rlx_adam_split_blocks(long long n, int blocks, const long long *ranges_host, int n_ranges, int *early_host,
+                          int *n_early_host, int *late_host, int *n_late_host) {
+    RLX_REQUIRE(n > 0 && blocks >= 1 && n_ranges >= 0 && (ranges_host || !n_ranges) && early_host && n_early_host &&
+                    late_host && n_late_host, "rlx_adam_split_blocks: bad arguments");
+    const long long n4 = n >> 2, stride = (long long)blocks * kBlock;
+    RLX_REQUIRE(n4 <= stride * kNormIt, "rlx_adam_split_blocks: %lld parameters do not fit %d register-held blocks", n, blocks);
+    int ne = 0, nl = 0;
+    for (int vb = 0; vb < blocks; ++vb) {
+        bool early = !(vb == 0 && (n & 3));
+        bool any = false;
+        for (int it = 0; it < kNormIt && early; ++it) {
+            const long long a = (long long)vb * kBlock + it * stride;
+            if (a >= n4) break;
+            const long long lo = 4 * a, hi = 4 * (a + kBlock < n4 ? a + kBlock : n4);
+            bool inside = false;
+            for (int r = 0; r < n_ranges && !inside; ++r) inside = ranges_host[2 * r] <= lo && hi <= ranges_host[2 * r + 1];
+            early = inside;
+            any = true;
+        }
+        if (early && any) early_host[ne++] = vb;
+        else late_host[nl++] = vb;
+    }
+    if (nl == 0) late_host[nl++] = early_host[--ne];
+    *n_early_host = ne;
+    *n_late_host = nl;
+    return RLX_OK;
+}
+
+int rlx_adam_tf1_step_early(const rlx_adam_split_desc *d, int workgroups, void *stream) {
+    rlx_adam::EarlyDev e;
+    const int rc = rlx_adam::early_dev(d, &e, "rlx_adam_tf1_step_early");
+    if (rc != RLX_OK) return rc;
+    RLX_REQUIRE(workgroups >= 1 && workgroups <= 1024, "rlx_adam_tf1_step_early: 1 .. 1024 workgroups");
+    if (e.n_early == 0) return RLX_OK;
+    if (workgroups > e.n_early) workgroups = e.n_early;
+    RLX_LAUNCH((adam_early_kernel), workgroups, kBlock, 0, rlx::as_stream(stream), e);
+    RLX_LAUNCH_CHECK();
+    return RLX_OK;
+}
+
+int rlx_adam_tf1_step_late(const rlx_adam_split_desc *d, float *norm_out, const float *acc_src, float *acc_dst, int n_acc,
+                           unsigned int *ticket, void *stream) {
+    rlx_adam::EarlyDev e;
+    const int rc = rlx_adam::early_dev(d, &e, "rlx_adam_tf1_step_late");
+    if (rc != RLX_OK) return rc;
+    RLX_REQUIRE(norm_out && ticket, "rlx_adam_tf1_step_late: null pointer");
+    RLX_REQUIRE(n_acc == 0 || (acc_src && acc_dst && n_acc > 0 && n_acc <= 64),
+                "rlx_adam_tf1_step_late: bad signal accumulation arguments");
+    RLX_LAUNCH((adam_late_kernel), d->n_late, kBlock, 0, rlx::as_stream(stream), d->weights, d->grads, d->m, d->v, d->n,
+               d->learning_rate, d->beta1, d->beta2, d->epsilon, d->state, d->grad_scale, d->partials, d->late, d->blocks, ticket,
+               norm_out, acc_src, acc_dst, n_acc);
+    RLX_LAUNCH_CHECK();
+    return RLX_OK;
+}
+
 int rlx_mix_weights(float *target, const float *online, long long n, double rate, void *stream) {
     RLX_REQUIRE(target && online && n > 0, "rlx_mix_weights: bad arguments");
     RLX_REQUIRE((((uintptr_t)target | (uintptr_t)online) & 15) == 0,
diff --git a/coach_amd/nn/graph.py b/coach_amd/nn/graph.py
--- a/coach_amd/nn/graph.py
+++ b/coach_amd/nn/graph.py
@@ -134,6 +134,8 @@
 CONV_DW_U8 = True
 CONV_DW_F32 = True
 CONV_DW_ONE_LAUNCH = True
+ADAM_RIDERS = 1024
+ADAM_RIDERS_FIRST = False
 
 
 class Workspace:
@@ -207,6 +209,7 @@
 
     ppo_tail = None
     per_tail = None
+    early_adam = None
 
     def flush_ppo_tail(self):
         tail, self.ppo_tail = self.ppo_tail, None
@@ -281,6 +284,10 @@
         self.init, self.params = init, params
         self.kname, self.bname = name + "/kernel", name + "/bias"
         params.add_group([(self.kname, (in_features, units)), (self.bname, (units,))], towers)
+
+    def group_range(self):
+        lo, _, towers, per = self.params.entries[self.kname]
+        return lo, lo + per * towers
 
     def initialize(self, rng):
         for t in range(self.T):
@@ -412,6 +419,9 @@
             x.grad_is_dz = lower is not None
         if need_dw:
             ctx.commit_deferred(job)
+            ea = ctx.early_adam
+            if ea is not None and job is not None and job.splits <= 1 and (t0, T) == (0, self.T) and p is ea.adam.params:
+                ea.final.append(self.group_range())
 
 
 class NoisyDense(Layer):
@@ -1081,7 +1091,12 @@
             while collect:
                 group = sorted(collect[:3], key=lambda e: (not e[0].x_is_u8, -e[0].H))
                 collect = collect[3:]
-                _rlx.conv_dw_multi([it for it, _ in group], [j for _, j in group], ctx.stream)
+                ea = ctx.early_adam
+                ride = ea is not None and not ea.done and _rlx.GEMM_HOOK is None and ea.covered()
+                _rlx.conv_dw_multi([it for it, _ in group], [j for _, j in group], ctx.stream,
+                                   adam=(ea.desc, ADAM_RIDERS, ADAM_RIDERS_FIRST) if ride else None)
+                if ride:
+                    ea.done = True
                 for _, j in group:
                     ctx.commit_deferred(j, reserved=True)
             while later:
@@ -1095,6 +1110,23 @@
                 ctx.flush_deferred()
 
 
+class EarlyAdam:
+
+    def __init__(self, adam, ranges, split, grad_scale, lr):
+        blocks, lists, n_early, n_late, partials = split
+        self.adam, self.ranges, self.grad_scale = adam, ranges, float(grad_scale)
+        self.final, self.done = [], False
+        p, d = adam.params, _rlx.AdamSplitDesc()
+        d.weights, d.grads, d.m, d.v, d.n = p.weights.data_ptr(), p.grads.data_ptr(), adam.m.data_ptr(), adam.v.data_ptr(), p.size
+        d.learning_rate, d.beta1, d.beta2, d.epsilon, d.grad_scale = lr, adam.beta1, adam.beta2, adam.eps, float(grad_scale)
+        d.state, d.partials, d.blocks = adam.state.data_ptr(), partials.data_ptr(), blocks
+        d.early, d.late, d.n_early, d.n_late = lists.data_ptr(), lists.data_ptr() + 4 * n_early, n_early, n_late
+        self.desc = d
+
+    def covered(self):
+        return all(r in self.final for r in self.ranges)
+
+
 class AdamState:
 
     def __init__(self, params, lr, beta1=0.9, beta2=0.99, epsilon=1e-4):
@@ -1105,6 +1137,8 @@
         self.state = torch.empty(2, dtype=torch.float32, device=dev)
         self.ticket = torch.zeros(_rlx.ADAM_TICKET_WORDS, dtype=torch.int32, device=dev)
         self.one_launch = True
+        self._splits = {}
+        self.split_steps = 0
         _rlx.lib().adam_init(self.m, self.v, params.size, self.state, beta1, beta2, _rlx.current_stream())
 
     def step(self, grad_scale=1.0, lr=None, norm_out=None, workspace=None, acc=None, grads=None, mix_target=None,
@@ -1121,6 +1155,47 @@
             return
         if mix_target is not None:
             raise ValueError("the two-launch Adam path does not fuse the target update")
+        self._step_two_launch(p, g, lr, grad_scale, norm_out, workspace, acc)
+
+    MAX_BLOCKS = 1024
+
+    def prepare_early(self, ranges, workspace_floats=MAX_BLOCKS):
+        key = (tuple((int(a), int(b)) for a, b in ranges), int(workspace_floats))
+        if key not in self._splits:
+            lib, n = _rlx.lib(), self.params.size
+            blocks = ctypes.c_int()
+            lib.adam_step_blocks(n, int(workspace_floats), ctypes.byref(blocks))
+            split = None
+            if self.one_launch and blocks.value >= 1 and key[0]:
+                nb = blocks.value
+                flat = (ctypes.c_longlong * (2 * len(key[0])))(*[x for r in key[0] for x in r])
+                early, late = (ctypes.c_int * nb)(), (ctypes.c_int * nb)()
+                ne, nl = ctypes.c_int(), ctypes.c_int()
+                lib.adam_split_blocks(n, nb, flat, len(key[0]), early, ctypes.byref(ne), late, ctypes.byref(nl))
+                if ne.value > 0:
+                    dev = self.m.device
+                    lists = torch.tensor(list(early[:ne.value]) + list(late[:nl.value]), dtype=torch.int32).to(dev)
+                    split = (nb, lists, ne.value, nl.value, torch.zeros(nb, dtype=torch.float32, device=dev))
+            self._splits[key] = split
+        return self._splits[key]
+
+    def arm_early(self, ranges, grad_scale=1.0, lr=None, workspace_floats=MAX_BLOCKS, prepare=True):
+        key = (tuple((int(a), int(b)) for a, b in ranges), int(workspace_floats))
+        split = self.prepare_early(ranges, workspace_floats) if prepare else self._splits.get(key)
+        return EarlyAdam(self, key[0], split, grad_scale, self.lr if lr is None else lr) if split is not None else None
+
+    def step_early(self, ea, workgroups=256):
+        _rlx.lib().adam_tf1_step_early(ctypes.byref(ea.desc), int(workgroups), _rlx.current_stream())
+        ea.done = True
+
+    def step_late(self, ea, norm_out, acc=None):
+        if not ea.done:
+            raise ValueError("the early blocks of this step have not run")
+        self.split_steps += 1
+        _rlx.lib().adam_tf1_step_late(ctypes.byref(ea.desc), norm_out, acc[0] if acc else None, acc[1] if acc else None,
+                                      int(acc[2]) if acc else 0, self.ticket, _rlx.current_stream())
+
+    def _step_two_launch(self, p, g, lr, grad_scale, norm_out, workspace, acc):
         if norm_out is not None:
             _rlx.lib().adam_tf1_norm(p.weights, g, self.m, self.v, p.size, lr, self.beta1,
                                      self.beta2, self.eps, self.state, grad_scale, norm_out, workspace,
diff --git a/coach_amd/nn/networks.py b/coach_amd/nn/networks.py
--- a/coach_amd/nn/networks.py
+++ b/coach_amd/nn/networks.py
@@ -300,9 +300,33 @@
         if k > 0:
             self.torso.backward(self.ctx, acts, layers=(0, k))
 
+    def early_adam_ranges(self):
+        if not self.image:
+            return []
+        return [l.group_range() for l in self.torso.layers if type(l) is G.Dense]
+
+    def prepare_early_adam(self):
+        ranges = self.early_adam_ranges()
+        return bool(ranges) and self.adam.prepare_early(ranges) is not None
+
+    def arm_early_adam(self, grad_scale=1.0, prepare=True):
+        ranges = self.early_adam_ranges()
+        self.ctx.early_adam = self.adam.arm_early(ranges, grad_scale, prepare=prepare) if ranges else None
+        return self.ctx.early_adam is not None
+
+    def disarm_early_adam(self):
+        self.ctx.early_adam = None
+
     def finish_update(self, grad_scale=1.0, signal_acc=None):
-        self.apply_gradients(grad_scale, with_norm=True,
-                             acc=(self.scalars, signal_acc, 6) if signal_acc is not None else None)
+        acc = (self.scalars, signal_acc, 6) if signal_acc is not None else None
+        ea, self.ctx.early_adam = self.ctx.early_adam, None
+        if ea is not None and ea.done:
+            if float(grad_scale) != ea.grad_scale:
+                raise ValueError("finish_update(%r): the early part of this step ran with gradient scale %r"
+                                 % (grad_scale, ea.grad_scale))
+            self.adam.step_late(ea, self.norm, acc)
+            return
+        self.apply_gradients(grad_scale, with_norm=True, acc=acc)
 
     def train_minibatch(self, obs, B, actions, advantages, value_targets, old_probs,
                         clip_rescaler=1.0, grad_scale=1.0, ratio_out=None, clipped_out=None):
diff --git a/include/rlx.h b/include/rlx.h
--- a/include/rlx.h
+++ b/include/rlx.h
@@ -448,6 +448,24 @@
                       float *workspace, long long workspace_floats, const float *acc_src, float *acc_dst, int n_acc,
                       float *target, double mix_rate, unsigned int *ticket, void *stream);
 int rlx_adam_norm_in_kernel(int on);
+typedef struct rlx_adam_split_desc {
+    float *weights;
+    const float *grads;
+    float *m, *v;
+    long long n;
+    float learning_rate, beta1, beta2, epsilon, grad_scale;
+    float *state;
+    float *partials;
+    int blocks;
+    const int *early, *late;
+    int n_early, n_late;
+} rlx_adam_split_desc;
+int rlx_adam_step_blocks(long long n, long long workspace_floats, int *blocks_host);
+int rlx_adam_split_blocks(long long n, int blocks, const long long *ranges_host, int n_ranges, int *early_host,
+                          int *n_early_host, int *late_host, int *n_late_host);
+int rlx_adam_tf1_step_early(const rlx_adam_split_desc *desc_host, int workgroups, void *stream);
+int rlx_adam_tf1_step_late(const rlx_adam_split_desc *desc_host, float *norm_out, const float *acc_src, float *acc_dst,
+                           int n_acc, unsigned int *ticket, void *stream);
 int rlx_mix_weights(float *target, const float *online, long long n, double rate,
                     void *stream);
 int rlx_global_norm(const float *x, long long n, float *norm_out, float *workspace,
@@ -670,6 +688,8 @@
     float *workspace; long long workspace_floats;
 } rlx_conv_dw_item;
 int rlx_conv_dw_multi(const rlx_conv_dw_item *items_host, rlx_splitk_job *jobs_host, int n_items, void *stream);
+int rlx_conv_dw_multi_adam(const rlx_conv_dw_item *items_host, rlx_splitk_job *jobs_host, int n_items,
+                           const rlx_adam_split_desc *adam_host, int riders, int riders_first, void *stream);
 int rlx_conv_dw_passes(int passes);
 int rlx_conv_dw_pairs_per_workgroup(int pairs);
 
```

New measurement: 40040 env-steps/s (median of 6 runs). +3.3%, better.
